# DearCaat/MHIM-MIL

Measured on AMD Instinct MI355X. Metric: patch-instances/sec through MHIM fwd+bwd, N=10k D=1024, higher is better.
Workload: dtype f32; 1 GPU; c2: MHIM(ABMIL) train step, one bag N=10000 D=1024 per GPU per step (teacher fwd + select + student fwd + bwd + Adam + EMA); rotating_bags_per_gpu=8, matrix_core_form=bf16x3, parallelism=dp1, launch=hipGraph replay, one graph per resident bag

## Files before the change

### include/mhimx.h

```cpp
#ifndef MHIMX_H
#define MHIMX_H

#include <stdint.h>

#ifdef __cplusplus
extern "C" {
#endif

#define MHIMX_VERSION 620

enum { MHIMX_ACT_NONE = 0, MHIMX_ACT_RELU = 1, MHIMX_ACT_GELU = 2, MHIMX_ACT_TANH = 3 };

enum { MHIMX_PREC_F32 = 0, MHIMX_PREC_F16S = 1, MHIMX_PREC_BF16X3 = 2 };

const char* mhimx_last_error(void);
int mhimx_version(void);


typedef struct {
  const float* A; int64_t lda; const int64_t* rows;
  const float* B; int64_t ldb;
  float* C; int64_t ldc;
  int64_t M, N, K;
  const float* bias;
// ... 81 lines not shown
  float* C; int64_t ldc;
  int64_t M, K1, K2;
  int32_t splits; float* ws;
  int32_t accumulate;
  int32_t prec;
  int64_t ws_floats;
  mhimx_reduce_list* defer;
} mhimx_gemm_tn_args;
int mhimx_gemm_tn(void* stream, const mhimx_gemm_tn_args* a);

int mhimx_pair_planes(void* stream, const float* x, int64_t ldx, int64_t M, int64_t K, float* out);

#define MHIMX_PREP_MAX 32
typedef struct { int32_t kind; const float* in; float* out; int64_t R, C; } mhimx_prep_job;
int mhimx_prep_batch(void* stream, const mhimx_prep_job* jobs, int32_t n);

int mhimx_transpose(void* stream, const float* in, float* out, int64_t R, int64_t C);

typedef struct {
  int64_t E;
  int64_t A;
  int32_t act;
  int32_t gated;
  int32_t prec;
  const float* wa; const float* ba;
  const float* wb; const float* bb;
  const float* wc; const float* bc;
  const float* wa_frag;
  float gate_drop_p;
  uint64_t gate_drop_seed;
} mhimx_scorer;

typedef struct {
  const float* T1; int64_t M1; const float* T2; int64_t M2;
  float* s; float* stats; float* z;
  float* u_pre;
  const float* wp; int64_t C; float* cproj;
  void* ws; int64_t ws_bytes;
  const float* bp; float* pscore;
  const int64_t* rows1;
  const uint8_t* excl;
  const mhimx_prep_job* ride_jobs;
  int32_t n_ride_jobs;
  int32_t phase; int32_t tail_tokens;
  const void* ride_merge;
  const float* ride_X; int64_t ride_R; void* ride_ws; int64_t ride_ws_bytes;
  int32_t rode_merge;
  const float* tail_wa_t;
  int64_t tail_row0;
  int32_t no_backward;
} mhimx_pool_io;
int64_t mhimx_abmil_pool_ws_bytes(int64_t M, int64_t E, int64_t A, int32_t gated);
int mhimx_abmil_pool_fwd(void* stream, const mhimx_scorer* sc, mhimx_pool_io* io);

typedef struct {
  const float* g_z;
  float* dT1; float* dT2;
  float* d_wa; float* d_ba; float* d_wb; float* d_bb; float* d_wc; float* d_bc;
  const float* wa_t; const float* wb_t;
  int32_t accumulate;
  int32_t splits;
  mhimx_reduce_list* defer;
  const float* wa_t_frag;
  void* img; const void* img_dact; float* img_part; int64_t img_rows;
} mhimx_pool_grad;
int mhimx_abmil_pool_bwd(void* stream, const mhimx_scorer* sc, const mhimx_pool_io* io, const mhimx_pool_grad* g);

int mhimx_softmax_from_stats(void* stream, const float* s, const float* stats, float* attn, int64_t M);

int mhimx_lse_merge(void* stream, const float* parts, int64_t W, int64_t E, float* stats, float* z);

int mhimx_pseudo_score(void* stream, const float* s, const float* stats, const float* cproj, const float* bp,
                       float* score, float* attn_out, int64_t M, int64_t C);

int mhimx_layernorm_fwd(void* stream, const float* x, int64_t M, int64_t E, const float* w, const float* b, float* y, float* mean,
                        float* rstd);
int mhimx_layernorm_bwd(void* stream, const float* dy, const float* x, int64_t M, int64_t E, const float* w, const float* mean,
                        const float* rstd, float* dx, float* d_w, float* d_b, int32_t accumulate, float* ws);
int mhimx_layernorm_bwd_res(void* stream, const float* dy, const float* x, int64_t M, int64_t E, const float* w, const float* mean,
                            const float* rstd, const float* resid, float* dx, float* d_w, float* d_b, int32_t accumulate, float* ws);
int mhimx_dropout_apply(void* stream, const float* x, float* out, int64_t M, int64_t E, float p, uint64_t seed, const uint64_t* tick);
int mhimx_dropout_apply_proj(void* stream, const float* x, float* out, int64_t M, int64_t E, float p, uint64_t seed, const uint64_t* tick);
int mhimx_softmax_rows(void* stream, const float* x, float* y, int64_t R, int64_t L, float alpha);
int mhimx_softmax_rows_bwd(void* stream, const float* y, const float* dy, float* dx, int64_t R, int64_t L, float alpha);
int mhimx_landmark_mean(void* stream, const float* x, int64_t ldx, int64_t T, int64_t l, int64_t C, float* out);
int mhimx_landmark_mean_bwd(void* stream, const float* dout, int64_t T, int64_t l, int64_t C, float* dx, int64_t ldx, int32_t accumulate);
int mhimx_affine_ident(void* stream, const float* x, float* y, int64_t B, int64_t n, float a, float b);
int mhimx_axpby(void* stream, const float* x, float* y, int64_t n, float alpha, float beta);
int mhimx_pinv_init(void* stream, const float* a, int64_t B, int64_t n, float* z, float* stats, float* ws);
int mhimx_pinv_init_bwd(void* stream, const float* dz, const float* z0, const float* stats, int64_t B, int64_t n, float* da, float* ws);
int mhimx_resconv(void* stream, const float* v, int64_t ldv, const float* w, int64_t KS, int64_t dh, int64_t T, int64_t C, float* out,
                  int64_t ldo, int32_t accumulate, int32_t flip);
int64_t mhimx_resconv_dw_ws_floats(int64_t T, int64_t C, int64_t dh, int64_t KS);
int mhimx_resconv_dw(void* stream, const float* dout, int64_t ldo, const float* v, int64_t ldv, int64_t KS, int64_t dh, int64_t T,
                     int64_t C, float* dw, float* ws);
typedef struct mhimx_nys {
  const float* q; const float* k; const float* v;
  int64_t ld, T;
  const float* ql; const float* kl;
  int64_t ldl;
  float scale;
  float* ws;
  int64_t ws_floats;
} mhimx_nys;
int64_t mhimx_nys_ws_floats(int64_t T);
int mhimx_nys_a3v_fwd(void* stream, const mhimx_nys* a, float* a3v, float* lse3);
int mhimx_nys_out_fwd(void* stream, const mhimx_nys* a, const float* w2, float* out, int64_t ldo, float* lse1, int32_t accumulate);
int mhimx_nys_out_bwd(void* stream, const mhimx_nys* a, const float* w2, const float* dout, int64_t ldd, const float* lse1,
                      float* delta1, float* dq, int64_t lddq, float* dkl, int64_t lddl, float* dw2);
int mhimx_nys_a3v_bwd(void* stream, const mhimx_nys* a, const float* a3v, const float* da3v, const float* lse3, float* dk, float* dv,
                      int64_t lddk, int32_t accumulate_dv, float* dql, int64_t lddl);
int mhimx_nys_cls_attn(void* stream, const mhimx_nys* a, const float* lse3, const float* u, float* r);
int64_t mhimx_bn_ws_floats(int64_t M, int64_t C);
int mhimx_bn_fwd(void* stream, const float* x, int64_t M, int64_t C, const float* w, const float* b, float eps, int32_t training, float* mean,
                 float* rstd, float* var_out, float* y, float* ws);
int mhimx_bn_bwd(void* stream, const float* dy, const float* x, int64_t M, int64_t C, const float* w, const float* mean, const float* rstd,
                 int32_t training, float* dx, float* dw, float* db, float* ws);
int mhimx_sincos_add(void* stream, const float* x, const int64_t* pos_xy, int64_t N, int64_t C, float* out);
int mhimx_ppeg_combine(void* stream, const float* w7, const float* w5, const float* w3, const float* b7, const float* b5,
                       const float* b3, int64_t C, float* wc, float* bc);
int mhimx_ppeg_fwd(void* stream, const float* x, int64_t N, int64_t C, const float* wc, const float* bc, float* y,
                   int64_t grid );
int64_t mhimx_ppeg_bwd_ws_floats(int64_t N, int64_t C);
int mhimx_ppeg_bwd(void* stream, const float* dy, const float* x, int64_t N, int64_t C, const float* wc, float* dx, float* dwc, float* dbc,
                   float* ws, int64_t grid);
typedef struct { int64_t H, cell0, ncell, out0, out1; } mhimx_ppeg_band;
int64_t mhimx_ppeg_side(int64_t N, int64_t* wrapN);
int mhimx_ppeg_band_fwd(void* stream, const float* xb, const mhimx_ppeg_band* band, int64_t C, const float* wc, const float* bc, float* y);
int64_t mhimx_ppeg_band_bwd_ws_floats(int64_t n_out, int64_t C);
int mhimx_ppeg_band_bwd(void* stream, const float* dyb, const float* xb, const mhimx_ppeg_band* band, int64_t n_dw, int64_t C, const float* wc,
                        float* dx, float* dwc, float* dbc, float* ws);
int mhimx_scale_heads(void* stream, const float* v, int64_t ldv, const float* a, int64_t lda, int64_t dh, int64_t T, int64_t C, float* out);

int64_t mhimx_select_ws_bytes(int64_t N);
int mhimx_select_mask(void* stream, const float* score, int64_t N, int64_t k, int64_t n_sel, int32_t largest,
                      const int64_t* perm, const int64_t* other, int64_t n_other,
                      int64_t* mask_ids, int64_t* len_keep_dev, int64_t* topk_sorted ,
                      void* ws, int64_t ws_bytes);

int mhimx_select_rows(void* stream, const float* score, int64_t N, int64_t k, int64_t n_sel, int32_t largest,
                      uint64_t rand_seed, const uint64_t* tick, int64_t merge_R, int64_t* rows_out, int64_t* mask_ids,
                      void* ws, int64_t ws_bytes, int32_t merge_first );

int mhimx_select_rows_img(void* stream, const float* score, int64_t N, int64_t k, int64_t n_sel, int32_t largest, uint64_t rand_seed,
                          const uint64_t* tick, int64_t merge_R, int64_t* rows_out, int64_t* rows_img, int64_t img_merge_off, void* ws,
                          int64_t ws_bytes, int32_t merge_first);
int mhimx_vote_scores(void* stream, const float* attn, int64_t H, int64_t N, int64_t k, int32_t largest,
                      float* vote, void* ws, int64_t ws_bytes);

int mhimx_compose_ids(void* stream, const int64_t* a, const int64_t* b, int64_t* out, int64_t n);
int mhimx_random_perm(void* stream, int64_t n, uint64_t seed, const uint64_t* tick, const int64_t* src, int64_t* out);

typedef struct { int64_t row0, N, k, n_sel, merge_R, out0; uint64_t seed; } mhimx_select_bag;
int64_t mhimx_select_rows_many_ws_bytes(int32_t n_bags, const mhimx_select_bag* bags);
int mhimx_select_rows_many(void* stream, const float* score, int32_t n_bags, const mhimx_select_bag* bags, const uint64_t* tick,
                           int64_t* rows_out, void* ws, int64_t ws_bytes, int32_t merge_first);

typedef struct {
  int64_t E; int64_t k;
  int64_t heads; int64_t dim_head;
  const float* q_param;
  const float* ln_w; const float* ln_b;
  const float* wkv; const float* wq; const float* wo; const float* bo;
  const float* wkv_t; const float* wq_t; const float* wo_t;
  float mm;
  float drop_p; uint64_t drop_seed;
  int32_t prec;
  const uint64_t* drop_tick;
  const float* wkv_frag;
  const int64_t* x_rows;
  int32_t prepared;
  int64_t own_lo, own_n;
  float rep;
  int32_t rows_done;
} mhimx_merge;
int64_t mhimx_merge_ws_bytes(int64_t R, int64_t E, int64_t k, int64_t heads, int64_t dim_head);
int mhimx_merge_fwd(void* stream, const mhimx_merge* m, const float* X, int64_t R, float* z, float* q_new,
                    int32_t update_q, void* ws, int64_t ws_bytes);
typedef struct {
  float* d_ln_w; float* d_ln_b; float* d_wkv; float* d_wq; float* d_wo; float* d_bo;
  int32_t accumulate; int32_t splits;
  mhimx_reduce_list* defer;
} mhimx_merge_grad;
int64_t mhimx_merge_part_floats(void);
int mhimx_merge_fwd_part(void* stream, const mhimx_merge* m, const float* X, int64_t R, float* part, void* ws, int64_t ws_bytes);
int mhimx_merge_fwd_finish(void* stream, const mhimx_merge* m, const float* parts, int32_t W, int64_t R, float* z, float* q_new,
                           int32_t update_q, void* ws, int64_t ws_bytes);
int mhimx_merge_bwd(void* stream, const mhimx_merge* m, const float* X, int64_t R, const float* dz, float* dX,
                    const mhimx_merge_grad* g, void* ws, int64_t ws_bytes);
int mhimx_merge_bwd_park(const mhimx_merge* m, const float* X, int64_t R, const float* dz, float* dX, const mhimx_merge_grad* g, void* ws,
                         int64_t ws_bytes);

int mhimx_act_bwd(void* stream, float* dH, const float* H, const float* pre, int64_t M, int64_t E, int32_t act,
                  float drop_p, uint64_t drop_seed, const uint8_t* drop_mask, const int64_t* rows, float* colsum_out,
                  int32_t accumulate, void* ws, int64_t ws_bytes, const uint64_t* drop_tick);
int mhimx_mul_colsum(void* stream, float* dH, const float* dact, int64_t M, int64_t E, float* colsum_out, int32_t accumulate,
                     void* ws, int64_t ws_bytes, mhimx_reduce_list* defer );
int mhimx_rows_dpre(void* stream, const float* dH, const void* dact16, const int64_t* rows, int64_t L, int64_t E, float* dpre,
                    float* colsum_out, int32_t accumulate, void* ws, int64_t ws_bytes, mhimx_reduce_list* defer );
// ... 41 lines not shown

int mhimx_adam_ema(void* stream, float* p, const float* g, float* m, float* v, float* teacher, int64_t n_train,
                   int64_t n_all, int64_t step, float lr, float beta1, float beta2, float eps, float weight_decay,
                   float grad_scale, float ema_mm, int32_t zero_grad ,
                   const uint64_t* step_dev ,
                   const float* mm_table, int64_t mm_len );

typedef struct {
  float* p; float* g; float* m; float* v; float* teacher;
  int64_t n_train, n_all;
  int64_t step; const uint64_t* step_dev;
  float lr; const float* lr_table; int64_t lr_len;
  float beta1, beta2, eps, weight_decay, grad_scale;
  float ema_mm; const float* mm_table; int64_t mm_len;
  int32_t zero_grad;
  const float* g_extra; int64_t n_extra; int64_t extra_pitch;
  float clip_norm;
  float* ws; int64_t ws_floats;
  mhimx_reduce_list* fold;
  int64_t extra_lo;
  int32_t extra_only;
} mhimx_optim_args;
int mhimx_optim_step(void* stream, const mhimx_optim_args* a);

#define MHIMX_STEP_MAX_ROWS 262144
#define MHIMX_WINDOW_MAX 8
typedef struct {
  const float* w1; const float* b1;
  const float* wa; const float* wc;
  const float* wp; const float* bp;
  float* q;
  const float* ln_w; const float* ln_b;
  const float* wkv; const float* wq; const float* wo; const float* bo;
} mhimx_step_params;
typedef struct {
  float* w1; float* b1; float* wa; float* wc; float* wp; float* bp; float* ln_w; float* ln_b; float* wkv; float* wq; float* wo; float* bo;
} mhimx_step_grads;
typedef struct {
  int64_t D, E, A, C, k;
  int32_t act, da_act;
  int32_t attn2score;
  float drop_p_teacher, drop_p_student;
  float merge_drop_p, merge_mm;
  float temp_t, main_alpha, aux_alpha;
  mhimx_step_params student, teacher;
  mhimx_step_grads grad;
  float* p; float* g; float* m; float* v; float* p_teacher;
  int64_t n_train, n_all;
  float lr, beta1, beta2, eps, weight_decay, ema_mm;
  const float* mm_table; int64_t mm_len; const float* lr_table; int64_t lr_len;
  uint64_t* tick; uint64_t* opt_step;
  float* q_out;
  int32_t time_project;
  void* side_stream;
} mhimx_step_cfg;
typedef struct { int64_t k_top, n_sel, len_keep, Lk, R; } mhimx_step_counts;
int mhimx_step_counts_of(int64_t N, double mask_ratio_h, double mask_ratio_hr, double merge_ratio, mhimx_step_counts* out);
typedef struct { uint64_t drop_teacher, drop_student, select, mca; } mhimx_step_seeds;
typedef struct {
  int64_t total;
  int64_t logits, losses;
  int64_t score;
  int64_t rows_all;
  int64_t H_teacher, H_student;
  int64_t dact;
  int64_t z_teacher, z_student, g_z;
  int64_t dH;
} mhimx_step_layout;
int mhimx_step_layout_of(const mhimx_step_cfg* cfg, int64_t N, const mhimx_step_counts* cnt, mhimx_step_layout* out);
int mhimx_step_run(void* stream, const mhimx_step_cfg* cfg, const float* X, int64_t ldx, int64_t N, const int64_t* label_dev,
                   const mhimx_step_counts* cnt, const mhimx_step_seeds* seeds, int64_t host_step, void* ws, int64_t ws_bytes, int32_t update);
int mhimx_step_project_ms(float* ms_out, float* empty_ms_out, int32_t cap);
int mhimx_step_run_many(void* stream, const mhimx_step_cfg* cfg, int32_t n_bags, const float* const* X, const int64_t* ldx, const int64_t* N,
                        const int64_t* const* labels_dev, const mhimx_step_counts* cnt, const mhimx_step_seeds* seeds, int64_t host_step0,
                        void* ws, int64_t ws_bytes);

int mhimx_pure_step_layout_of(const mhimx_step_cfg* cfg, int64_t N, mhimx_step_layout* out);
int mhimx_pure_step_run(void* stream, const mhimx_step_cfg* cfg, const float* X, int64_t ldx, int64_t N, const int64_t* label_dev,
                        uint64_t drop_seed, int64_t host_step, void* ws, int64_t ws_bytes, int32_t update);
int mhimx_pure_step_run_many(void* stream, const mhimx_step_cfg* cfg, int32_t n_bags, const float* const* X, const int64_t* ldx, const int64_t* N,
                             const int64_t* const* labels_dev, const uint64_t* drop_seeds, int64_t host_step0, void* ws, int64_t ws_bytes);

typedef struct { int64_t total, bag0, bag_stride, grad_slab; mhimx_step_layout bag; } mhimx_window_layout;
int mhimx_window_layout_of(const mhimx_step_cfg* cfg, int32_t n_bags, int64_t N, const mhimx_step_counts* cnt, mhimx_window_layout* out);
int mhimx_window_run(void* stream, const mhimx_step_cfg* cfg, int32_t n_bags, const float* const* X, int64_t ldx, int64_t N,
                     const int64_t* const* labels_dev, const mhimx_step_counts* cnt, const mhimx_step_seeds* seeds, int64_t host_step, void* ws,
                     int64_t ws_bytes, int32_t update);

#define MHIMX_PURE_WINDOW_MAX 32
#define MHIMX_PURE_WINDOW_MAX_ROWS 524288
typedef struct {
  const float* X; int64_t ldx, N;
  const int64_t* label_dev;
  uint64_t drop_seed;
} mhimx_pure_window_bag;
typedef struct {
  int64_t total, rows;
  int64_t logits, losses;
  int64_t H, dact, s, stats, z, g_z;
  int64_t row0[MHIMX_PURE_WINDOW_MAX];
} mhimx_pure_window_layout;
int mhimx_pure_window_layout_of(const mhimx_step_cfg* cfg, int32_t n_bags, const mhimx_pure_window_bag* bags, mhimx_pure_window_layout* out);
int mhimx_pure_window_run(void* stream, const mhimx_step_cfg* cfg, int32_t n_bags, const mhimx_pure_window_bag* bags, int64_t host_step,
                          void* ws, int64_t ws_bytes, int32_t update);

#define MHIMX_RAGGED_WINDOW_MAX 32
// ... 241 lines not shown
```

### mhim_mil_amd/_lib.py

```python
from __future__ import annotations

import ctypes as C
import os

HERE = os.path.dirname(os.path.abspath(__file__))
LIB_PATH = os.path.join(HERE, os.environ.get("MHIMX_LIB_NAME", "libmhimx.so"))

c_f32p = C.c_void_p
c_i64p = C.c_void_p
c_u8p = C.c_void_p

ABI_VERSION = 620

ACT = {None: 0, "none": 0, "identity": 0, "relu": 1, "gelu": 2, "tanh": 3}
PREC = {"f32": 0, "f16s": 1, "bf16x3": 2}


def act_code(name, allowed):
    n = name.lower() if isinstance(name, str) else None
    return ACT[n] if n in allowed else 0


class GemmNT(C.Structure):
    _fields_ = [("A", c_f32p), ("lda", C.c_int64), ("rows", c_i64p),
# ... 38 lines not shown
    _fields_ = [("kind", C.c_int32), ("inp", C.c_void_p), ("out", C.c_void_p), ("R", C.c_int64), ("C", C.c_int64)]


class ReduceJob(C.Structure):
    _fields_ = [("kind", C.c_int32), ("accumulate", C.c_int32), ("parts", c_f32p), ("out", c_f32p),
                ("G", C.c_int64), ("W", C.c_int64), ("ld", C.c_int64), ("K1", C.c_int64), ("K2", C.c_int64), ("ldo", C.c_int64)]


REDUCE_MAX = 16


SIDE_BYTES = 512


class SideWork(C.Structure):
    _fields_ = [("pending", C.c_int32), ("reserved", C.c_int32), ("blob", C.c_ubyte * SIDE_BYTES)]


class ParkedGemm(C.Structure):
    _fields_ = [("pending", C.c_int32), ("reserved", C.c_int32), ("blob", C.c_ubyte * 128)]


class ReduceListC(C.Structure):
    _fields_ = [("j", ReduceJob * REDUCE_MAX), ("n", C.c_int32), ("side", SideWork), ("parked", ParkedGemm), ("pre", SideWork)]


class GemmTN(C.Structure):
    _fields_ = [("A", c_f32p), ("lda", C.c_int64),
                ("B", c_f32p), ("ldb", C.c_int64), ("rows", c_i64p),
                ("C", c_f32p), ("ldc", C.c_int64),
                ("M", C.c_int64), ("K1", C.c_int64), ("K2", C.c_int64),
                ("splits", C.c_int32), ("ws", c_f32p),
                ("accumulate", C.c_int32), ("prec", C.c_int32), ("ws_floats", C.c_int64),
                ("defer", C.c_void_p)]


class Scorer(C.Structure):
    _fields_ = [("E", C.c_int64), ("A", C.c_int64), ("act", C.c_int32), ("gated", C.c_int32), ("prec", C.c_int32),
                ("wa", c_f32p), ("ba", c_f32p), ("wb", c_f32p), ("bb", c_f32p), ("wc", c_f32p), ("bc", c_f32p),
                ("wa_frag", c_f32p), ("gate_drop_p", C.c_float), ("gate_drop_seed", C.c_uint64)]


class PoolIO(C.Structure):
    _fields_ = [("T1", c_f32p), ("M1", C.c_int64), ("T2", c_f32p), ("M2", C.c_int64),
                ("s", c_f32p), ("stats", c_f32p), ("z", c_f32p), ("u_pre", c_f32p),
                ("wp", c_f32p), ("C", C.c_int64), ("cproj", c_f32p),
                ("ws", C.c_void_p), ("ws_bytes", C.c_int64), ("bp", c_f32p), ("pscore", c_f32p), ("rows1", c_i64p),
                ("excl", C.c_void_p), ("ride_jobs", C.c_void_p), ("n_ride_jobs", C.c_int32),
                ("phase", C.c_int32), ("tail_tokens", C.c_int32), ("ride_merge", C.c_void_p), ("ride_X", c_f32p), ("ride_R", C.c_int64),
                ("ride_ws", C.c_void_p), ("ride_ws_bytes", C.c_int64), ("rode_merge", C.c_int32), ("tail_wa_t", c_f32p), ("tail_row0", C.c_int64),
                ("no_backward", C.c_int32)]


class PoolGrad(C.Structure):
    _fields_ = [("g_z", c_f32p), ("dT1", c_f32p), ("dT2", c_f32p),
                ("d_wa", c_f32p), ("d_ba", c_f32p), ("d_wb", c_f32p), ("d_bb", c_f32p), ("d_wc", c_f32p),
                ("d_bc", c_f32p), ("wa_t", c_f32p), ("wb_t", c_f32p),
                ("accumulate", C.c_int32), ("splits", C.c_int32), ("defer", C.c_void_p), ("wa_t_frag", c_f32p),
                ("img", C.c_void_p), ("img_dact", C.c_void_p), ("img_part", c_f32p), ("img_rows", C.c_int64)]


class Merge(C.Structure):
    _fields_ = [("E", C.c_int64), ("k", C.c_int64), ("heads", C.c_int64), ("dim_head", C.c_int64),
                ("q_param", c_f32p), ("ln_w", c_f32p), ("ln_b", c_f32p),
                ("wkv", c_f32p), ("wq", c_f32p), ("wo", c_f32p), ("bo", c_f32p),
                ("wkv_t", c_f32p), ("wq_t", c_f32p), ("wo_t", c_f32p),
                ("mm", C.c_float), ("drop_p", C.c_float), ("drop_seed", C.c_uint64), ("prec", C.c_int32), ("drop_tick", C.c_void_p),
                ("wkv_frag", c_f32p), ("x_rows", c_i64p), ("prepared", C.c_int32), ("own_lo", C.c_int64), ("own_n", C.c_int64),
                ("rep", C.c_float), ("rows_done", C.c_int32)]


class MergeGrad(C.Structure):
    _fields_ = [("d_ln_w", c_f32p), ("d_ln_b", c_f32p), ("d_wkv", c_f32p), ("d_wq", c_f32p), ("d_wo", c_f32p),
                ("d_bo", c_f32p), ("accumulate", C.c_int32), ("splits", C.c_int32), ("defer", C.c_void_p)]


_P = C.c_void_p
_I64 = C.c_int64
_I32 = C.c_int32
_F = C.c_float
_U64 = C.c_uint64


class Nys(C.Structure):
    _fields_ = [("q", C.c_void_p), ("k", C.c_void_p), ("v", C.c_void_p), ("ld", C.c_int64), ("T", C.c_int64),
                ("ql", C.c_void_p), ("kl", C.c_void_p), ("ldl", C.c_int64), ("scale", C.c_float),
                ("ws", C.c_void_p), ("ws_floats", C.c_int64)]


class BmmStep(C.Structure):
    _fields_ = [("A", C.c_void_p), ("B", C.c_void_p), ("C", C.c_void_p), ("PN", C.c_void_p), ("PT", C.c_void_p),
                ("PN2", C.c_void_p), ("PT2", C.c_void_p), ("D", C.c_void_p), ("D2", C.c_void_p), ("alpha", C.c_float), ("ident", C.c_float),
                ("alpha2", C.c_float), ("ident2", C.c_float), ("dscale", C.c_float), ("d2scale", C.c_float), ("kind", C.c_int32)]


class OptimArgs(C.Structure):
    _fields_ = [("p", C.c_void_p), ("g", C.c_void_p), ("m", C.c_void_p), ("v", C.c_void_p), ("teacher", C.c_void_p),
                ("n_train", C.c_int64), ("n_all", C.c_int64), ("step", C.c_int64), ("step_dev", C.c_void_p),
                ("lr", C.c_float), ("lr_table", C.c_void_p), ("lr_len", C.c_int64),
                ("beta1", C.c_float), ("beta2", C.c_float), ("eps", C.c_float), ("weight_decay", C.c_float), ("grad_scale", C.c_float),
                ("ema_mm", C.c_float), ("mm_table", C.c_void_p), ("mm_len", C.c_int64), ("zero_grad", C.c_int32),
                ("g_extra", C.c_void_p), ("n_extra", C.c_int64), ("extra_pitch", C.c_int64), ("clip_norm", C.c_float),
                ("ws", C.c_void_p), ("ws_floats", C.c_int64), ("fold", C.c_void_p), ("extra_lo", C.c_int64), ("extra_only", C.c_int32)]


class StepParams(C.Structure):
    _fields_ = [(n, C.c_void_p) for n in ("w1", "b1", "wa", "wc", "wp", "bp", "q", "ln_w", "ln_b", "wkv", "wq", "wo", "bo")]


class StepGrads(C.Structure):
    _fields_ = [(n, C.c_void_p) for n in ("w1", "b1", "wa", "wc", "wp", "bp", "ln_w", "ln_b", "wkv", "wq", "wo", "bo")]


class StepCfg(C.Structure):
    _fields_ = [("D", C.c_int64), ("E", C.c_int64), ("A", C.c_int64), ("C", C.c_int64), ("k", C.c_int64),
                ("act", C.c_int32), ("da_act", C.c_int32), ("attn2score", C.c_int32),
                ("drop_p_teacher", C.c_float), ("drop_p_student", C.c_float), ("merge_drop_p", C.c_float), ("merge_mm", C.c_float),
                ("temp_t", C.c_float), ("main_alpha", C.c_float), ("aux_alpha", C.c_float),
                ("student", StepParams), ("teacher", StepParams), ("grad", StepGrads),
                ("p", C.c_void_p), ("g", C.c_void_p), ("m", C.c_void_p), ("v", C.c_void_p), ("p_teacher", C.c_void_p),
                ("n_train", C.c_int64), ("n_all", C.c_int64),
                ("lr", C.c_float), ("beta1", C.c_float), ("beta2", C.c_float), ("eps", C.c_float), ("weight_decay", C.c_float), ("ema_mm", C.c_float),
                ("mm_table", C.c_void_p), ("mm_len", C.c_int64), ("lr_table", C.c_void_p), ("lr_len", C.c_int64),
                ("tick", C.c_void_p), ("opt_step", C.c_void_p), ("q_out", C.c_void_p), ("time_project", C.c_int32), ("side_stream", C.c_void_p)]


class StepCounts(C.Structure):
    _fields_ = [("k_top", C.c_int64), ("n_sel", C.c_int64), ("len_keep", C.c_int64), ("Lk", C.c_int64), ("R", C.c_int64)]


class StepSeeds(C.Structure):
    _fields_ = [("drop_teacher", C.c_uint64), ("drop_student", C.c_uint64), ("select", C.c_uint64), ("mca", C.c_uint64)]


class StepLayout(C.Structure):
    _fields_ = [(n, C.c_int64) for n in ("total", "logits", "losses", "score", "rows_all", "H_teacher", "H_student", "dact", "z_teacher",
                                        "z_student", "g_z", "dH")]


class WindowLayout(C.Structure):
    _fields_ = [("total", C.c_int64), ("bag0", C.c_int64), ("bag_stride", C.c_int64), ("grad_slab", C.c_int64), ("bag", StepLayout)]


WINDOW_MAX = 8
STEP_MAX_ROWS = 262144


class InferCfg(C.Structure):
    _fields_ = [("D", C.c_int64), ("E", C.c_int64), ("A", C.c_int64), ("C", C.c_int64), ("act", C.c_int32), ("da_act", C.c_int32),
                ("p", StepParams)]


class InferBag(C.Structure):
    _fields_ = [("X", c_f32p), ("ldx", C.c_int64), ("N", C.c_int64)]


class InferOut(C.Structure):
    _fields_ = [(n, c_f32p) for n in ("logits", "z", "stats", "score", "attn", "loss")]


class InferDsmilCfg(C.Structure):
    _fields_ = [("D", C.c_int64), ("E", C.c_int64), ("C", C.c_int64), ("act", C.c_int32), ("cls_attn", C.c_int32), ("no_norm", C.c_int32),
                ("pad", C.c_int32)] + [(n, c_f32p) for n in ("w1", "b1", "wi", "bi", "wq0", "bq0", "wq2", "bq2", "wv", "bv", "wfcc", "bfcc")]


class InferDsmilOut(C.Structure):
    _fields_ = [(n, c_f32p) for n in ("logits_bag", "logits_ins", "logits", "B")] + [("crit", C.c_void_p)] + [(n, c_f32p) for n in ("attn", "loss")]


INFER_MAX = 32


class TransmilLayer(C.Structure):
    _fields_ = [(n, c_f32p) for n in ("ln_w", "ln_b", "w_qkv", "w_out", "b_out", "conv_w")]


class InferTransmilCfg(C.Structure):
# ... 82 lines not shown
                ("q", c_f32p), ("q_out", c_f32p), ("k", C.c_int64), ("cls_attn", C.c_int32), ("pad", C.c_int32),
                ("drop_p_teacher", C.c_float), ("merge_drop_p", C.c_float), ("merge_mm", C.c_float), ("temp_t", C.c_float),
                ("aux_alpha", C.c_float), ("ema_mm", C.c_float), ("p_teacher", c_f32p), ("mm_table", c_f32p), ("mm_len", C.c_int64)]


class DsmilMhimWindowLayout(C.Structure):
    _fields_ = [(n, C.c_int64) for n in ("total", "rows", "tok_rows", "logits", "losses", "logits_bag", "logits_ins", "B", "crit", "B_teacher",
                                        "H_teacher", "H_student", "dact", "score", "rows_all", "tokens")] + [
        ("row0", C.c_int64 * DSMIL_MHIM_WINDOW_MAX), ("tok0", C.c_int64 * DSMIL_MHIM_WINDOW_MAX)]


RAGGED_WINDOW_MAX = 32
RAGGED_WINDOW_MAX_ROWS = 524288


class RaggedWindowBag(C.Structure):
    _fields_ = [("X", c_f32p), ("ldx", C.c_int64), ("N", C.c_int64), ("label_dev", C.c_void_p), ("cnt", StepCounts), ("seeds", StepSeeds)]


class RaggedWindowLayout(C.Structure):
    _fields_ = [(n, C.c_int64) for n in ("total", "rows", "logits", "losses", "score", "rows_all", "H_teacher", "H_student", "dact", "dpre",
                                        "z_teacher", "z_student")] + [("row0", C.c_int64 * RAGGED_WINDOW_MAX)]


class SurvSpec(C.Structure):
    _fields_ = [("alpha", C.c_float), ("eps", C.c_float), ("censor_dev", C.c_void_p * INFER_MAX), ("risk", C.c_void_p)]


SYMBOLS = {
    "mhimx_last_error": (C.c_char_p, []),
    "mhimx_version": (C.c_int, []),
    "mhimx_gemm_nt": (C.c_int, [_P, C.POINTER(GemmNT)]),
    "mhimx_pool_finalize": (C.c_int, [_P, _P, _P, _P, _I64, _I64, _P, _P, _P, _P, _P, _I64, _I64, _P]),
    "mhimx_proj_score_parts": (_I64, [_I64]),
    "mhimx_proj_score_xch_floats": (_I64, [_I64]),
    "mhimx_bag_project": (C.c_int, [_P, C.POINTER(BagProject)]),
    "mhimx_bag_project_multi": (C.c_int, [_P, _P, _I32]),
    "mhimx_gemm_nn": (C.c_int, [_P, C.POINTER(GemmNT), _F, _I32, _P]),
    "mhimx_prep_batch": (C.c_int, [_P, C.POINTER(PrepJob), _I32]),
    "mhimx_pair_planes": (C.c_int, [_P, _P, _I64, _I64, _I64, _P]),
    "mhimx_lse_merge": (C.c_int, [_P, _P, _I64, _I64, _P, _P]),
    "mhimx_gemm_batched": (C.c_int, [_P, _I32, C.POINTER(GemmNT), _I32, _I64, _I64, _I64, _F, _I32, _P]),
    "mhimx_gemm_tn": (C.c_int, [_P, C.POINTER(GemmTN)]),
    "mhimx_transpose": (C.c_int, [_P, _P, _P, _I64, _I64]),
    "mhimx_abmil_pool_ws_bytes": (_I64, [_I64, _I64, _I64, _I32]),
    "mhimx_abmil_pool_fwd": (C.c_int, [_P, C.POINTER(Scorer), C.POINTER(PoolIO)]),
    "mhimx_abmil_pool_bwd": (C.c_int, [_P, C.POINTER(Scorer), C.POINTER(PoolIO), C.POINTER(PoolGrad)]),
    "mhimx_softmax_from_stats": (C.c_int, [_P, _P, _P, _P, _I64]),
    "mhimx_pseudo_score": (C.c_int, [_P, _P, _P, _P, _P, _P, _P, _I64, _I64]),
    "mhimx_select_ws_bytes": (_I64, [_I64]),
    "mhimx_select_mask": (C.c_int, [_P, _P, _I64, _I64, _I64, _I32, _P, _P, _I64, _P, _P, _P, _P, _I64]),
    "mhimx_select_rows": (C.c_int, [_P, _P, _I64, _I64, _I64, _I32, _U64, _P, _I64, _P, _P, _P, _I64, _I32]),
    "mhimx_select_rows_img": (C.c_int, [_P, _P, _I64, _I64, _I64, _I32, _U64, _P, _I64, _P, _P, _I64, _P, _I64, _I32]),
    "mhimx_vote_scores": (C.c_int, [_P, _P, _I64, _I64, _I64, _I32, _P, _P, _I64]),
    "mhimx_compose_ids": (C.c_int, [_P, _P, _P, _P, _I64]),
    "mhimx_random_perm": (C.c_int, [_P, _I64, _U64, _P, _P, _P]),
    "mhimx_select_rows_many_ws_bytes": (_I64, [_I32, _P]),
    "mhimx_select_rows_many": (C.c_int, [_P, _P, _I32, _P, _P, _P, _P, _I64, _I32]),
    "mhimx_merge_ws_bytes": (_I64, [_I64, _I64, _I64, _I64, _I64]),
    "mhimx_merge_fwd": (C.c_int, [_P, C.POINTER(Merge), _P, _I64, _P, _P, _I32, _P, _I64]),
    "mhimx_merge_part_floats": (_I64, []),
    "mhimx_merge_fwd_part": (C.c_int, [_P, C.POINTER(Merge), _P, _I64, _P, _P, _I64]),
    "mhimx_merge_fwd_finish": (C.c_int, [_P, C.POINTER(Merge), _P, _I32, _I64, _P, _P, _I32, _P, _I64]),
    "mhimx_merge_bwd": (C.c_int, [_P, C.POINTER(Merge), _P, _I64, _P, _P, C.POINTER(MergeGrad), _P, _I64]),
    "mhimx_merge_bwd_park": (C.c_int, [C.POINTER(Merge), _P, _I64, _P, _P, C.POINTER(MergeGrad), _P, _I64]),
    "mhimx_act_bwd": (C.c_int, [_P, _P, _P, _P, _I64, _I64, _I32, _F, _U64, _P, _P, _P, _I32, _P, _I64, _P]),
    "mhimx_softmax_cols": (C.c_int, [_P, _P, _P, _I64, _I64, _F]),
    "mhimx_softmax_cols_bwd": (C.c_int, [_P, _P, _P, _P, _I64, _I64, _F]),
    "mhimx_colmax": (C.c_int, [_P, _P, _I64, _I64, _P, _P]),
    "mhimx_rowmax": (C.c_int, [_P, _P, _I64, _I64, _P]),
    "mhimx_dsmil_head": (C.c_int, [_P, _P, _P, _P, _P, _P, _I64, _I64, _F, _F, _F, _F, _P, _P, _P, _P, _P]),
    "mhimx_mul_colsum": (C.c_int, [_P, _P, _P, _I64, _I64, _P, _I32, _P, _I64, _P]),
    "mhimx_rows_dpre": (C.c_int, [_P, _P, _P, _P, _I64, _I64, _P, _P, _I32, _P, _I64, _P]),
    "mhimx_bmm_affine": (C.c_int, [_P, _I32, _P, _I32, _I64, _I64, _I64, C.c_float, C.c_float]),
    "mhimx_bmm_affine2": (C.c_int, [_P, _I32, _P, _I32, _I64, _I64, _I64, C.c_float, C.c_float, _P, C.c_float, C.c_float]),
    "mhimx_bmm_affine_pair": (C.c_int, [_P, _I32, C.POINTER(GemmNT), _F, _F, _I32, C.POINTER(GemmNT), _F, _F, _I32, _I64]),
    "mhimx_shard_flags": (C.c_int, [_P, _P, _I64, _I64, _I64, _I64, _I64, _I32, _P]),
    "mhimx_shard_gather": (C.c_int, [_P, _P, _I64, _P, _I64, _I64, _I64, _P]),
    "mhimx_shard_scatter": (C.c_int, [_P, _P, _I64, _P, _I64, _I64, _I64, _P]),
    "mhimx_rows_dpre_image": (C.c_int, [_P, _P, _P, _P, _I64, _I64, _P, _P, _I32, _P, _I64, _P]),
    "mhimx_rows_dpre_image_c": (C.c_int, [_P, _P, _P, _P, _I64, _I64, _P, _P, _I32, _P, _I64, _P]),
    "mhimx_rows_dpre_image_k": (C.c_int, [_P, _P, _P, _P, _I64, _I64, _P, _P, _I32, _P, _I64, _P]),
    "mhimx_wgrad_image_bytes": (_I64, [_I64, _I64]),
    "mhimx_wgrad_ws_floats": (_I64, [_I64, _I64, _I64]),
    "mhimx_bag_wgrad": (C.c_int, [_P, _P]),
    "mhimx_bag_wgrad_multi": (C.c_int, [_P, _P, _I32]),
    "mhimx_wgrad_multi_ws_floats": (C.c_int64, [_I64, _I64, _I64, _I32]),
    "mhimx_reduce_flush": (C.c_int, [_P, _P]),
    "mhimx_cls_metrics_ws_bytes": (C.c_int64, [_I64, _I64, _I64]),
    "mhimx_cls_metrics": (C.c_int, [_P, _P, _I64, _P, _I64, _I64, _I32, _P, _I64, _P, _P, _I64]),
    "mhimx_surv_nll": (C.c_int, [_P, _P, _I64, _P, _P, _I64, _I64, _F, _F, _F, _P, _P, _P]),
    "mhimx_cindex_ws_bytes": (C.c_int64, [_I64, _I64]),
    "mhimx_cindex": (C.c_int, [_P, _P, _P, _P, _I64, _P, _I64, _F, _P, _P, _I64]),
    "mhimx_colsum": (C.c_int, [_P, _P, _I64, _I64, _P, _I32, _P, _I64]),
    "mhimx_head_fwd_bwd": (C.c_int, [_P, _P, _P, _P, _P, _P, _I64, _I64, _F, _F, _F, _F, _P, _P, _P, _P, _P, _I32, _P, _P]),
    "mhimx_head_surv_fwd_bwd": (C.c_int, [_P, _P, _P, _P, _P, _P, _P, _I64, _I64, _F, _F, _F, _F, _F, _F, _P, _P, _P, _P, _P, _P, _I32]),
    "mhimx_adam_ema": (C.c_int, [_P, _P, _P, _P, _P, _P, _I64, _I64, _I64, _F, _F, _F, _F, _F, _F, _F, _I32, _P, _P, _I64]),
    "mhimx_bmm_chain": (C.c_int, [_P, C.POINTER(BmmStep), _I32, _I32, _P]),
    "mhimx_optim_step": (C.c_int, [_P, C.POINTER(OptimArgs)]),
    "mhimx_stream_copy": (C.c_int, [_P, _P, _P, _I64]),
    "mhimx_tick": (C.c_int, [_P, _P]),
    "mhimx_layernorm_fwd": (C.c_int, [_P, _P, _I64, _I64, _P, _P, _P, _P, _P]),
    "mhimx_layernorm_bwd": (C.c_int, [_P, _P, _P, _I64, _I64, _P, _P, _P, _P, _P, _P, _I32, _P]),
    "mhimx_layernorm_bwd_res": (C.c_int, [_P, _P, _P, _I64, _I64, _P, _P, _P, _P, _P, _P, _P, _I32, _P]),
    "mhimx_dropout_apply": (C.c_int, [_P, _P, _P, _I64, _I64, _F, _U64, _P]),
    "mhimx_dropout_apply_proj": (C.c_int, [_P, _P, _P, _I64, _I64, _F, _U64, _P]),
# ... 102 lines not shown
```

### mhim_mil_amd/csrc/rows.hip

```cpp
#include <math.h>
#include <string.h>

#include "mca2_rows.hpp"
#include "reduce_jobs.hpp"

namespace mhimx {

int gemm_nt(hipStream_t st, const mhimx_gemm_nt_args& g);
int gemm_tn(hipStream_t st, const mhimx_gemm_tn_args& g);
bool scorer_fused_ok(int64_t E, int64_t A, int gated, int prec, const float* T, const float* wa, const float* wp, int64_t C);
int scorer_fused_fwd(hipStream_t st, const float* T, int64_t M, const float* wa, const float* wa_frag, const float* ba, int act, const float* wc,
                     const float* bc, const float* wp, int C, float* u_pre, float* s_out, float* cproj, float* pm, float* pl,
                     float* pz, int max_parts, const int64_t* rows, const uint8_t* excl, const mhimx_prep_job* ride_jobs, int n_ride_jobs,
                     const void* merge_rows);
int merge2_fwd_rows_args(const mhimx_merge* m, const float* X, int64_t R, void* ws, int64_t ws_bytes, M2RowsFwd* out);
int prep_batch(hipStream_t st, const mhimx_prep_job* jobs, int n);
int scorer_fused_bwd(hipStream_t st, const float* T, int64_t M, const float* u_pre, const float* s_in, const float* stats,
                     const float* g_z, const float* z, const float* wc, int act, const float* wa_t, const float* wa_t_frag, float* du,
                     float* dT, float* dwc_part, float* dbc_part, int max_parts, const int64_t* rows, const void* pre_side, int64_t gate_row0,
                     void* img, const void* img_dact, float* img_part, int64_t img_rows);

constexpr int ROWS_THREADS = 256;
constexpr int MAX_PART = 512;
constexpr int TN_SLABS = 128;

MHIMX_DEV float sigmoidf_(float x) { return 1.f / (1.f + __expf(-x)); }

constexpr int FWD_WAVES = 16;
template <int EPL>
__global__ __launch_bounds__(64 * FWD_WAVES) void score_rows_fwd_kernel(
    const float* __restrict__ T, int64_t M, int E, int A, int act, int gated, const float* __restrict__ u_pre,
    const float* __restrict__ wc, const float* __restrict__ bc, const float* __restrict__ wp, int C,
    float* __restrict__ s_out, float* __restrict__ cproj, float* __restrict__ pm, float* __restrict__ pl,
    float* __restrict__ pz, float gdrop_p, uint64_t gdrop_seed, int64_t row0 ) {
  extern __shared__ __attribute__((aligned(16))) float sm[];
  constexpr int NWV = FWD_WAVES;
  const int lane = threadIdx.x & 63, wave = threadIdx.x >> 6;
  const int ldu = A * (1 + gated);
  const float bias_c = bc ? bc[0] : 0.f;

  float mw = -INFINITY, lw = 0.f, zacc[EPL];
#pragma unroll
  for (int q = 0; q < EPL; ++q) zacc[q] = 0.f;

  for (int64_t n = (int64_t)blockIdx.x * NWV + wave; n < M; n += (int64_t)gridDim.x * NWV) {
    const float* up = u_pre + n * ldu;
    float part = 0.f;
    const bool gdrop = gated && gdrop_p > 0.f;
    const uint32_t rkey = gdrop ? drop_row_key(gdrop_seed, (uint64_t)(row0 + n)) : 0u;
    const float ginv = gdrop ? 1.f / (1.f - gdrop_p) : 1.f;
    for (int j = lane; j < A; j += 64) {
      float u = act_fwd(up[j], act);
      if (gated) {
        float sg = sigmoidf_(up[A + j]);
        if (gdrop) {
          u = drop_keep_k(rkey, (uint32_t)j, gdrop_p) ? u * ginv : 0.f;
          sg = drop_keep_k(rkey, (uint32_t)(A + j), gdrop_p) ? sg * ginv : 0.f;
        }
        u *= sg;
      }
      part += wc[j] * u;
    }
    const float s = wave_sum(part) + bias_c;
    const float* h = T + n * (int64_t)E;
    float hv[EPL];
#pragma unroll
    for (int q = 0; q < EPL; ++q) hv[q] = h[lane + 64 * q];
// ... 770 lines not shown

static int grid_for_ln(int64_t M) {
  int64_t g = cdiv(M, 4);
  if (g < 1) g = 1;
  if (g > MAX_PART) g = MAX_PART;
  return (int)g;
}

static int grid_for_rows(int64_t M) {
  int64_t g = cdiv(M, 20);
  if (g < 1) g = 1;
  if (g > MAX_PART) g = MAX_PART;
  return (int)g;
}

struct PoolWs {
  float *pm, *pl, *pz, *attn, *du, *dwc_part, *dbc_part, *u_pre, *tn_ws, *nt_ws;
};

static int64_t pool_ws_layout(Arena& ar, int64_t M, int64_t E, int64_t A, int gated, PoolWs* w) {
  const int64_t G = 2 * MAX_PART;
  PoolWs t;
  t.pm = ar.take<float>(G);
  t.pl = ar.take<float>(G);
  t.pz = ar.take<float>(G * E);
  t.attn = ar.take<float>(M);
  t.du = ar.take<float>(M * A * (1 + gated));
  t.dwc_part = ar.take<float>(G * A);
  t.dbc_part = ar.take<float>(G);
  t.u_pre = ar.take<float>(M * A * (1 + gated));
  t.tn_ws = ar.take<float>((int64_t)TN_SLABS * A * E);
  t.nt_ws = ar.take<float>(4 * M * A);
  if (w) *w = t;
  return ar.off;
}

template <typename F>
static int dispatch_epl(int64_t E, F&& f) {
  switch (E) {
    case 256: return f(std::integral_constant<int, 4>());
    case 512: return f(std::integral_constant<int, 8>());
    case 1024: return f(std::integral_constant<int, 16>());
    default: return fail(-1, "token width E=%lld unsupported (256, 512 or 1024)", (long long)E);
  }
}

static int check_scorer(const mhimx_scorer* sc) {
  MHIMX_CHECK_ARG(sc && sc->wa && sc->wc, "scorer: null weights");
  MHIMX_CHECK_ARG(sc->A > 0 && sc->A <= 512 && sc->A % 4 == 0, "scorer: A must be a multiple of 4, <= 512");
  MHIMX_CHECK_ARG(!sc->gated || sc->wb, "scorer: gated needs wb");
  return 0;
}

int abmil_pool_fwd(hipStream_t st, const mhimx_scorer* sc, mhimx_pool_io* io) {
  if (int r = check_scorer(sc)) return r;
  MHIMX_CHECK_ARG(io && io->T1 && io->M1 > 0 && io->s && io->stats && io->z, "pool_fwd: null io");
  MHIMX_CHECK_ARG(io->M2 == 0 || io->T2, "pool_fwd: M2>0 needs T2");
  MHIMX_CHECK_ARG(!io->cproj || (io->wp && io->C > 0), "pool_fwd: cproj needs wp, C");
  MHIMX_CHECK_ARG(!io->rows1 || (io->M2 == 0 && scorer_fused_ok(sc->E, sc->A, sc->gated, sc->prec, io->T1, sc->wa, io->cproj ? io->wp : nullptr, io->C)),
                  "pool_fwd: gathered tokens (rows1) need the one-pass scorer (E = 512, A = 128, plain form, not f32) and a single segment");
  MHIMX_CHECK_ARG(!io->excl || scorer_fused_ok(sc->E, sc->A, sc->gated, sc->prec, io->T1, sc->wa, io->cproj ? io->wp : nullptr, io->C),
                  "pool_fwd: excluded rows (excl) need the one-pass scorer (E = 512, A = 128, plain form, not f32)");
  const int64_t M = io->M1 + io->M2, E = sc->E, A = sc->A;
  const int gated = sc->gated ? 1 : 0;
  Arena ar(io->ws, io->ws_bytes);
  PoolWs w;
  pool_ws_layout(ar, M, E, A, gated, &w);
  MHIMX_CHECK_ARG(ar.ok(), "pool_fwd: workspace too small (%lld < %lld)", (long long)io->ws_bytes, (long long)ar.off);
  float* u_pre = io->u_pre ? io->u_pre : w.u_pre;
  const int64_t ldu = A * (1 + gated);
  if (io->phase != 0) {
    const int64_t K = io->tail_tokens, Ms1 = io->M1 - K;
    MHIMX_CHECK_ARG((io->phase == 1 || io->phase == 2) && K >= 1 && K <= FIN_MAXTOK && Ms1 >= 1 && io->M2 == 0 && !io->cproj && !io->pscore && !io->excl &&
                        E == 512 && A == 128 && scorer_fused_ok(E, A, gated, sc->prec, io->T1, sc->wa, nullptr, 0),
                    "pool_fwd: the two-call forward takes the one-pass scorer shapes, one segment, 1..%d tail tokens, no class projections", FIN_MAXTOK);
    const int tiles = (int)cdiv(Ms1, 32);
    const int G1 = tiles < MAX_PART ? tiles : MAX_PART;
    if (io->phase == 1) {
      M2RowsFwd mfbuf;
      const void* mf = nullptr;
      io->rode_merge = 0;
      if (io->ride_merge) {
        const int rc = merge2_fwd_rows_args(reinterpret_cast<const mhimx_merge*>(io->ride_merge), io->ride_X, io->ride_R, io->ride_ws, io->ride_ws_bytes,
                                            &mfbuf);
        if (rc < 0) return rc;
        if (rc == 0) { mf = &mfbuf; io->rode_merge = 1; }
      }
      const int g1 = scorer_fused_fwd(st, io->T1, Ms1, sc->wa, sc->wa_frag, sc->ba, sc->act, sc->wc, sc->bc, nullptr, 0, u_pre, io->s, nullptr, w.pm, w.pl,
                                      w.pz, MAX_PART, io->rows1, nullptr, io->ride_jobs, io->n_ride_jobs, mf);
      return g1 < 0 ? g1 : 0;
    }
    hipLaunchKernelGGL(pool_finalize_tok_kernel, bgrid((unsigned)cdiv(E, 64)), dim3(FIN_THREADS), 0, st, w.pm, w.pl, w.pz, G1, (int)E, io->stats, io->z, io->T1,
                       (io->rows1 && io->tail_row0 < 0) ? io->rows1 + Ms1 : nullptr, io->rows1 ? io->tail_row0 : Ms1, (int)K, sc->wa, io->tail_wa_t, sc->ba, sc->wc,
                       sc->bc, (int)A, sc->act, u_pre + Ms1 * ldu, io->s + Ms1, cur_batch());
    MHIMX_LAUNCH_CHECK();
    return 0;
  }

  const float* Ts[2] = {io->T1, io->T2};
  const int64_t Ms[2] = {io->M1, io->M2};
  int64_t off = 0;
  int G = 0;
  bool rode = false;
  for (int seg = 0; seg < 2; ++seg) {
    if (Ms[seg] == 0) continue;
    if (scorer_fused_ok(E, A, gated, sc->prec, Ts[seg], sc->wa, io->cproj ? io->wp : nullptr, io->C)) {
      const int g1 = scorer_fused_fwd(st, Ts[seg], Ms[seg], sc->wa, sc->wa_frag, sc->ba, sc->act, sc->wc, sc->bc, io->cproj ? io->wp : nullptr,
                                      (int)io->C, io->no_backward ? nullptr : u_pre + off * ldu, io->s + off, io->cproj ? io->cproj + off * io->C : nullptr,
                                      w.pm + G, w.pl + G, w.pz + (int64_t)G * E, MAX_PART, seg == 0 ? io->rows1 : nullptr,
                                      seg == 0 ? io->excl : nullptr, rode ? nullptr : io->ride_jobs, rode ? 0 : io->n_ride_jobs, nullptr);
      if (g1 < 0) return g1;
      rode = true;
      G += g1;
      off += Ms[seg];
      continue;
    }
    MHIMX_CHECK_ARG(cur_batch().n == 0, "pool_fwd: a bag-batched launch needs the one-pass scorer");
    mhimx_gemm_nt_args g = {};
    g.A = Ts[seg]; g.lda = E; g.B = sc->wa; g.ldb = E; g.C = u_pre + off * ldu; g.ldc = ldu;
    g.M = Ms[seg]; g.N = A; g.K = E; g.bias = sc->ba;
    g.ws = w.nt_ws; g.ws_floats = 4 * M * A;
    g.prec = sc->prec == MHIMX_PREC_F32 ? MHIMX_PREC_F32 : MHIMX_PREC_BF16X3;
    if (int r = gemm_nt(st, g)) return r;
    if (gated) {
      g.B = sc->wb; g.bias = sc->bb; g.C = u_pre + off * ldu + A;
      if (int r = gemm_nt(st, g)) return r;
    }
    int grid = (int)cdiv(Ms[seg], 5 * FWD_WAVES);
    if (grid < 1) grid = 1;
    if (grid > MAX_PART) grid = MAX_PART;
    const float* Tseg = Ts[seg];
    const int64_t Mseg = Ms[seg];
    int r = dispatch_epl(E, [&](auto epl) {
      constexpr int EPL = decltype(epl)::value;
      const size_t smem = (size_t)(FWD_WAVES * E + 2 * FWD_WAVES) * sizeof(float);
      if (smem > 48 * 1024)
        MHIMX_ONCE_PER_DEVICE(MHIMX_HIP(hipFuncSetAttribute((const void*)score_rows_fwd_kernel<EPL>, hipFuncAttributeMaxDynamicSharedMemorySize, (int)smem)));
      hipLaunchKernelGGL(score_rows_fwd_kernel<EPL>, dim3(grid), dim3(64 * FWD_WAVES), smem, st, Tseg, Mseg, (int)E, (int)A,
                         sc->act, gated, u_pre + off * ldu, sc->wc, sc->bc, io->cproj ? io->wp : nullptr, (int)io->C,
                         io->s + off, io->cproj ? io->cproj + off * io->C : nullptr, w.pm + G, w.pl + G,
                         w.pz + (int64_t)G * E, sc->gate_drop_p, sc->gate_drop_seed, off);
      MHIMX_LAUNCH_CHECK();
      return 0;
    });
    if (r) return r;
    G += grid;
    off += Ms[seg];
  }
  if (!rode && io->ride_jobs && io->n_ride_jobs > 0)
    if (int r = prep_batch(st, io->ride_jobs, io->n_ride_jobs)) return r;
  MHIMX_CHECK_ARG(!io->pscore || io->cproj, "pool_fwd: pscore needs cproj (and wp)");
  static_assert(2 * MAX_PART <= FIN_THREADS, "pool_finalize_kernel reads one partial per thread");
  const int64_t ps_blocks = io->pscore ? (cdiv(io->M1, FIN_THREADS) < 64 ? cdiv(io->M1, FIN_THREADS) : 64) : 0;
  hipLaunchKernelGGL(pool_finalize_kernel, bgrid((unsigned)(cdiv(E, 64) + ps_blocks)), dim3(FIN_THREADS), 0, st, w.pm, w.pl, w.pz, G, (int)E, io->stats,
                     io->z, io->s, io->cproj, io->bp, (int)io->C, io->M1, io->pscore, cur_batch());
  MHIMX_LAUNCH_CHECK();
  return 0;
}

int abmil_pool_bwd(hipStream_t st, const mhimx_scorer* sc, const mhimx_pool_io* io, const mhimx_pool_grad* gr) {
  if (int r = check_scorer(sc)) return r;
  MHIMX_CHECK_ARG(io && gr && gr->g_z && gr->dT1 && gr->d_wa && gr->d_wc && gr->wa_t, "pool_bwd: null args");
  MHIMX_CHECK_ARG(io->M2 == 0 || gr->dT2, "pool_bwd: M2>0 needs dT2");
// ... 203 lines not shown
      Merge2Side sz = {};
      sz.w.T = list->parked.reserved - 1;
      list->parked.reserved = 0;
      const int rc = gemm_tn_rider(st, pg, &sz, 5);
      if (rc < 0) return rc;
    } else if (int r = gemm_tn(st, pg)) return r;
  }
  if (int r = merge2_side_finish(st, &list->side, list->n == 0 ? 3 : 2)) return r;
  if (list->n == 0) return 0;
  ReduceJobs rj;
  rj.side_blocks = 0;
  if (list->side.pending == 3) {
    memcpy(&rj.side, list->side.blob, sizeof(rj.side));
    rj.side_blocks = merge2_side_blocks(3, rj.side);
    list->side.pending = 0;
  }
  for (int i = 0; i < list->n; ++i) {
    const mhimx_reduce_job& j = list->j[i];
    MHIMX_CHECK_ARG(j.parts && j.out && j.G > 0 && (j.kind == 0 ? j.W > 0 : (j.kind == 1 && j.K1 > 0 && j.K2 > 0)), "reduce_flush: bad job %d", i);
  }
  const int first = reduce_table_fill(rj.t, list->j, list->n, RP_THREADS);
  list->n = 0;
  hipLaunchKernelGGL(reduce_batch_kernel, bgrid((unsigned)(first + rj.side_blocks)), dim3(RP_THREADS), 0, st, rj, cur_batch());
  MHIMX_LAUNCH_CHECK();
  return 0;
}

int colsum(hipStream_t st, const float* X, int64_t M, int64_t E, float* out, int accumulate, void* ws, int64_t ws_bytes) {
  MHIMX_CHECK_ARG(X && out && E > 0 && M >= 0, "colsum: bad args");
  const int64_t nrows = M > 0 ? M : 1, avail = ws ? ws_bytes / (E * 4) : 0;
  int64_t want = cdiv(nrows, 16) < 512 ? cdiv(nrows, 16) : 512;
  MHIMX_CHECK_ARG(avail >= (want < 128 ? want : 128), "colsum: workspace too small (need %lld bytes)", (long long)((want < 128 ? want : 128) * E * 4));
  if (want > avail) want = avail;
  const int64_t chunk = cdiv(M > 0 ? M : 1, want);
  const int gy = (int)cdiv(M > 0 ? M : 1, chunk);
  hipLaunchKernelGGL(colsum_part_kernel, dim3((unsigned)cdiv(E, 128), gy), dim3(128), 0, st, X, M, (int)E, chunk, (float*)ws);
  MHIMX_LAUNCH_CHECK();
  hipLaunchKernelGGL(reduce_parts_kernel, dim3((unsigned)cdiv(E, 32)), dim3(RP_THREADS), 0, st, (const float*)ws, gy, (int)E, (int)E, out, accumulate);
  MHIMX_LAUNCH_CHECK();
  return 0;
}

}

using namespace mhimx;

extern "C" int64_t mhimx_abmil_pool_ws_bytes(int64_t M, int64_t E, int64_t A, int32_t gated) {
  Arena ar(nullptr, 0);
  return pool_ws_layout(ar, M, E, A, gated ? 1 : 0, nullptr);
}
extern "C" int mhimx_abmil_pool_fwd(void* stream, const mhimx_scorer* sc, mhimx_pool_io* io) {
  return abmil_pool_fwd((hipStream_t)stream, sc, io);
}
extern "C" int mhimx_abmil_pool_bwd(void* stream, const mhimx_scorer* sc, const mhimx_pool_io* io, const mhimx_pool_grad* g) {
  return abmil_pool_bwd((hipStream_t)stream, sc, io, g);
}
extern "C" int mhimx_softmax_from_stats(void* stream, const float* s, const float* stats, float* attn, int64_t M) {
  if (M <= 0) return 0;
  hipLaunchKernelGGL(softmax_from_stats_kernel, bgrid((unsigned)(cdiv(M, 256) < 1024 ? cdiv(M, 256) : 1024)), dim3(256), 0,
                     (hipStream_t)stream, s, stats, attn, M, cur_batch());
  MHIMX_LAUNCH_CHECK();
  return 0;
}
extern "C" int mhimx_lse_merge(void* stream, const float* parts, int64_t W, int64_t E, float* stats, float* z) {
  MHIMX_CHECK_ARG(parts && stats && z && W >= 1 && E >= 1, "lse_merge: bad args");
  hipLaunchKernelGGL(lse_merge_kernel, dim3((unsigned)cdiv(E, 256)), dim3(256), 0, (hipStream_t)stream, parts, (int)W, (int)E, stats, z);
  MHIMX_LAUNCH_CHECK();
  return 0;
}
extern "C" int mhimx_pseudo_score(void* stream, const float* s, const float* stats, const float* cproj, const float* bp,
                                  float* score, float* attn_out, int64_t M, int64_t C) {
  MHIMX_CHECK_ARG((!s || stats) && cproj && score && C > 0, "pseudo_score: null args");
  if (M <= 0) return 0;
  hipLaunchKernelGGL(pseudo_score_kernel, dim3((unsigned)(cdiv(M, 256) < 1024 ? cdiv(M, 256) : 1024)), dim3(256), 0,
                     (hipStream_t)stream, s, stats, cproj, bp, score, attn_out, M, (int)C);
  MHIMX_LAUNCH_CHECK();
  return 0;
}
extern "C" int mhimx_act_bwd(void* stream, float* dH, const float* H, const float* pre, int64_t M, int64_t E, int32_t act,
                             float drop_p, uint64_t drop_seed, const uint8_t* drop_mask, const int64_t* rows, float* colsum_out,
                             int32_t accumulate, void* ws, int64_t ws_bytes, const uint64_t* drop_tick) {
  MHIMX_CHECK_ARG(dH && (H || pre), "act_bwd: null args");
  MHIMX_CHECK_ARG(act == MHIMX_ACT_NONE || act == MHIMX_ACT_RELU || pre, "act_bwd: gelu/tanh need the pre-activation");
  if (M <= 0) return 0;
  int64_t nblk = cdiv(M, 16);
  if (nblk > 1024) nblk = 1024;
  const int64_t chunk = cdiv(M, nblk);
  nblk = cdiv(M, chunk);
  MHIMX_CHECK_ARG(!colsum_out || (ws && ws_bytes >= nblk * E * 4), "act_bwd: workspace too small for the column sums (%lld bytes)",
                  (long long)(nblk * E * 4));
  hipLaunchKernelGGL(act_bwd_kernel, dim3((unsigned)nblk), dim3(256), 0, (hipStream_t)stream, dH, H, pre, M, (int)E, act, drop_p,
                     drop_seed, drop_mask, rows, chunk, colsum_out ? (float*)ws : nullptr, drop_tick);
  MHIMX_LAUNCH_CHECK();
  if (colsum_out) {
    hipLaunchKernelGGL(reduce_parts_kernel, dim3((unsigned)cdiv(E, 32)), dim3(RP_THREADS), 0, (hipStream_t)stream, (const float*)ws, (int)nblk,
                       (int)E, (int)E, colsum_out, accumulate);
    MHIMX_LAUNCH_CHECK();
  }
  return 0;
}
extern "C" int mhimx_colmax(void* stream, const float* x, int64_t M, int64_t C, float* vals, int64_t* idx) {
  MHIMX_CHECK_ARG(x && vals && idx && M > 0 && C > 0 && C <= 16, "colmax: bad args (C <= 16)");
  hipLaunchKernelGGL(colmax_kernel, dim3(1), dim3(1024), 0, (hipStream_t)stream, x, M, (int)C, vals, idx);
  MHIMX_LAUNCH_CHECK();
  return 0;
}
// ... 116 lines not shown
```

### mhim_mil_amd/csrc/scorer_fused.hip

```cpp
#include <math.h>

#include "common.hpp"
#include "mca2_rows.hpp"
#include "prep_jobs.hpp"

namespace mhimx {

typedef float sf_f32x16 __attribute__((ext_vector_type(16)));
typedef float sf_f4 __attribute__((ext_vector_type(4)));
typedef __bf16 sf_b8 __attribute__((ext_vector_type(8)));

#ifdef MHIMX_SF_PROF
__device__ unsigned long long sf_prof[16];
#define SF_STAMP(i) do { __syncthreads(); if (threadIdx.x == 0 && blockIdx.x == 7) sf_prof[i] = wall_clock64(); } while (0)
#else
#define SF_STAMP(i)
#endif

constexpr int SF_ROWS = 32, SF_E = 512, SF_A = 128, SF_LD = SF_E + 4, SF_THREADS = 256;
constexpr int SF_MAXC = 4;
constexpr size_t SF_SMEM = (size_t)(SF_ROWS * SF_LD + 4 * SF_ROWS + 2 * SF_ROWS + SF_MAXC * SF_E + 2 * SF_ROWS) * sizeof(float);

MHIMX_DEV void sf_split(const sf_f4& a, const sf_f4& b, sf_b8& hi, sf_b8& lo) {
  const float x[8] = {a[0], a[1], a[2], a[3], b[0], b[1], b[2], b[3]};
#pragma unroll
  for (int i = 0; i < 8; ++i) {
    const __bf16 h = (__bf16)x[i];
    hi[i] = h;
    lo[i] = (__bf16)(x[i] - (float)h);
  }
}

MHIMX_DEV float sf_sum32(float v) {
  v += dpp_mov<0xB1, 0xf>(0.f, v);
  v += dpp_mov<0x4E, 0xf>(0.f, v);
  v += dpp_mov<0x141, 0xf>(0.f, v);
  v += dpp_mov<0x140, 0xf>(0.f, v);
  v += dpp_mov<0x142, 0xa>(0.f, v);
  return v;
}

template <bool FRAG>
__global__ __launch_bounds__(SF_THREADS, 2) void scorer_fused_kernel(
    const float* __restrict__ T, int64_t M, const float* __restrict__ wa, const float* __restrict__ wa_frag,
    const float* __restrict__ ba, int act,
    const float* __restrict__ wc, const float* __restrict__ bc, const float* __restrict__ wp, int C, float* __restrict__ u_pre,
    float* __restrict__ s_out, float* __restrict__ cproj, float* __restrict__ pm, float* __restrict__ pl, float* __restrict__ pz,
    int tiles, const int64_t* __restrict__ rows ,
    const uint8_t* __restrict__ excl ,
    int n_main , PrepJobs rider,
    int n_front ,
    M2RowsFwd mf, BagBatch bb ) {
  extern __shared__ __attribute__((aligned(16))) float sf_sm[];
  if (blockIdx.z) {
    MHIMX_BAG(T); MHIMX_BAG(u_pre); MHIMX_BAG(s_out); MHIMX_BAG(cproj); MHIMX_BAG(pm); MHIMX_BAG(pl); MHIMX_BAG(pz); MHIMX_BAG(rows); MHIMX_BAG(excl);
    MHIMX_BAG(wa_frag);
    bag_move(mf, bb);
  }
  if ((int)blockIdx.x < n_front) {
    if ((int)blockIdx.x < mf.w.T)
      merge2_rows_fwd_body<16>((int)blockIdx.x, sf_sm, mf.X, mf.xrows, mf.R, mf.ln_w, mf.ln_b, mf.J, mf.drop_p, mf.seed0, mf.tick, mf.w);
    return;
  }
  const int bid = (int)blockIdx.x - n_front;
  if (bid >= n_main) {
    prep_job_block(rider, bid - n_main, sf_sm);
    return;
  }
  float* Hs = sf_sm;
  float* sred = Hs + SF_ROWS * SF_LD;
  float* srow = sred + 4 * SF_ROWS;
  float* prow = srow + SF_ROWS;
  float* wps = prow + SF_ROWS;
  int64_t* ridx = reinterpret_cast<int64_t*>(wps + SF_MAXC * SF_E);
  const int tid = threadIdx.x, lane = tid & 63, wave = tid >> 6;
  const int r32 = lane & 31, kg = lane >> 5;
  const int n_col = 32 * wave + r32;
  const float bias_c = bc ? bc[0] : 0.f;
  const float bn = ba ? ba[n_col] : 0.f, wn = wc[n_col];
  const float* bptr = wa + (int64_t)n_col * SF_E + 8 * kg;
  const float* fptr = wa_frag ? wa_frag + ((int64_t)wave * (SF_E / 16) * 64 + lane) * 8 : nullptr;
  const unsigned foff = ((unsigned)wave * (SF_E / 16) * 64 + (unsigned)lane) * 8;
  const float* aptr = Hs + r32 * SF_LD + 8 * kg;
  if (wp)
    for (int i = tid; i < C * SF_E / 4; i += SF_THREADS) reinterpret_cast<sf_f4*>(wps)[i] = reinterpret_cast<const sf_f4*>(wp)[i];

  float m_run = -INFINITY, l_run = 0.f, z0 = 0.f, z1 = 0.f;
  for (int tile = bid; tile < tiles; tile += n_main) {
    const int64_t row0 = (int64_t)tile * SF_ROWS;
    SF_STAMP(0);
    sf_f32x16 acc, acc2, acc3;
    if constexpr (FRAG) {
    if (rows) {
      if (tid < SF_ROWS) { const int64_t n = row0 + tid; ridx[tid] = rows[n < M ? n : M - 1]; }
      __syncthreads();
    }
    const int lr = tid >> 3, ls = tid & 7;
    const int64_t ln = row0 + lr;
    const float* lsrc = T + (rows ? ridx[lr] : (ln < M ? ln : M - 1)) * SF_E + 4 * ls;
    float* ldst = Hs + lr * SF_LD + 4 * ls;
    const unsigned fo = foff * 4;
    sf_f4 av[16], bh_[4], bl_[4];
#pragma unroll
    for (int i = 0; i < 16; ++i) { acc[i] = 0.f; acc2[i] = 0.f; acc3[i] = 0.f; }
#define SF_LOAD_A(c)                                                                                                                          \
    asm volatile("global_load_dwordx4 %0, %4, off offset:%5\n\tglobal_load_dwordx4 %1, %4, off offset:%6\n\t"                                  \
                 "global_load_dwordx4 %2, %4, off offset:%7\n\tglobal_load_dwordx4 %3, %4, off offset:%8"                                      \
                 : "=&v"(av[4 * (c)]), "=&v"(av[4 * (c) + 1]), "=&v"(av[4 * (c) + 2]), "=&v"(av[4 * (c) + 3])                                  \
                 : "v"(lsrc), "i"(512 * (c)), "i"(512 * (c) + 128), "i"(512 * (c) + 256), "i"(512 * (c) + 384) : "memory")
#define SF_LOAD_B(ks)                                                                                                                         \
    asm volatile("s_nop 4\n\tglobal_load_dwordx4 %0, %2, %3\n\tglobal_load_dwordx4 %1, %2, %3 offset:16"                                      \
                 : "=&v"(bh_[(ks) & 3]), "=&v"(bl_[(ks) & 3]) : "v"(fo + 2048u * (ks)), "s"(wa_frag) : "memory")
#define SF_WAIT_B(n, ks) asm volatile("s_waitcnt vmcnt(" #n ")" : "+v"(bh_[(ks) & 3]), "+v"(bl_[(ks) & 3]) : : "memory")
#define SF_WAIT_A(n, c)                                                                                                                       \
    asm volatile("s_waitcnt vmcnt(" #n ")" : "+v"(av[4 * (c)]), "+v"(av[4 * (c) + 1]), "+v"(av[4 * (c) + 2]), "+v"(av[4 * (c) + 3]) : : "memory")
#define SF_KSTEP(ks, n, refill)                                                                                                               \
    {                                                                                                                                        \
      SF_WAIT_B(n, ks);                                                                                                                      \
      const sf_b8 bh = __builtin_bit_cast(sf_b8, bh_[(ks) & 3]), bl = __builtin_bit_cast(sf_b8, bl_[(ks) & 3]);                             \
      if (refill) SF_LOAD_B((ks) + 4 < SF_E / 16 ? (ks) + 4 : (ks));                                                                         \
      const sf_f4 a0 = *reinterpret_cast<const sf_f4*>(aptr + 16 * (ks)), a1 = *reinterpret_cast<const sf_f4*>(aptr + 16 * (ks) + 4);       \
      sf_b8 ah, al;                                                                                                                          \
      sf_split(a0, a1, ah, al);                                                                                                              \
      acc2 = __builtin_amdgcn_mfma_f32_32x32x16_bf16(al, bh, acc2, 0, 0, 0);                                                                 \
      acc = __builtin_amdgcn_mfma_f32_32x32x16_bf16(ah, bh, acc, 0, 0, 0);                                                                   \
      acc3 = __builtin_amdgcn_mfma_f32_32x32x16_bf16(ah, bl, acc3, 0, 0, 0);                                                                 \
    }
#define SF_STORE_A(c)                                                                                                                         \
    _Pragma("unroll") for (int q = 0; q < 4; ++q)                                                                                            \
        *reinterpret_cast<sf_f4*>(ldst + 128 * (c) + 32 * q) = ln < M ? av[4 * (c) + q] : sf_f4{0.f, 0.f, 0.f, 0.f};
    SF_LOAD_A(0);
    SF_LOAD_A(1);
    SF_LOAD_B(0); SF_LOAD_B(1); SF_LOAD_B(2); SF_LOAD_B(3);
    SF_WAIT_A(12, 0);
    SF_STORE_A(0);
    __syncthreads();
    SF_STAMP(1);
    SF_LOAD_A(2);
    SF_KSTEP(0, 10, true) SF_KSTEP(1, 10, true) SF_KSTEP(2, 10, true) SF_KSTEP(3, 10, true)
    SF_KSTEP(4, 6, true) SF_KSTEP(5, 6, true) SF_KSTEP(6, 6, true) SF_KSTEP(7, 6, true)
    SF_WAIT_A(8, 1);
    SF_STORE_A(1);
    __syncthreads();
// ... 23 lines not shown
    }
#pragma unroll
    for (int i = 0; i < 16; ++i) {
      const int f = tid + SF_THREADS * i, r = f >> 7, c4 = f & 127;
      const int64_t n = row0 + r;
      const int64_t nc = n < M ? n : M - 1;
      sf_f4 v = reinterpret_cast<const sf_f4*>(T + (rows ? ridx[r] : nc) * SF_E)[c4];
      if (n >= M) v = sf_f4{0.f, 0.f, 0.f, 0.f};
      *reinterpret_cast<sf_f4*>(Hs + r * SF_LD + 4 * c4) = v;
    }
    __syncthreads();
    SF_STAMP(1);
#pragma unroll
    for (int i = 0; i < 16; ++i) { acc[i] = 0.f; acc2[i] = 0.f; acc3[i] = 0.f; }
    {
      sf_f4 b0 = *reinterpret_cast<const sf_f4*>(bptr), b1 = *reinterpret_cast<const sf_f4*>(bptr + 4);
#pragma unroll 4
      for (int ks = 0; ks < SF_E / 16; ++ks) {
        const int kn = ks + 1 < SF_E / 16 ? ks + 1 : ks;
        const sf_f4 nb0 = *reinterpret_cast<const sf_f4*>(bptr + 16 * kn), nb1 = *reinterpret_cast<const sf_f4*>(bptr + 16 * kn + 4);
        const sf_f4 a0 = *reinterpret_cast<const sf_f4*>(aptr + 16 * ks), a1 = *reinterpret_cast<const sf_f4*>(aptr + 16 * ks + 4);
        sf_b8 ah, al, bh, bl;
        sf_split(a0, a1, ah, al);
        sf_split(b0, b1, bh, bl);
        acc2 = __builtin_amdgcn_mfma_f32_32x32x16_bf16(al, bh, acc2, 0, 0, 0);
        acc = __builtin_amdgcn_mfma_f32_32x32x16_bf16(ah, bh, acc, 0, 0, 0);
        acc3 = __builtin_amdgcn_mfma_f32_32x32x16_bf16(ah, bl, acc3, 0, 0, 0);
        b0 = nb0;
        b1 = nb1;
      }
    }
    }
#pragma unroll
    for (int i = 0; i < 16; ++i) acc[i] += acc2[i] + acc3[i];
    SF_STAMP(2);
#pragma unroll
    for (int i = 0; i < 16; ++i) {
      const int row = 8 * (i >> 2) + 4 * kg + (i & 3);
      const int64_t n = row0 + row;
      const float u = acc[i] + bn;
      if (n < M && u_pre) u_pre[n * SF_A + n_col] = u;
      const float v = sf_sum32(wn * act_fwd(u, act));
      if (r32 == 31) sred[wave * SF_ROWS + row] = v;
    }
    __syncthreads();
    if (tid < SF_ROWS) {
      const int64_t n = row0 + tid;
      float s = (sred[tid] + sred[SF_ROWS + tid]) + (sred[2 * SF_ROWS + tid] + sred[3 * SF_ROWS + tid]) + bias_c;
      if (n >= M || (excl && excl[rows ? ridx[tid] : n])) s = -INFINITY;
      if (n < M) s_out[n] = s;
      srow[tid] = s;
    }
    __syncthreads();
    SF_STAMP(3);
    float mt = -INFINITY;
#pragma unroll
    for (int q = 0; q < SF_ROWS / 4; ++q) {
      const sf_f4 v = reinterpret_cast<const sf_f4*>(srow)[q];
      mt = fmaxf(fmaxf(mt, fmaxf(v[0], v[1])), fmaxf(v[2], v[3]));
    }
    const float m_new = fmaxf(m_run, mt);
    const float scale = (m_run == -INFINITY) ? 0.f : __expf(m_run - m_new);
    if (tid < SF_ROWS) prow[tid] = srow[tid] == -INFINITY ? 0.f : __expf(srow[tid] - m_new);
    __syncthreads();
    float lsum = 0.f, a0 = 0.f, a1 = 0.f;
#pragma unroll
    for (int q = 0; q < SF_ROWS / 4; ++q) {
      const sf_f4 p = reinterpret_cast<const sf_f4*>(prow)[q];
#pragma unroll
      for (int j = 0; j < 4; ++j) {
        const float* hr = Hs + (4 * q + j) * SF_LD;
        lsum += p[j];
        a0 += p[j] * hr[tid];
        a1 += p[j] * hr[tid + SF_THREADS];
      }
    }
    l_run = l_run * scale + lsum;
    z0 = z0 * scale + a0;
    z1 = z1 * scale + a1;
    m_run = m_new;
    SF_STAMP(4);
    if (wp) {
      const int r = tid >> 3, seg = tid & 7;
      const int64_t n = row0 + r;
      const sf_f4* hr = reinterpret_cast<const sf_f4*>(Hs + r * SF_LD) + seg;
      for (int c = 0; c < C; ++c) {
        const sf_f4* w = reinterpret_cast<const sf_f4*>(wps + c * SF_E) + seg;
        float d = 0.f;
#pragma unroll 8
        for (int q = 0; q < 16; ++q) {
          const sf_f4 hv = hr[8 * q], ww = w[8 * q];
          d += hv[0] * ww[0] + hv[1] * ww[1] + hv[2] * ww[2] + hv[3] * ww[3];
        }
        d += dpp_mov<0xB1, 0xf>(0.f, d);
        d += dpp_mov<0x4E, 0xf>(0.f, d);
        d += dpp_mov<0x141, 0xf>(0.f, d);
        if (seg == 0 && n < M) cproj[n * C + c] = d;
      }
    }
    __syncthreads();
    SF_STAMP(5);
  }
  if (tid == 0) { pm[bid] = m_run; pl[bid] = l_run; }
  pz[(int64_t)bid * SF_E + tid] = z0;
  pz[(int64_t)bid * SF_E + tid + SF_THREADS] = z1;
}
// ... 323 lines not shown
          *reinterpret_cast<sf_f4*>(u) = __builtin_bit_cast(sf_f4, hi);
          *reinterpret_cast<sf_f4*>(u + 2048) = __builtin_bit_cast(sf_f4, lo);
        }
        if (img_part) {
          const float tot = cs + __shfl_xor(cs, 32);
          if (kg == 0) img_part[(int64_t)tile * SF_E + e] = tot;
        }
      }
    } else {
#pragma unroll
    for (int nt = 0; nt < 4; ++nt) {
      const int e = 128 * wave + 32 * nt + r32;
      const float ge = gzs[e];
#pragma unroll
      for (int i = 0; i < 16; ++i) {
        const int row = 8 * (i >> 2) + 4 * kg + (i & 3);
        const int64_t n = row0 + row;
        if (n < M) {
          const int64_t dr = rows ? ridx[row] : n;
          const float v = acc[nt][i] + an_s[row] * ge;
          if (gated && dr >= gate_row0) {
            if (n < tok_n0) __hip_atomic_store(dT + dr * SF_E + e, v, __ATOMIC_RELAXED, __HIP_MEMORY_SCOPE_AGENT);
          } else dT[dr * SF_E + e] = v;
        }
      }
    }
    }
    if (gated) asm volatile("s_waitcnt vmcnt(0)" ::: "memory");
    __syncthreads();
    if (gated && wave == 0) {
      const int64_t n = row0 + lane;
      const bool mine = lane < SF_ROWS && n < M && (rows ? ridx[lane < SF_ROWS ? lane : 0] : n) >= gate_row0 && n < tok_n0;
      const unsigned cnt = (unsigned)__builtin_popcountll(__builtin_amdgcn_ballot_w64(mine));
      if (lane == 0 && cnt) __hip_atomic_fetch_add(pre.w.gate + 1, cnt, __ATOMIC_RELAXED, __HIP_MEMORY_SCOPE_AGENT);
    }
  }
  dwc_s[half * SF_A + a_col] = dwc_run;
  __syncthreads();
  if (tid < SF_A) dwc_part[(int64_t)bx * SF_A + tid] = dwc_s[tid] + dwc_s[SF_A + tid];
  if (tid == 0) dbc_part[bx] = dbc_run;
}

#ifdef MHIMX_SF_PROF
extern "C" int mhimx_sf_prof_read(unsigned long long* out) { return (int)hipMemcpyFromSymbol(out, HIP_SYMBOL(sf_prof), 16 * 8); }
#endif

bool scorer_fused_ok(int64_t E, int64_t A, int gated, int prec, const float* T, const float* wa, const float* wp, int64_t C) {
  return E == SF_E && A == SF_A && !gated && prec != MHIMX_PREC_F32 && aligned16(T) && aligned16(wa) && (!wp || (aligned16(wp) && C <= SF_MAXC));
}

int scorer_fused_fwd(hipStream_t st, const float* T, int64_t M, const float* wa, const float* wa_frag, const float* ba, int act, const float* wc,
                     const float* bc, const float* wp, int C, float* u_pre, float* s_out, float* cproj, float* pm, float* pl,
                     float* pz, int max_parts, const int64_t* rows, const uint8_t* excl, const mhimx_prep_job* ride_jobs, int n_ride_jobs,
                     const void* merge_rows ) {
  MHIMX_ONCE_PER_DEVICE(MHIMX_HIP(hipFuncSetAttribute((const void*)scorer_fused_kernel<true>, hipFuncAttributeMaxDynamicSharedMemorySize, (int)SF_SMEM)));
  MHIMX_ONCE_PER_DEVICE(MHIMX_HIP(hipFuncSetAttribute((const void*)scorer_fused_kernel<false>, hipFuncAttributeMaxDynamicSharedMemorySize, (int)SF_SMEM)));
  const int tiles = (int)cdiv(M, SF_ROWS);
  const int grid = tiles < max_parts ? tiles : max_parts;
  static_assert(SF_SMEM >= PREP_LDS_FLOATS * sizeof(float), "the riders' LDS is the scorer's");
  static_assert(SF_SMEM >= m2_fwd_smem(16), "the Merge row tiles' LDS is the scorer's");
  static_assert(SF_THREADS == 256 && SF_THREADS == M2_THREADS, "the preparation jobs and the Merge row tiles are written for 256 threads");
  PrepJobs rider = {};
  int ride_blocks = 0;
  MHIMX_CHECK_ARG(!(ride_jobs && n_ride_jobs > 0 && cur_batch().n > 0), "scorer: preparation jobs do not ride in a bag-batched launch");
  if (ride_jobs && n_ride_jobs > 0) {
    ride_blocks = prep_jobs_fill(ride_jobs, n_ride_jobs, &rider);
    if (ride_blocks < 0) return ride_blocks;
  }
  M2RowsFwd mf = {};
  int n_front = 0;
  if (merge_rows) {
    mf = *reinterpret_cast<const M2RowsFwd*>(merge_rows);
    n_front = mf.w.T;
  }
  if (wa_frag)
    hipLaunchKernelGGL(scorer_fused_kernel<true>, bgrid(n_front + grid + ride_blocks), dim3(SF_THREADS), SF_SMEM, st, T, M, wa, wa_frag, ba, act, wc, bc, wp, C, u_pre,
                       s_out, cproj, pm, pl, pz, tiles, rows, excl, grid, rider, n_front, mf, cur_batch());
  else
    hipLaunchKernelGGL(scorer_fused_kernel<false>, bgrid(n_front + grid + ride_blocks), dim3(SF_THREADS), SF_SMEM, st, T, M, wa, wa_frag, ba, act, wc, bc, wp, C, u_pre,
                       s_out, cproj, pm, pl, pz, tiles, rows, excl, grid, rider, n_front, mf, cur_batch());
  MHIMX_LAUNCH_CHECK();
  return grid;
}

int scorer_fused_bwd(hipStream_t st, const float* T, int64_t M, const float* u_pre, const float* s_in, const float* stats,
                     const float* g_z, const float* z, const float* wc, int act, const float* wa_t, const float* wa_t_frag, float* du,
                     float* dT, float* dwc_part, float* dbc_part, int max_parts, const int64_t* rows, const void* pre_side, int64_t gate_row0,
                     void* img, const void* img_dact, float* img_part, int64_t img_rows) {
    MHIMX_ONCE_PER_DEVICE(MHIMX_HIP(hipFuncSetAttribute((const void*)scorer_fused_bwd_kernel, hipFuncAttributeMaxDynamicSharedMemorySize, (int)SB_SMEM_IMG)));
  MHIMX_CHECK_ARG(!img || (img_dact && aligned16(img) && aligned16(img_dact) && img_rows >= 0 && img_rows <= M),
                  "scorer backward: the dPRE image needs the d out / d pre rows, 16-byte aligned buffers and img_rows <= M");
  const int tiles = (int)cdiv(M, SF_ROWS);
  const int grid = tiles < max_parts ? tiles : max_parts;
  static_assert(SB_SMEM >= M2_BWD_PRE_LDS * sizeof(float), "the riding Merge stage's LDS is the backward's");
  static_assert(SF_THREADS == M2_THREADS, "the riding Merge stage is written for 256 threads");
  MHIMX_CHECK_ARG(!pre_side || gate_row0 >= 0, "scorer backward: a riding Merge stage needs the first row of its dz in dT");
  Merge2Side pre = {};
  int front = 0, ride = 0;
  if (pre_side) {
    pre = *reinterpret_cast<const Merge2Side*>(pre_side);
    front = 1;
    ride = M2_BWD_PRE_BLOCKS;
  } else {
    gate_row0 = -1;
  }
  hipLaunchKernelGGL(scorer_fused_bwd_kernel, bgrid(front + grid + ride), dim3(SF_THREADS), img ? SB_SMEM_IMG : SB_SMEM, st, T, M, u_pre, s_in, stats, g_z, z, wc, act, wa_t,
                     wa_t_frag, du, dT, dwc_part, dbc_part, tiles, rows, grid, pre, gate_row0, (char*)img, (const _Float16*)img_dact, img_part, img_rows, cur_batch());
  MHIMX_LAUNCH_CHECK();
  return grid;
}

}
```

### mhim_mil_amd/csrc/select.hip

```cpp
#include "select_dev.hpp"

namespace mhimx {

#ifdef MHIMX_SEL_PROF
__device__ unsigned long long sel_prof[32];
#define SEL_STAMP(i) do { __syncthreads(); if (threadIdx.x == 0) sel_prof[i] = wall_clock64(); } while (0)
#else
#define SEL_STAMP(i)
#endif


template <bool VOTE>
__global__ __launch_bounds__(SEL_THREADS) void select_kernel(
    const float* __restrict__ score_all, int64_t N, int k, int n_sel, int largest, const int64_t* __restrict__ perm,
    const int64_t* __restrict__ other, int64_t n_other, int64_t* __restrict__ mask_ids,
    int64_t* __restrict__ len_keep_dev, int64_t* __restrict__ topk_out, uint8_t* __restrict__ flags,
    float* __restrict__ vote, int P ) {
  extern __shared__ __attribute__((aligned(16))) char smem_raw[];
  uint64_t* keys = reinterpret_cast<uint64_t*>(smem_raw);
  uint32_t* hist = reinterpret_cast<uint32_t*>(keys + P);
  uint32_t* wave_tot = hist + SEL_WAVES * 256;
  uint32_t* misc = wave_tot + SEL_WAVES;
  const int tid = threadIdx.x, lane = tid & 63, wave = tid >> 6;
  const float* score = score_all + (VOTE ? (int64_t)blockIdx.x * N : 0);
  const bool lg = largest != 0;

  uint32_t mn = 0xFFFFFFFFu, mx = 0u;
  for (int64_t i = tid; i < N; i += SEL_THREADS) {
    const uint32_t key = mono32(score[i], lg);
    mn = key < mn ? key : mn;
    mx = key > mx ? key : mx;
  }
#pragma unroll
  for (int o = 32; o > 0; o >>= 1) {
    const uint32_t a = (uint32_t)__shfl_xor((int)mn, o, 64), c = (uint32_t)__shfl_xor((int)mx, o, 64);
    mn = a < mn ? a : mn;
    mx = c > mx ? c : mx;
  }
  if (lane == 0) { hist[wave] = mn; hist[SEL_WAVES + wave] = mx; }
  __syncthreads();
  for (int w = 0; w < SEL_WAVES; ++w) {
    const uint32_t a = hist[w], c = hist[SEL_WAVES + w];
    mn = a < mn ? a : mn;
    mx = c > mx ? c : mx;
  }
  __syncthreads();
  uint32_t prefix = mx, remaining = (uint32_t)k;
  if (mn != mx) {
    const int hb = 31 - __clz(mn ^ mx);
    uint32_t fixed_mask = hb >= 31 ? 0u : ~((2u << hb) - 1u);
    prefix = mx & fixed_mask;
    int shift = hb - 7 < 0 ? 0 : hb - 7;
// ... 78 lines not shown
      __syncthreads();
    }
  }
  if (topk_out)
    for (int j = tid; j < k; j += SEL_THREADS) topk_out[j] = (int64_t)(0xFFFFFFFFu - (uint32_t)(keys[j] & 0xFFFFFFFFull));

  for (int64_t i = tid; i < N; i += SEL_THREADS) flags[i] = 0;
  __syncthreads();
  const bool has_other = other != nullptr && n_other > 0;
  const int64_t len_keep_simple = N - n_sel;
  for (int j = tid; j < n_sel; j += SEL_THREADS) {
    const int64_t src = perm ? perm[j] : (int64_t)j;
    const int64_t idx = (int64_t)(0xFFFFFFFFu - (uint32_t)(keys[src] & 0xFFFFFFFFull));
    flags[idx] = 1;
    if (!has_other) mask_ids[len_keep_simple + j] = idx;
  }
  if (has_other)
    for (int64_t j = tid; j < n_other; j += SEL_THREADS) flags[other[j]] = 1;
  __threadfence_block();
  __syncthreads();

  uint32_t kept_base = 0;
  for (int64_t c0 = 0; c0 < N; c0 += SEL_THREADS) {
    const int64_t i = c0 + tid;
    const bool keep = (i < N) && flags[i] == 0;
    uint32_t tot;
    const uint32_t rank = block_prefix(keep, wave_tot, &tot);
    if (keep) mask_ids[kept_base + rank] = i;
    kept_base += tot;
  }
  if (has_other) {
    uint32_t m_base = 0;
    for (int64_t c0 = 0; c0 < N; c0 += SEL_THREADS) {
      const int64_t i = c0 + tid;
      const bool msk = (i < N) && flags[i] != 0;
      uint32_t tot;
      const uint32_t rank = block_prefix(msk, wave_tot, &tot);
      if (msk) mask_ids[kept_base + m_base + rank] = i;
      m_base += tot;
    }
  }
  if (tid == 0 && len_keep_dev) *len_keep_dev = (int64_t)kept_base;
}



template <int KPT, bool LEAN = false>
__global__ __launch_bounds__(SEL_THREADS) void select_small_kernel(
    const float* __restrict__ score, int N, int k, int n_sel, int largest, const int64_t* __restrict__ perm,
    const int64_t* __restrict__ other, int64_t n_other, int64_t* __restrict__ mask_ids, int64_t* __restrict__ len_keep_dev,
    int64_t* __restrict__ topk_out, int P, int use_rand, uint64_t rand_seed0, const uint64_t* __restrict__ tick, int merge_R,
    int64_t* __restrict__ rows_out,
    int64_t* __restrict__ rows_img ,
    int img_off, BagBatch bb ) {
  extern __shared__ __attribute__((aligned(16))) char smem_raw[];
  if (blockIdx.z) {
    MHIMX_BAG(score); MHIMX_BAG(perm); MHIMX_BAG(other); MHIMX_BAG(mask_ids); MHIMX_BAG(len_keep_dev); MHIMX_BAG(topk_out); MHIMX_BAG(rows_out);
    MHIMX_BAG(rows_img);
    rand_seed0 = bag_sel_seed(rand_seed0, bb);
  }
  const uint64_t rand_seed = eff_seed(rand_seed0, tick);
  uint64_t* keys = reinterpret_cast<uint64_t*>(smem_raw);
  uint64_t* sorted = keys + P;
  uint32_t* hist = reinterpret_cast<uint32_t*>(sorted + P);
  uint32_t* wave_tot = hist + SEL_COPIES * SEL_BINS;
  uint32_t* misc = wave_tot + SEL_WAVES;
  uint32_t* bitmap = misc + 8;
  uint32_t* rank = bitmap + 512;
  uint16_t* klist = reinterpret_cast<uint16_t*>(rank + P);
  uint16_t* stage = reinterpret_cast<uint16_t*>(smem_raw);
  const int tid = threadIdx.x;
  const bool lg = largest != 0;
  const int i0 = tid * KPT;

  SEL_STAMP(8);
  uint32_t key[KPT];
  bool valid[KPT];
#pragma unroll
  for (int j = 0; j < KPT; ++j) {
    valid[j] = (i0 + j) < N;
    key[j] = valid[j] ? mono32(score[i0 + j], lg) : 0u;
  }
  SEL_STAMP(0);
  for (int i = tid; i < 512; i += SEL_THREADS) bitmap[i] = 0;
  if (tid == 0) misc[2] = 0;

  uint32_t remaining, n_eq;
  const uint32_t T = radix_select_regs<KPT, false>(key, valid, (uint32_t)k, hist, wave_tot, misc, &remaining, &n_eq);

  SEL_STAMP(1);
  uint32_t eq_rank = 0;
  if (remaining != n_eq) {
    uint32_t neq = 0;
#pragma unroll
    for (int j = 0; j < KPT; ++j) neq += (valid[j] && key[j] == T) ? 1u : 0u;
    uint32_t tot;
    eq_rank = block_scan_excl(neq, wave_tot, &tot);
  }
  bool take[KPT];
  uint32_t ntake = 0;
#pragma unroll
  for (int j = 0; j < KPT; ++j) {
    bool t = valid[j] && key[j] > T;
    if (valid[j] && key[j] == T) { t = remaining == n_eq || eq_rank < remaining; ++eq_rank; }
    take[j] = t;
    ntake += t ? 1u : 0u;
  }
  {
// ... 359 lines not shown

using namespace mhimx;

#ifdef MHIMX_SEL_PROF
extern "C" int mhimx_sel_prof_read(unsigned long long* out) {
  return (int)hipMemcpyFromSymbol(out, HIP_SYMBOL(mhimx::sel_prof), 32 * 8);
}
#endif

static int64_t selm_extra_bytes() { return 3 * SELM_BINS * 4 + 2 * 16384 * 4 + 4 * SELM_MAXG * 4 + 256 + 16384 * 8; }
extern "C" int64_t mhimx_select_ws_bytes(int64_t N) { return align_up(N, 256) + (N > 16384 ? selm_extra_bytes() : 0); }

static int select_multi(hipStream_t st, const float* score, int64_t N, int k, int n_sel, int largest, const int64_t* perm, const int64_t* other,
                        int64_t n_other, int64_t* mask_ids, int64_t* len_keep_dev, int64_t* topk_sorted, void* ws, int P) {
  char* base = (char*)ws;
  SelMultiWs w;
  const int64_t nf = align_up(N, 256);
  w.flags = (uint8_t*)base;
  w.hist = (uint32_t*)(base + nf);
  w.rank = w.hist + 3 * SELM_BINS;
  w.selpos = w.rank + 16384;
  w.blk_gt = w.selpos + 16384;
  w.blk_eq = w.blk_gt + SELM_MAXG;
  w.blk_keep = w.blk_eq + SELM_MAXG;
  w.blk_mask = w.blk_keep + SELM_MAXG;
  w.state = w.blk_mask + SELM_MAXG;
  w.cand = (uint64_t*)((char*)w.state + 256);
  MHIMX_CHECK_ARG(aligned16(ws), "select_mask: workspace must be 16-byte aligned");
  sel_zero(st, base, nf + (3 * SELM_BINS + 2 * 16384) * 4);
  int G = (int)cdiv(N, 4 * SEL_THREADS);
  if (G > SELM_MAXG) G = SELM_MAXG;
  if (G < 1) G = 1;
  const int64_t chunk = cdiv(N, G);
  hipLaunchKernelGGL(selm_hist_kernel<0>, dim3(G), dim3(SEL_THREADS), 0, st, score, N, largest, k, w);
  hipLaunchKernelGGL(selm_hist_kernel<1>, dim3(G), dim3(SEL_THREADS), 0, st, score, N, largest, k, w);
  hipLaunchKernelGGL(selm_hist_kernel<2>, dim3(G), dim3(SEL_THREADS), 0, st, score, N, largest, k, w);
  hipLaunchKernelGGL(selm_count_kernel, dim3(G), dim3(SEL_THREADS), 0, st, score, N, largest, k, chunk, w);
  hipLaunchKernelGGL(selm_gather_kernel, dim3(G), dim3(SEL_THREADS), 0, st, score, N, largest, chunk, w);
  (void)P;
  hipLaunchKernelGGL(selm_rank_kernel, dim3((unsigned)cdiv(k, SEL_THREADS), (unsigned)cdiv(k, SELM_SEG)), dim3(SEL_THREADS), 0, st, k, n_sel, perm, w);
  hipLaunchKernelGGL(selm_finish_kernel, dim3((unsigned)(cdiv(k, SEL_THREADS) < 16 ? 16 : cdiv(k, SEL_THREADS))), dim3(SEL_THREADS), 0, st, k, n_sel, N,
                     other, n_other, mask_ids, topk_sorted, w);
  hipLaunchKernelGGL(selm_keepcount_kernel, dim3(G), dim3(SEL_THREADS), 0, st, N, chunk, w);
  hipLaunchKernelGGL(selm_compact_kernel, dim3(G), dim3(SEL_THREADS), 0, st, N, chunk, (other != nullptr && n_other > 0) ? 1 : 0, mask_ids,
                     len_keep_dev, w);
  MHIMX_LAUNCH_CHECK();
  return 0;
}

static int select_impl(void* stream, const float* score, int64_t N, int64_t k, int64_t n_sel, int32_t largest,
                       const int64_t* perm, const int64_t* other, int64_t n_other, int64_t* mask_ids,
                       int64_t* len_keep_dev, int64_t* topk_sorted, void* ws, int64_t ws_bytes, int g_use_rand,
                       uint64_t g_rand_seed, const uint64_t* g_tick, int g_merge_R, int64_t* g_rows_out, int64_t* g_rows_img = nullptr,
                       int g_img_off = 0) {
  MHIMX_CHECK_ARG(score && (mask_ids || g_rows_out) && ws, "select_mask: null args");
  MHIMX_CHECK_ARG(!g_rows_img || (g_rows_out && N <= 16384 && next_pow2((int)k < 2 ? 2 : (int)k) <= 4096),
                  "select_rows_img: the image-order list comes from the one-workgroup select (N <= 16384, k <= 4096)");
  MHIMX_CHECK_ARG(!g_rows_out || N <= 16384, "select_rows: fused row list needs N <= 16384 (use select_mask + compose_ids)");
  MHIMX_CHECK_ARG(N > 0 && N <= (1ll << 24), "select_mask: N out of range");
  MHIMX_CHECK_ARG(k >= 1 && k <= N && k <= 16384, "select_mask: k=%lld out of range (1..min(N,16384))", (long long)k);
  MHIMX_CHECK_ARG(n_sel >= 0 && n_sel <= k, "select_mask: n_sel out of range");
  MHIMX_CHECK_ARG(ws_bytes >= N, "select_mask: workspace too small");
  const int P = next_pow2((int)k < 2 ? 2 : (int)k);
  if (N <= 16384 && P <= 4096) {
    const size_t sm = select_small_smem(P);
#define MHIMX_SEL_SMALL(KPT)                                                                                                   \
    hipLaunchKernelGGL(select_small_kernel<KPT>, bgrid(1), dim3(SEL_THREADS), sm, (hipStream_t)stream, score, (int)N, (int)k,   \
                       (int)n_sel, largest, perm, other, n_other, mask_ids, len_keep_dev, topk_sorted, P, g_use_rand,          \
                       g_rand_seed, g_tick, g_merge_R, g_rows_out, g_rows_img, g_img_off, cur_batch())
    MHIMX_ONCE_PER_DEVICE(
        MHIMX_HIP(hipFuncSetAttribute((const void*)select_small_kernel<16>, hipFuncAttributeMaxDynamicSharedMemorySize, (int)select_small_smem(4096)));
        MHIMX_HIP(hipFuncSetAttribute((const void*)select_small_kernel<10>, hipFuncAttributeMaxDynamicSharedMemorySize, (int)select_small_smem(4096)));
        MHIMX_HIP(hipFuncSetAttribute((const void*)select_small_kernel<4>, hipFuncAttributeMaxDynamicSharedMemorySize, (int)select_small_smem(4096))));
    const bool lean = g_use_rand && g_rows_out && !perm && !other && !mask_ids && !len_keep_dev && !topk_sorted && n_sel < k;
    if (lean) {
#define MHIMX_SEL_LEAN(KPT)                                                                                                    \
      hipLaunchKernelGGL((select_small_kernel<KPT, true>), bgrid(1), dim3(SEL_THREADS), sm, (hipStream_t)stream, score, (int)N, (int)k,   \
                         (int)n_sel, largest, perm, other, n_other, mask_ids, len_keep_dev, topk_sorted, P, g_use_rand,        \
                         g_rand_seed, g_tick, g_merge_R, g_rows_out, g_rows_img, g_img_off, cur_batch())
      MHIMX_ONCE_PER_DEVICE(
          MHIMX_HIP(hipFuncSetAttribute((const void*)select_small_kernel<16, true>, hipFuncAttributeMaxDynamicSharedMemorySize, (int)select_small_smem(4096)));
          MHIMX_HIP(hipFuncSetAttribute((const void*)select_small_kernel<10, true>, hipFuncAttributeMaxDynamicSharedMemorySize, (int)select_small_smem(4096)));
          MHIMX_HIP(hipFuncSetAttribute((const void*)select_small_kernel<4, true>, hipFuncAttributeMaxDynamicSharedMemorySize, (int)select_small_smem(4096))));
      if (N <= 4096) MHIMX_SEL_LEAN(4);
      else if (N <= 10240) MHIMX_SEL_LEAN(10);
      else MHIMX_SEL_LEAN(16);
#undef MHIMX_SEL_LEAN
    } else if (N <= 4096) MHIMX_SEL_SMALL(4);
    else if (N <= 10240) MHIMX_SEL_SMALL(10);
    else MHIMX_SEL_SMALL(16);
#undef MHIMX_SEL_SMALL
    MHIMX_LAUNCH_CHECK();
    return 0;
  }
  MHIMX_CHECK_ARG(cur_batch().n == 0, "select: a bag-batched launch takes the one-workgroup select (N <= 16384, k <= 4096)");
  const size_t smem = select_smem(P);
    MHIMX_ONCE_PER_DEVICE(MHIMX_HIP(hipFuncSetAttribute((const void*)select_kernel<false>, hipFuncAttributeMaxDynamicSharedMemorySize, (int)select_smem(16384))); MHIMX_HIP(hipFuncSetAttribute((const void*)select_kernel<true>, hipFuncAttributeMaxDynamicSharedMemorySize, (int)select_smem(16384))));
  MHIMX_CHECK_ARG(!g_use_rand && !g_rows_out, "select: the random-subset forms need N <= 16384 and k <= 4096");
  if (N > 16384 && ws_bytes >= mhimx_select_ws_bytes(N) && mask_ids)
    return select_multi((hipStream_t)stream, score, N, (int)k, (int)n_sel, largest, perm, other, n_other, mask_ids, len_keep_dev, topk_sorted, ws, P);
  hipLaunchKernelGGL(select_kernel<false>, dim3(1), dim3(SEL_THREADS), smem, (hipStream_t)stream, score, N, (int)k, (int)n_sel,
                     largest, perm, other, n_other, mask_ids, len_keep_dev, topk_sorted, (uint8_t*)ws, (float*)nullptr, P);
  MHIMX_LAUNCH_CHECK();
  return 0;
}

extern "C" int mhimx_select_mask(void* stream, const float* score, int64_t N, int64_t k, int64_t n_sel, int32_t largest,
                                 const int64_t* perm, const int64_t* other, int64_t n_other, int64_t* mask_ids,
                                 int64_t* len_keep_dev, int64_t* topk_sorted, void* ws, int64_t ws_bytes) {
  return select_impl(stream, score, N, k, n_sel, largest, perm, other, n_other, mask_ids, len_keep_dev, topk_sorted, ws, ws_bytes,
                     0, 0, nullptr, 0, nullptr);
}

extern "C" int mhimx_select_rows(void* stream, const float* score, int64_t N, int64_t k, int64_t n_sel, int32_t largest,
                                 uint64_t rand_seed, const uint64_t* tick, int64_t merge_R, int64_t* rows_out, int64_t* mask_ids,
                                 void* ws, int64_t ws_bytes, int32_t merge_first) {
  MHIMX_CHECK_ARG(rows_out && merge_R >= 0 && merge_R <= N - n_sel, "select_rows: bad args");
  return select_impl(stream, score, N, k, n_sel, largest, nullptr, nullptr, 0, mask_ids, nullptr, nullptr, ws, ws_bytes,
                     merge_first ? 2 : 1, rand_seed, tick, (int)merge_R, rows_out);
}

extern "C" int mhimx_select_rows_img(void* stream, const float* score, int64_t N, int64_t k, int64_t n_sel, int32_t largest, uint64_t rand_seed,
                                     const uint64_t* tick, int64_t merge_R, int64_t* rows_out, int64_t* rows_img, int64_t img_merge_off, void* ws,
                                     int64_t ws_bytes, int32_t merge_first) {
  MHIMX_CHECK_ARG(rows_out && rows_img && merge_R >= 0 && merge_R <= N - n_sel && img_merge_off >= N - n_sel - merge_R && img_merge_off % 32 == 0 &&
                      img_merge_off <= 32768,
                  "select_rows_img: bad args (the merged rows' image position is a multiple of 32 behind the rows that stay)");
  return select_impl(stream, score, N, k, n_sel, largest, nullptr, nullptr, 0, nullptr, nullptr, nullptr, ws, ws_bytes, merge_first ? 2 : 1, rand_seed, tick,
                     (int)merge_R, rows_out, rows_img, (int)img_merge_off);
}

extern "C" int mhimx_vote_scores(void* stream, const float* attn, int64_t H, int64_t N, int64_t k, int32_t largest,
                                 float* vote, void* ws, int64_t ws_bytes) {
  (void)ws; (void)ws_bytes;
  MHIMX_CHECK_ARG(attn && vote && H > 0 && N > 0 && N <= (1ll << 24), "vote_scores: bad args");
  MHIMX_CHECK_ARG(k >= 1 && k <= N && k <= 16384, "vote_scores: k out of range");
  {
    const int64_t nb = (N * 4 / 16) * 16;
    if (aligned16(vote) && nb) sel_zero((hipStream_t)stream, vote, nb);
    if (!aligned16(vote) || nb != N * 4) MHIMX_HIP(hipMemsetAsync((char*)vote + (aligned16(vote) ? nb : 0), 0, (size_t)(N * 4 - (aligned16(vote) ? nb : 0)), (hipStream_t)stream));
  }
  const int P = next_pow2((int)k < 2 ? 2 : (int)k);
    MHIMX_ONCE_PER_DEVICE(MHIMX_HIP(hipFuncSetAttribute((const void*)select_kernel<true>, hipFuncAttributeMaxDynamicSharedMemorySize, (int)select_smem(16384))));
  hipLaunchKernelGGL(select_kernel<true>, dim3((unsigned)H), dim3(SEL_THREADS), select_smem(P), (hipStream_t)stream, attn, N, (int)k,
                     0, largest, (const int64_t*)nullptr, (const int64_t*)nullptr, (int64_t)0, (int64_t*)nullptr,
                     (int64_t*)nullptr, (int64_t*)nullptr, (uint8_t*)nullptr, vote, P);
  MHIMX_LAUNCH_CHECK();
  return 0;
}
```

### mhim_mil_amd/csrc/step.hip

```cpp
#include <math.h>
#include <string.h>

#include "infer_tab.hpp"
#include "step_mid.hpp"

namespace mhimx {

int64_t merge2_rows_tiles(int64_t R);

namespace {

struct DagEvents {
  hipEvent_t e[64][6];
  bool have[64] = {};
  int get(hipEvent_t** out) {
    int dev = 0;
    MHIMX_HIP(hipGetDevice(&dev));
    MHIMX_CHECK_ARG(dev >= 0 && dev < 64, "step: device index %d", dev);
    if (!have[dev]) {
      for (int i = 0; i < 6; ++i) MHIMX_HIP(hipEventCreateWithFlags(&e[dev][i], hipEventDisableTiming));
      have[dev] = true;
    }
    *out = e[dev];
    return 0;
  }
};
DagEvents g_dag_events;
constexpr int TP_RING = 256;
struct ProjTimes {
  hipEvent_t e[64][TP_RING][3];
  bool have[64] = {};
  int n[64] = {};
  int next(int* dev_out, hipEvent_t** pair) {
    int dev = 0;
    MHIMX_HIP(hipGetDevice(&dev));
    MHIMX_CHECK_ARG(dev >= 0 && dev < 64, "step: device index %d", dev);
    if (!have[dev]) {
      for (int i = 0; i < TP_RING; ++i)
        for (int j = 0; j < 3; ++j) MHIMX_HIP(hipEventCreate(&e[dev][i][j]));
      have[dev] = true;
    }
    *dev_out = dev;
    *pair = n[dev] < TP_RING ? e[dev][n[dev]] : nullptr;
    return 0;
  }
};
ProjTimes g_proj_times;
int dag_edge(hipEvent_t ev, hipStream_t from, hipStream_t to) {
  MHIMX_HIP(hipEventRecord(ev, from));
  MHIMX_HIP(hipStreamWaitEvent(to, ev, 0));
  return 0;
}

struct Carve {
  char* base;
  int64_t off = 0;
  explicit Carve(void* p) : base(static_cast<char*>(p)) {}
  int64_t take_off(int64_t bytes) {
    const int64_t o = off;
    off = (off + bytes + 255) / 256 * 256;
    return o;
  }
  template <typename T> T* at(int64_t o) const { return base ? reinterpret_cast<T*>(base + o) : nullptr; }
};

struct StepBufs {
  int64_t w1p_t, wa_frag_t, w1p_s, wa_frag_s, wa_t, wa_t_frag, wo_t, q_old, merge_ws, merge_ws_bytes;
  int64_t H_t, Hbuf, dact;
  int64_t s_t, stats_t, z_t, cproj_t, pscore, attn, pool_ws_t, pool_ws_t_bytes;
  int64_t rows_all, sel_ws, sel_ws_bytes, sel_perm, sel_ids, sel_rows, sel_lk;
  int64_t s_s, stats_s, z_s, pool_ws_s, pool_ws_s_bytes;
  int64_t logits, losses, g_z;
  int64_t dH, img, ws_b, ws_b_bytes, wg_ws, wg_ws_floats;
  int64_t q_scr, gslab;
  int64_t rows_img, P0, L_img;
  int64_t bag0, bag_stride;
  int64_t total;
};

int dpre_merge_rows(void* stream, const float* dH, const void* dact, const int64_t* rows_merge, int64_t R, int64_t E, char* img, int64_t P0, float* d_b1,
                    float* ws_b, int64_t ws_b_bytes, mhimx_reduce_list* lst) {
  const int64_t t0 = P0 / 32;
  const int n0 = lst->n;
  float* part_m = ws_b + t0 * E;
  if (int r = mhimx_rows_dpre_image(stream, dH, dact, rows_merge, R, E, img + t0 * (E / 128) * 16384, d_b1, 0, part_m, ws_b_bytes - t0 * E * 4, lst)) return r;
  MHIMX_CHECK_ARG(lst->n == n0 + 1 && lst->j[n0].kind == 0 && lst->j[n0].parts == part_m, "step: the bias gradient's partial sum was not queued");
  lst->j[n0].parts = ws_b;
  lst->j[n0].G += t0;
  return 0;
}

int check_cfg(const mhimx_step_cfg* c, int64_t N, const mhimx_step_counts* n) {
  MHIMX_CHECK_ARG(c && n, "step: null configuration / counts");
  MHIMX_CHECK_ARG(c->E == 512 && c->A == 128 && c->C >= 1 && c->C <= 4 && c->k >= 1 && 8 * c->k <= 48 && c->D > 0 && c->D % 256 == 0,
                  "step: shapes outside the single-pass ABMIL step (E = 512, A = 128, C <= 4, 8 k <= 48, D %% 256 == 0)");
  MHIMX_CHECK_ARG(N >= 64 && N <= MHIMX_STEP_MAX_ROWS && n->k_top >= 1 && n->k_top <= (N <= 16384 ? 4096 : 16384) && n->n_sel >= 1 && n->n_sel <= n->k_top &&
                      n->len_keep == N - n->n_sel && n->Lk >= 1 && n->R >= 1 && n->R <= 32768 && n->Lk + n->R == n->len_keep,
                  "step: row counts outside the device-drawn select (64 <= N <= %d, k_top <= 4096 up to 16384 rows / 16384 above, rows to merge "
                  "<= 32768, rows to merge and rows that stay >= 1)", MHIMX_STEP_MAX_ROWS);
  const mhimx_step_params &s = c->student, &t = c->teacher;
  MHIMX_CHECK_ARG(s.w1 && s.b1 && s.wa && s.wc && s.wp && s.bp && s.q && s.ln_w && s.ln_b && s.wkv && s.wq && s.wo && s.bo, "step: null student parameter");
  MHIMX_CHECK_ARG(t.w1 && t.b1 && t.wa && t.wc && (!c->attn2score || (t.wp && t.bp)), "step: null teacher parameter");
  const mhimx_step_grads& g = c->grad;
  MHIMX_CHECK_ARG(g.w1 && g.b1 && g.wa && g.wc && g.wp && g.bp && g.ln_w && g.ln_b && g.wkv && g.wq && g.wo && g.bo, "step: null gradient view");
  MHIMX_CHECK_ARG(c->tick, "step: the device dropout / draw counter (tick) is required");
  return 0;
}

void layout(const mhimx_step_cfg* c, int64_t N, const mhimx_step_counts* n, StepBufs* b, int n_bags = 1) {
  const int64_t D = c->D, E = c->E, A = c->A, C = c->C, k = c->k, I = 512;
  Carve cv(nullptr);
  const int64_t F = sizeof(float);
  b->w1p_t = cv.take_off(E * D * F);
  b->wa_frag_t = cv.take_off(A * E * F);
  b->w1p_s = cv.take_off(E * D * F);
  b->wa_frag_s = cv.take_off(A * E * F);
  b->wa_t = cv.take_off(E * A * F);
  b->wa_t_frag = cv.take_off(E * A * F);
  b->wo_t = cv.take_off(I * E * F);
  b->q_old = cv.take_off(k * E * F);
  if (n_bags > 1) {
    b->wg_ws_floats = mhimx_wgrad_multi_ws_floats(N <= 16384 ? (n->Lk + k + 31) / 32 * 32 + n->R : n->len_keep, E, D, n_bags);
    b->wg_ws = cv.take_off(b->wg_ws_floats * F);
  }
  b->bag0 = cv.off;
  b->merge_ws_bytes = mhimx_merge_ws_bytes(n->R, E, k, 8, 64);
  b->merge_ws = cv.take_off(b->merge_ws_bytes);
  const bool fuse_img = N <= 16384;
  b->P0 = fuse_img ? (n->Lk + k + 31) / 32 * 32 : 0;
  b->L_img = fuse_img ? b->P0 + n->R : n->len_keep;
  b->H_t = cv.take_off(N * E * F);
  b->Hbuf = cv.take_off((N + k) * E * F);
  b->dact = cv.take_off(N * E * 2);
  b->s_t = cv.take_off(N * F);
  b->stats_t = cv.take_off(2 * F);
  b->z_t = cv.take_off(E * F);
  b->cproj_t = cv.take_off(N * C * F);
  b->pscore = cv.take_off(N * F);
  b->attn = cv.take_off(N * F);
  b->pool_ws_t_bytes = mhimx_abmil_pool_ws_bytes(N, E, A, 0);
  b->pool_ws_t = cv.take_off(b->pool_ws_t_bytes);
  b->rows_all = cv.take_off((n->len_keep + k) * 8);
  b->sel_ws_bytes = mhimx_select_ws_bytes(N);
  b->sel_ws = cv.take_off(b->sel_ws_bytes);
  b->rows_img = fuse_img ? cv.take_off((b->L_img + 31) / 32 * 32 * 8) : 0;
  b->sel_perm = b->sel_ids = b->sel_rows = b->sel_lk = 0;
  if (N > 16384) {
    b->sel_perm = cv.take_off(n->k_top * 8);
    b->sel_ids = cv.take_off(N * 8);
    b->sel_rows = cv.take_off(n->len_keep * 8);
    b->sel_lk = cv.take_off(8);
  }
  const int64_t M = n->Lk + k;
  b->s_s = cv.take_off(M * F);
  b->stats_s = cv.take_off(2 * F);
  b->z_s = cv.take_off(E * F);
  b->pool_ws_s_bytes = mhimx_abmil_pool_ws_bytes(M, E, A, 0);
  b->pool_ws_s = cv.take_off(b->pool_ws_s_bytes);
  b->logits = cv.take_off(16 * F);
  b->losses = cv.take_off(4 * F);
  b->g_z = cv.take_off(E * F);
  b->dH = cv.take_off((N + k) * E * F);
  b->img = cv.take_off(mhimx_wgrad_image_bytes(b->L_img, E));
  b->ws_b_bytes = (fuse_img ? b->P0 / 32 + (n->R + 31) / 32 : (n->len_keep + 31) / 32) * E * F;
  b->ws_b = cv.take_off(b->ws_b_bytes);
  b->q_scr = b->gslab = 0;
  if (n_bags > 1) {
    b->q_scr = cv.take_off(k * E * F);
    b->gslab = cv.take_off(c->n_all * F);
  } else {
    b->wg_ws_floats = mhimx_wgrad_ws_floats(b->L_img, E, D);
    b->wg_ws = cv.take_off(b->wg_ws_floats * F);
  }
  b->bag_stride = cv.off - b->bag0;
  b->total = b->bag0 + (int64_t)n_bags * b->bag_stride;
}

}

int step_check_cfg(const mhimx_step_cfg* c, int64_t N, const mhimx_step_counts* n) { return check_cfg(c, N, n); }

mhimx_merge mid_merge_params(const mhimx_step_cfg& c) {
  const mhimx_step_params& S = c.student;
  mhimx_merge m = {};
  m.E = c.E; m.k = c.k; m.heads = 8; m.dim_head = 64;
  m.q_param = S.q; m.ln_w = S.ln_w; m.ln_b = S.ln_b; m.wkv = S.wkv; m.wq = S.wq; m.wo = S.wo; m.bo = S.bo;
  m.mm = c.merge_mm; m.prec = MHIMX_PREC_BF16X3; m.drop_tick = c.tick; m.rep = 1.f;
  return m;
}

int mid_prep_head(const mhimx_step_cfg& c, const MidImages& im, mhimx_prep_job* j) {
  int n = prep_counters(c, j);
  j[n++] = mhimx_prep_job{1, c.teacher.w1, im.w1p_t, c.E, c.D};
  j[n++] = mhimx_prep_job{4, c.teacher.wa, im.wa_frag_t, c.A, c.E};
  j[n++] = mhimx_prep_job{1, c.student.w1, im.w1p_s, c.E, c.D};
  return n;
}

int mid_prep_student(const mhimx_step_cfg& c, const MidImages& im, mhimx_prep_job* j) {
  const mhimx_step_params& S = c.student;
  j[0] = mhimx_prep_job{4, S.wa, im.wa_frag_s, c.A, c.E};
  j[1] = mhimx_prep_job{0, S.wa, im.wa_t, c.A, c.E};
  j[2] = mhimx_prep_job{5, S.wa, im.wa_t_frag, c.A, c.E};
  j[3] = mhimx_prep_job{0, S.wo, im.wo_t, c.E, 512};
  j[4] = mhimx_prep_job{2, S.q, im.q_old, 1, c.k * c.E};
  return 5;
}

mhimx_scorer mid_scorer(const mhimx_step_cfg& c, const mhimx_step_params& p, const float* wa_frag) {
  mhimx_scorer sc = {};
  sc.E = c.E; sc.A = c.A; sc.act = c.da_act; sc.prec = MHIMX_PREC_BF16X3; sc.wa = p.wa; sc.wc = p.wc; sc.wa_frag = wa_frag;
  return sc;
}

int mid_student_fwd(void* stream, const mhimx_step_cfg& c, const MidImages& im, const mhimx_merge& mw_prep, const MidBag& g, const MidDag* dag, MidFwd* f) {
  const int64_t E = c.E, k = c.k;
  mhimx_merge& mw = f->mw;
  mw = mw_prep;
  mw.drop_p = c.merge_drop_p; mw.drop_seed = g.mca_seed; mw.x_rows = g.rows_all; mw.prepared = 1;
  f->sc_s = mid_scorer(c, c.student, im.wa_frag_s);
  mhimx_pool_io& io = f->io_s;
  io = mhimx_pool_io{};
  io.T1 = g.Hbuf; io.M1 = g.Lk + k; io.s = g.s_s; io.stats = g.stats_s; io.z = g.z_s;
  io.ws = g.pool_ws; io.ws_bytes = g.pool_ws_bytes; io.rows1 = g.rows_all + g.R;
  io.tail_row0 = -1;
  io.phase = 1; io.tail_tokens = (int32_t)k;
  if (dag) {
    if (int r = dag_edge(dag->ev[0], dag->main_st, dag->side_st)) return r;
  } else {
    io.ride_merge = &mw; io.ride_X = g.Hbuf; io.ride_R = g.R; io.ride_ws = g.merge_ws; io.ride_ws_bytes = g.merge_ws_bytes;
  }
  if (int r = mhimx_abmil_pool_fwd(dag ? dag->side_st : stream, &f->sc_s, &io)) return r;
  mw.rows_done = io.rode_merge;
  if (int r = mhimx_merge_fwd(stream, &mw, g.Hbuf, g.R, g.Hbuf + g.N * E, g.q_out, 1, g.merge_ws, g.merge_ws_bytes)) return r;
  mw.rows_done = 0;
  if (dag)
    if (int r = dag_edge(dag->ev[1], dag->side_st, dag->main_st)) return r;
  io.phase = 2; io.tail_wa_t = im.wa_t; io.tail_row0 = g.N;
  if (int r = mhimx_abmil_pool_fwd(stream, &f->sc_s, &io)) return r;
  io.phase = 0; io.ride_merge = nullptr;
  return 0;
}

int mid_head(void* stream, const mhimx_step_cfg& c, const MidBag& g, const float* z_t, const int64_t* label, float loss_scale, float* logits,
             float* losses, const mhimx_step_grads& gr, int accumulate, const MidSurv* sv) {
  if (sv)
    return mhimx_head_surv_fwd_bwd(stream, g.z_s, c.aux_alpha != 0.f ? z_t : nullptr, c.student.wp, c.student.bp, label, sv->censor, c.E, c.C, c.temp_t,
                                   c.main_alpha, c.aux_alpha, loss_scale, sv->alpha, sv->eps, logits, losses, sv->risk, g.g_z, gr.wp, gr.bp, accumulate);
  return mhimx_head_fwd_bwd(stream, g.z_s, c.aux_alpha != 0.f ? z_t : nullptr, c.student.wp, c.student.bp, label, c.E, c.C, c.temp_t, c.main_alpha,
                            c.aux_alpha, loss_scale, logits, losses, g.g_z, gr.wp, gr.bp, accumulate, nullptr, nullptr);
}

int mid_bwd_rows(void* stream, const MidImages& im, const MidFwd& f, const MidBag& g, const mhimx_step_grads& gr, int accumulate, const MidImg* img,
                 const MidDag* dag, mhimx_reduce_list* lst) {
  const int64_t E = f.mw.E;
  float* d_tok = g.dH + g.N * E;
  mhimx_merge mwb = f.mw;
  mwb.q_param = im.q_old; mwb.wo_t = im.wo_t; mwb.prepared = 0;
  mhimx_merge_grad mg = {};
  mg.d_ln_w = gr.ln_w; mg.d_ln_b = gr.ln_b; mg.d_wkv = gr.wkv; mg.d_wq = gr.wq; mg.d_wo = gr.wo; mg.d_bo = gr.bo;
  mg.accumulate = accumulate; mg.splits = 8; mg.defer = lst;
  if (int r = mhimx_merge_bwd_park(&mwb, g.Hbuf, g.R, d_tok, g.dH, &mg, g.merge_ws, g.merge_ws_bytes)) return r;
  {
    mhimx_scorer sc_b = f.sc_s;
    sc_b.wa_frag = nullptr;
    mhimx_pool_grad pg = {};
    pg.g_z = g.g_z; pg.dT1 = g.dH; pg.d_wa = gr.wa; pg.d_wc = gr.wc; pg.wa_t = im.wa_t; pg.accumulate = accumulate; pg.splits = 8; pg.defer = lst;
    pg.wa_t_frag = im.wa_t_frag;
    if (img) { pg.img = img->img; pg.img_dact = img->dact; pg.img_part = img->part; pg.img_rows = g.Lk; }
    if (int r = mhimx_abmil_pool_bwd(stream, &sc_b, &f.io_s, &pg)) return r;
  }
  if (dag) {
    if (int r = dag_edge(dag->ev[2], dag->main_st, dag->side_st)) return r;
    if (lst->parked.pending && lst->pre.pending == 2) lst->parked.reserved = (int32_t)merge2_rows_tiles(g.R) + 1;
    if (int r = mhimx_reduce_flush(dag->side_st, lst)) return r;
  }
  if (int r = mhimx_merge_bwd(stream, &mwb, g.Hbuf, g.R, d_tok, g.dH, &mg, g.merge_ws, g.merge_ws_bytes)) return r;
  if (dag) {
    if (int r = dag_edge(dag->ev[3], dag->main_st, dag->side_st)) return r;
    if (int r = mhimx_reduce_flush(dag->side_st, lst)) return r;
  }
  return 0;
}

void q_chain_weights(double mm, int n, float* wq, float* w) {
// ... 59 lines not shown
    if (int r = g_dag_events.get(&dag_st.ev)) return r;

  const mhimx_merge mw_prep = mid_merge_params(c);
  {
    mhimx_prep_job early[8];
    int n = mid_prep_head(c, im, early);
    early[n++] = mhimx_prep_job{10, nullptr, reinterpret_cast<float*>(rows_all + len_keep), N, k};
    if (int r = mhimx_prep_batch(stream, early, n)) return r;
  }
  mhimx_prep_job late[6];
  mid_prep_student(c, im, late);
  late[5] = mhimx_prep_job{6, reinterpret_cast<const float*>(&mw_prep), static_cast<float*>(merge_ws), R, b.merge_ws_bytes};

  {
    mhimx_bag_project_args a = {};
    a.X = X; a.ldx = ldx; a.N = N; a.D = D; a.E = E; a.act = c.act; a.n_heads = 2; a.drop_tick = tick;
    a.head[0].wp = im.w1p_t; a.head[0].bias = T.b1; a.head[0].H = H_t; a.head[0].ldh = E; a.head[0].drop_p = c.drop_p_teacher; a.head[0].drop_seed = seeds->drop_teacher;
    a.head[1].wp = im.w1p_s; a.head[1].bias = S.b1; a.head[1].H = Hbuf; a.head[1].ldh = E; a.head[1].dact = dact; a.head[1].drop_p = c.drop_p_student;
    a.head[1].drop_seed = seeds->drop_student;
    hipEvent_t* tp = nullptr;
    int tp_dev = 0;
    if (c.time_project) {
      hipStreamCaptureStatus cs = hipStreamCaptureStatusNone;
      MHIMX_HIP(hipStreamIsCapturing(main_st, &cs));
      if (cs == hipStreamCaptureStatusNone)
        if (int r = g_proj_times.next(&tp_dev, &tp)) return r;
    }
    if (tp) MHIMX_HIP(hipEventRecord(tp[0], main_st));
    if (int r = mhimx_bag_project(stream, &a)) return r;
    if (tp) {
      MHIMX_HIP(hipEventRecord(tp[1], main_st));
      MHIMX_HIP(hipEventRecord(tp[2], main_st));
      ++g_proj_times.n[tp_dev];
    }
  }

  const mhimx_scorer sc_t = mid_scorer(c, T, im.wa_frag_t);
  const float* score = nullptr;
  {
    mhimx_pool_io io = {};
    io.T1 = H_t; io.M1 = N; io.s = cv.at<float>(b.s_t); io.stats = cv.at<float>(b.stats_t); io.z = cv.at<float>(b.z_t);
    io.ws = cv.at<char>(b.pool_ws_t); io.ws_bytes = b.pool_ws_t_bytes;
    if (c.attn2score) { io.wp = T.wp; io.C = C; io.cproj = cv.at<float>(b.cproj_t); io.bp = T.bp; io.pscore = cv.at<float>(b.pscore); }
    io.no_backward = 1;
    io.ride_jobs = late; io.n_ride_jobs = 6;
    if (int r = mhimx_abmil_pool_fwd(stream, &sc_t, &io)) return r;
    if (c.attn2score) score = io.pscore;
    else {
      if (int r = mhimx_softmax_from_stats(stream, io.s, io.stats, cv.at<float>(b.attn), N)) return r;
      score = cv.at<float>(b.attn);
    }
  }

  if (fuse_img) {
    if (int r = mhimx_select_rows_img(stream, score, N, cnt->k_top, cnt->n_sel, 1, seeds->select, tick, R, rows_all, cv.at<int64_t>(b.rows_img), b.P0,
                                      cv.at<char>(b.sel_ws), b.sel_ws_bytes, 1))
      return r;
  } else {
    const SelLargeWs lw = {cv.at<int64_t>(b.sel_perm), cv.at<int64_t>(b.sel_ids), cv.at<int64_t>(b.sel_rows), cv.at<int64_t>(b.sel_lk), cv.at<char>(b.sel_ws),
                           b.sel_ws_bytes};
    if (int r = select_large_rows(main_st, score, N, cnt->k_top, cnt->n_sel, seeds->select, tick, R, rows_all, 1, lw)) return r;
  }

  const MidBag bag = {Hbuf, dH, rows_all, N, R, Lk, seeds->mca, c.q_out ? c.q_out : S.q, cv.at<float>(b.s_s), cv.at<float>(b.stats_s), cv.at<float>(b.z_s),
                      cv.at<float>(b.g_z), cv.at<char>(b.pool_ws_s), b.pool_ws_s_bytes, merge_ws, b.merge_ws_bytes};
  MidFwd fwd;
  if (int r = mid_student_fwd(stream, c, im, mw_prep, bag, dag, &fwd)) return r;
  if (int r = mid_head(stream, c, bag, cv.at<float>(b.z_t), label_dev, 1.f, cv.at<float>(b.logits), cv.at<float>(b.losses), c.grad, 0)) return r;

  mhimx_reduce_list lst;
  memset(&lst, 0, sizeof(lst));
  const MidImg pimg = {cv.at<char>(b.img), dact, cv.at<float>(b.ws_b)};
  if (int r = mid_bwd_rows(stream, im, fwd, bag, c.grad, 0, fuse_img ? &pimg : nullptr, dag, &lst)) return r;
  mhimx_reduce_list lst_main;
  memset(&lst_main, 0, sizeof(lst_main));
  mhimx_reduce_list* lm = dag ? &lst_main : &lst;
  if (fuse_img) {
    if (int r = dpre_merge_rows(stream, dH, dact, rows_all, R, E, cv.at<char>(b.img), b.P0, c.grad.b1, cv.at<float>(b.ws_b), b.ws_b_bytes, lm)) return r;
  } else if (int r = mhimx_rows_dpre_image(stream, dH, dact, rows_all, len_keep, E, cv.at<char>(b.img), c.grad.b1, 0, cv.at<char>(b.ws_b), b.ws_b_bytes, lm))
    return r;
  {
    mhimx_bag_wgrad_args g = {};
    g.img = cv.at<char>(b.img); g.X = X; g.ldx = ldx; g.n_bag_rows = N; g.rows = fuse_img ? cv.at<int64_t>(b.rows_img) : rows_all; g.L = b.L_img; g.E = E; g.D = D;
    g.C = c.grad.w1; g.ldc = D;
    g.accumulate = 0; g.ws = cv.at<float>(b.wg_ws); g.ws_floats = b.wg_ws_floats; g.defer = lm; g.ride_tail = update ? 1 : 0;
    if (int r = mhimx_bag_wgrad(stream, &g)) return r;
  }
  if (dag)
    if (int r = dag_edge(dag->ev[4], dag->side_st, dag->main_st)) return r;
  if (!update) return mhimx_reduce_flush(stream, lm);

  mhimx_optim_args o = optim_args_of(c, host_step, true);
  o.fold = lm;
  return mhimx_optim_step(stream, &o);
}

namespace mhimx {
namespace {

struct QChainW { float wq; float w[MHIMX_WINDOW_MAX]; };
struct SlabGaps { int n; int64_t off[16], len[16]; };
__global__ __launch_bounds__(256) void window_q_chain_kernel(float* __restrict__ q, const float* __restrict__ z0, int64_t z_stride, int n_bags, int64_t n,
                                                             QChainW cw, float* __restrict__ slab0, int64_t pitch, SlabGaps gaps) {
  for (int64_t i = (int64_t)blockIdx.x * blockDim.x + threadIdx.x; i < n; i += (int64_t)gridDim.x * blockDim.x) {
    float acc = 0.f;
    for (int b = 0; b < n_bags; ++b) acc += z0[b * z_stride + i] * cw.w[b];
    q[i] = q[i] * cw.wq + acc;
  }
  for (int gi = 0; gi < gaps.n; ++gi)
    for (int b = 0; b < n_bags; ++b)
      for (int64_t i = (int64_t)blockIdx.x * blockDim.x + threadIdx.x; i < gaps.len[gi]; i += (int64_t)gridDim.x * blockDim.x)
        slab0[b * pitch + gaps.off[gi] + i] = 0.f;
}
__global__ __launch_bounds__(256) void window_sum_slabs_kernel(float* __restrict__ g, const float* __restrict__ slab0, int64_t pitch, int n_bags, int64_t n) {
  for (int64_t i = (int64_t)blockIdx.x * blockDim.x + threadIdx.x; i < n; i += (int64_t)gridDim.x * blockDim.x) {
    float acc = 0.f;
    for (int b = 0; b < n_bags; ++b) acc += slab0[b * pitch + i];
    g[i] = acc;
  }
}
// ... 359 lines not shown
```

### mhim_mil_amd/csrc/step_mid.hpp

```cpp
#pragma once
#include "common.hpp"

namespace mhimx {

struct MidImages { float *w1p_t, *wa_frag_t, *w1p_s, *wa_frag_s, *wa_t, *wa_t_frag, *wo_t, *q_old; };

struct MidBag {
  float *Hbuf, *dH;
  int64_t* rows_all;
  int64_t N, R, Lk;
  uint64_t mca_seed;
  float* q_out;
  float *s_s, *stats_s, *z_s, *g_z;
  void* pool_ws; int64_t pool_ws_bytes;
  void* merge_ws; int64_t merge_ws_bytes;
};
struct MidDag { hipStream_t main_st, side_st; hipEvent_t* ev; };
struct MidFwd { mhimx_merge mw; mhimx_scorer sc_s; mhimx_pool_io io_s; };
struct MidImg { void* img; const void* dact; float* part; };

mhimx_merge mid_merge_params(const mhimx_step_cfg& c);
int mid_prep_head(const mhimx_step_cfg& c, const MidImages& im, mhimx_prep_job* j);
int mid_prep_student(const mhimx_step_cfg& c, const MidImages& im, mhimx_prep_job* j);
mhimx_scorer mid_scorer(const mhimx_step_cfg& c, const mhimx_step_params& p, const float* wa_frag);
int mid_student_fwd(void* stream, const mhimx_step_cfg& c, const MidImages& im, const mhimx_merge& mw_prep, const MidBag& g, const MidDag* dag, MidFwd* f);
struct MidSurv { const float* censor; float alpha, eps; float* risk; };
int mid_head(void* stream, const mhimx_step_cfg& c, const MidBag& g, const float* z_t, const int64_t* label, float loss_scale, float* logits,
             float* losses, const mhimx_step_grads& gr, int accumulate, const MidSurv* sv = nullptr);
int mid_bwd_rows(void* stream, const MidImages& im, const MidFwd& f, const MidBag& g, const mhimx_step_grads& gr, int accumulate, const MidImg* img,
                 const MidDag* dag, mhimx_reduce_list* lst);
void q_chain_weights(double mm, int n, float* wq, float* w);

}
```

### mhim_mil_amd/engine.py

```python
from __future__ import annotations

from typing import Optional

import collections
import contextlib
import dataclasses
import os

import torch

from . import mhim as mh
from . import ops
from .mhim import MHIM, BagPlan


class CommonMIL:

    def __init__(self, args=None, fused=None, graph_cache=0) -> None:
        self.training = True
        self.fused = fused
        self.graph_cache = int(graph_cache)

    def _native_step(self, tr, bag, label, n_iter, extra):
        if self.graph_cache > 0 and not extra:
# ... 363 lines not shown
            if process_group is not None or (torch.distributed.is_available() and torch.distributed.is_initialized()
                                             and torch.distributed.get_world_size() > 1):
                raise mh.L.MhimxError("FusedTrainer(loss='nll_surv'): one process (world > 1 trains through CommonMIL.forward_func's autograd form)")
            if not (0.0 <= float(surv_alpha) <= 1.0 and 0.0 < float(surv_eps) < 1.0):
                raise mh.L.MhimxError(f"FusedTrainer(loss='nll_surv'): surv_alpha={surv_alpha} must be in [0, 1], surv_eps={surv_eps} in (0, 1)")
        self.loss, self.surv_alpha, self.surv_eps = loss, float(surv_alpha), float(surv_eps)
        if model == "mhim" and teacher is None:
            raise mh.L.MhimxError("FusedTrainer(model='mhim') needs the EMA teacher (modules/__init__.py:176-214 builds it)")
        if model == "mhim" and not student.merge_enable:
            raise mh.L.MhimxError("FusedTrainer(model='mhim') needs merge_enable=True: the reference's MHIM.forward rejects the Identity "
                                  "merge (mhim.py:82,351)")
        self.s, self.t = student, teacher
        self.flat = FlatState(student, teacher, step_merges=(model == "mhim"))
        self.lr, self.wd, self.betas, self.eps, self.mm = lr, weight_decay, betas, eps, mm
        self.main_alpha, self.aux_alpha = main_alpha, aux_alpha
        self.accum = max(1, int(accumulation_steps))
        self.pg = process_group
        self.comm = None
        self.world = torch.distributed.get_world_size(process_group) if self._dist() else 1
        self.model_kind = model
        self._chain, self._chain_tokens, self._q_scratch = None, None, None
        if (self.world > 1 and self.accum == 1 and model == "mhim" and student.merge_enable and student.baseline == "attn"
                and "merge.global_q_mm" in self.flat.offsets):
            rank = torch.distributed.get_rank(process_group)
            self._chain = QueryChain(self.flat.offsets["merge.global_q_mm"], student.merge.global_q_mm.numel(), float(student.merge.g_q_mm),
                                     self.world, rank)
        self._micro = 0
        self.last = {}
        dev = self.flat.student.device
        self.tick = torch.zeros(1, dtype=torch.int64, device=dev)
        self.opt_step = torch.zeros(1, dtype=torch.int64, device=dev)
        self._defer = ops.ReduceList()
        self.overlap_comm = True
        self._work_a = None
        self._capturing = False
        fo = self.flat.offsets
        self._split = fo["feature.0.bias"] + (student.feature[0].bias.numel() + 3) // 4 * 4 if "feature.0.bias" in fo else 0
        if not (self.flat.names[:2] == ["feature.0.weight", "feature.0.bias"]):
            self._split = 0
        student._tick = self.tick
        if teacher is not None:
            teacher._tick = self.tick
        self.mm_table = None if mm_sche is None else torch.as_tensor(mm_sche, dtype=torch.float32).to(dev).contiguous()
        self.clip_grad = None if clip_grad is None else float(clip_grad)
        self.lr_table = None if lr_sche is None else torch.as_tensor(lr_sche, dtype=torch.float32).to(dev).contiguous()
        self._clip_ws = torch.empty(1024, device=dev) if self.clip_grad else None
        self._g_extra = None
        self._fold_now, self._fold_list = False, None
        self._graph_pool = None
        self._cap_stream = None
        self._side = None
        self.step_dag = os.environ.get("MHIMX_STEP_DAG", "0") != "0"
        self.use_executor = os.environ.get("MHIMX_STEP_EXEC", "1") != "0"
        self._exec, self.time_project = None, False
        self.exec_max_rows = 262144
        self.single_pass = True
        self.window_streams = 4
        self.window_batched = _WINDOW_BATCHED
        self._win, self._win_w, self._shape_graphs = None, {}, None
        self._rows_cache = {}
        self.pure_window_row_cap = 262144
        self.ragged_window_row_cap = 262144
        self.dsmil_window_row_cap = 131072
        self._dsmil_exec = None
        self.dsmil_mhim_window_row_cap = 131072
        self._dsmil_mhim_exec = None

    def _dist(self):
        return torch.distributed.is_available() and torch.distributed.is_initialized()

    @contextlib.contextmanager
    def _merge_off_if_pure(self):
        s, merge_on = self.s, self.s.merge_enable
        if self.model_kind != "mhim":
            s.merge_enable = False
        try:
            yield
        finally:
            s.merge_enable = merge_on

    def _head(self, z, teacher_feat, label, gv, accumulate):
        s = self.s
        t_in = teacher_feat.view(-1) if (teacher_feat is not None and self.aux_alpha != 0.) else None
        logits, losses, g_z, _, _ = (self._surv_head if self.loss == "nll_surv" else ops.head_fwd_bwd)(
            z, t_in, s.predictor.weight.data, s.predictor.bias.data, label, temp_t=float(s.temp_t),
            main_alpha=self.main_alpha, aux_alpha=self.aux_alpha, inv_accum=1.0 / self.accum,
            d_wp=gv["predictor.weight"], d_bp=gv["predictor.bias"], accumulate=accumulate)
        return logits, losses, g_z

    def _overlap_hook(self, first):
        return self._mid_hook if (first and self.overlap_comm and self.comm is None and self.world > 1 and self.accum == 1
                                  and not self._capturing and self._split > 0) else None

    def forward_backward(self, bag, label, perm=None, ids_shuffle=None, i=None):
        x = self.s._check_x(bag)
        if self.loss == "nll_surv":
            label = self._surv_label(label, x.device)
        r = self._step_route(x, label, i, perm, ids_shuffle)
        if r.fam is not None:
            out = self._run_native(r.fam, [x], r.labels, i, bool(self._fold_now), surv=r.surv, single=True)
            return out[0][0], out[1][0]
        if r.name == "exec":
            return self._exec_step(x, label, i)
        return (self._forward_backward_nat if r.name == "nat" else self._forward_backward_py)(x, label, perm, ids_shuffle, i)

    def _step_route(self, x, label, i, perm, ids_shuffle, executor=True):
# ... 394 lines not shown

    def _exec_cfg(self):
        s, t, fl = self.s, self.t, self.flat
        L = mh.L
        ex = self._exec
        mhim = self.model_kind == "mhim"
        key = (s.feature[0].weight.data_ptr(), t.feature[0].weight.data_ptr() if mhim else 0, fl.grad.data_ptr())
        if ex is None or ex["key"] != key:
            P = lambda tns: tns.data_ptr()
            def params(m, with_merge):
                att = m.online_encoder.attention
                pr = L.StepParams(w1=P(m.feature[0].weight), b1=P(m.feature[0].bias), wa=P(att.attention[0].weight), wc=P(att.attention[2].weight),
                                  wp=P(m.predictor.weight), bp=P(m.predictor.bias))
                if with_merge:
                    mg = m.merge
                    pr.q, pr.ln_w, pr.ln_b = P(mg.global_q_mm), P(mg.norm.weight), P(mg.norm.bias)
                    pr.wkv, pr.wq, pr.wo, pr.bo = P(mg.attn.to_kv.weight), P(mg.attn.to_q.weight), P(mg.attn.to_out[0].weight), P(mg.attn.to_out[0].bias)
                return pr
            gv = fl.grad_views
            pre = "online_encoder.attention.attention."
            grads = L.StepGrads(w1=P(gv["feature.0.weight"]), b1=P(gv["feature.0.bias"]), wa=P(gv[pre + "0.weight"]), wc=P(gv[pre + "2.weight"]),
                                wp=P(gv["predictor.weight"]), bp=P(gv["predictor.bias"]))
            if mhim:
                grads.ln_w, grads.ln_b = P(gv["merge.norm.weight"]), P(gv["merge.norm.bias"])
                grads.wkv, grads.wq = P(gv["merge.attn.to_kv.weight"]), P(gv["merge.attn.to_q.weight"])
                grads.wo, grads.bo = P(gv["merge.attn.to_out.0.weight"]), P(gv["merge.attn.to_out.0.bias"])
            cfg = L.StepCfg(D=s.input_dim, E=s.mlp_dim, A=s.online_encoder.attention.attention[0].weight.shape[0], C=s.n_classes,
                            k=s.merge.k if mhim else 0,
                            act=L.act_code(s.act, mh._FEATURE_ACTS), da_act=L.act_code(s.da_act, mh._SCORER_ACTS),
                            student=params(s, mhim), teacher=params(t, False) if mhim else L.StepParams(), grad=grads,
                            p=P(fl.student), g=P(fl.grad), m=P(fl.m), v=P(fl.v), n_train=fl.n_train, n_all=fl.n_all,
                            tick=P(self.tick), opt_step=P(self.opt_step))
            ex = self._exec = {"key": key, "cfg": cfg, "layouts": {}, "ws": None}
        cfg = ex["cfg"]
        cfg.lr, cfg.beta1, cfg.beta2, cfg.eps, cfg.weight_decay, cfg.ema_mm = self.lr, self.betas[0], self.betas[1], self.eps, self.wd, self.mm
        cfg.lr_table, cfg.lr_len = (None, 0) if self.lr_table is None else (self.lr_table.data_ptr(), self.lr_table.numel())
        cfg.drop_p_student = float(s.dropout_p)
        cfg.main_alpha = float(self.main_alpha)
        if not mhim:
            return ex
        if self.step_dag:
            if self._side is None or self._side.device != fl.student.device:
                self._side = torch.cuda.Stream(device=fl.student.device)
            cfg.side_stream = self._side.cuda_stream
        else:
            cfg.side_stream = None
        if self._chain is not None:
            if self._q_scratch is None:
                self._q_scratch = torch.empty((s.merge.k, s.mlp_dim), device=fl.student.device)
            cfg.q_out = self._q_scratch.data_ptr()
        else:
            cfg.q_out = None
        cfg.time_project = int(bool(self.time_project))
        cfg.attn2score = int(bool(t.attn2score))
        cfg.drop_p_teacher = float(t.dropout_p if t.training else 0.0)
        cfg.merge_drop_p, cfg.merge_mm = float(s.merge.dropout), float(s.merge.g_q_mm)
        cfg.temp_t, cfg.aux_alpha = float(s.temp_t), float(self.aux_alpha)
        cfg.p_teacher = None if fl.same_teacher else fl.teacher.data_ptr()
        cfg.mm_table, cfg.mm_len = (None, 0) if self.mm_table is None else (self.mm_table.data_ptr(), self.mm_table.numel())
        return ex

    def _exec_window_ok(self, xs, labels, i=None):
        n = len(xs)
        if not (self.window_batched and 2 <= n <= _L.WINDOW_MAX and self.world == 1 and self._chain is None and not self.step_dag
                and self.flat.n_all % 4 == 0 and self.s.merge.k <= 6 and self.s.mrh_sche is None and self.flat.names[0] == "feature.0.weight"):
            return False
        x0 = xs[0]
        if not (x0.dim() == 2 and x0.shape[0] <= 16384 and all(x.shape == x0.shape and x.stride() == x0.stride() and x.device == x0.device for x in xs)):
            return False
        if not ops.window_labels_ok(labels, x0.device):
            return False
        return all(self._exec_ok(x, i, window=True) for x in xs)

    def _exec_window(self, xs, labels, i, update):
        L = mh.L
        s, t, fl = self.s, self.t, self.flat
        n = len(xs)
        ex = self._exec_cfg()
        N = xs[0].shape[0]
        k, n_sel, len_keep, Lk, R = s.v2_counts(N, i)
        key = ("window", n, N, k, n_sel, Lk)
        ent = ex["layouts"].get(key)
        if ent is None:
            cnt = L.StepCounts(k_top=k, n_sel=n_sel, len_keep=len_keep, Lk=Lk, R=R)
            ent = ex["layouts"][key] = (cnt, ops.window_layout(ex["cfg"], n, N, cnt))
        cnt, lay = ent
        ws = ops.workspace(ex, "ws_win", lay.total, xs[0].device, slack=1.0)
        seeds = (L.StepSeeds * n)()
        for j in range(n):
            seeds[j].drop_teacher, seeds[j].drop_student = t._next_seed(teacher=True), s._next_seed()
        for j in range(n):
            seeds[j].select, seeds[j].mca = s._next_seed(), s._next_seed()
        inside = bool(update and not self.clip_grad)
        ops.window_run(ex["cfg"], xs, labels, cnt, seeds, fl.step + int(inside), ws, inside)
        bg = lay.bag
        per = []
        for j in range(n):
            base = j * lay.bag_stride
            per.append(self._last_full(ws, bg, N, cnt, ops.ws_view(ws, base + bg.logits, s.n_classes), ops.ws_view(ws, base + bg.losses, 3), base=base))
        logits, losses = [p["logits"] for p in per], [p["losses"] for p in per]
        self.last = dict(per[-1], logits=logits, losses=losses, bags=per, ws=ws, exec="mhimx_window_run")
        self._window_done(n, inside, update)
        return logits, losses

    @staticmethod
    def ragged_window_shapes_ok(bags, D, k, E=512, A=128, C=2, max_rows=262144, row_cap=524288, max_bags=32, elem=4):
# ... 622 lines not shown
```

### mhim_mil_amd/ops.py

```python
from __future__ import annotations

import collections
import ctypes as C
import functools
import itertools
import math
from typing import Optional

import torch

from . import _lib as L


KERNEL_EVENT_HOOK = None


import threading

_PIN = threading.local()


def _pinned():
    st = getattr(_PIN, "stream", None)
    if st is not None and getattr(_PIN, "device", -1) == torch.cuda.current_device():
# ... 248 lines not shown
    if splits > 1:
        nslab = max(nslab, min(64, -(-512 // max(1, (K1 // 128) * (K2 // 128)))), -(-M // 4096))
    ws = torch.empty((nslab, K1, K2), device=a.device, dtype=torch.float32) if nslab > 1 else None
    g = L.GemmTN(A=_p(a), lda=a.stride(0), B=_p(b), ldb=b.stride(0), rows=_p(rows), C=_p(out), ldc=out.stride(0), M=M,
                 K1=K1, K2=K2, splits=int(splits), ws=_p(ws), accumulate=int(bool(accumulate)), prec=prec_code(prec),
                 ws_floats=0 if ws is None else ws.numel(), defer=_dp(defer))
    L.check(L.lib().mhimx_gemm_tn(_stream(), C.byref(g)), "mhimx_gemm_tn")
    if defer is not None:
        defer.keep.append(ws)
    return out


def transpose(x, out=None):
    _chk(x, name="x")
    R, Cc = x.shape
    if out is None:
        out = torch.empty((Cc, R), device=x.device, dtype=torch.float32)
    L.check(L.lib().mhimx_transpose(_stream(), _p(x), _p(out), R, Cc), "mhimx_transpose")
    return out


class ScorerW:

    def __init__(self, wa, wc, act, ba=None, wb=None, bb=None, bc=None, prec="bf16x3", wa_frag=None, gate_drop_p=0.0, gate_drop_seed=0):
        self.t = (wa, wc, ba, wb, bb, bc, wa_frag)
        for t in self.t:
            _chk(t, name="scorer weight")
        self.A, self.E = wa.shape
        self.gated = wb is not None
        self.c = L.Scorer(E=self.E, A=self.A, act=int(act), gated=int(self.gated), prec=prec_code(prec), wa=_p(wa),
                          ba=_p(ba), wb=_p(wb), bb=_p(bb), wc=_p(wc), bc=_p(bc), wa_frag=_p(wa_frag),
                          gate_drop_p=float(gate_drop_p), gate_drop_seed=int(gate_drop_seed) & 0xFFFFFFFFFFFFFFFF)


class PoolState:

    def __init__(self, T1, T2, C_classes=0, wp=None, device=None, bp=None, rows1=None, excl=None):
        dev = T1.device
        M1 = T1.shape[0] if rows1 is None else rows1.shape[0]
        self.rows1 = rows1
        self.excl = excl
        M2 = 0 if T2 is None else T2.shape[0]
        self.T1, self.T2, self.M1, self.M2 = T1, T2, M1, M2
        M = M1 + M2
        self.s = torch.empty(M, device=dev)
        self.stats = torch.empty(2, device=dev)
        self.z = torch.empty(T1.shape[1], device=dev)
        self.cproj = torch.empty((M, C_classes), device=dev) if wp is not None else None
        self.wp = wp
        self.bp = bp
        self.pscore = torch.empty(M1, device=dev) if (wp is not None and bp is not None) else None
        self.ws = None
        self.ride = None

    def io(self, sc: ScorerW):
        M = self.M1 + self.M2
        nbytes = L.lib().mhimx_abmil_pool_ws_bytes(M, sc.E, sc.A, int(sc.gated))
        if self.ws is None or self.ws.numel() < nbytes:
            self.ws = torch.empty(nbytes, device=self.T1.device, dtype=torch.uint8)
        return L.PoolIO(T1=_p(self.T1), M1=self.M1, T2=_p(self.T2), M2=self.M2, s=_p(self.s), stats=_p(self.stats),
                        z=_p(self.z), u_pre=None, wp=_p(self.wp), C=0 if self.cproj is None else self.cproj.shape[1],
                        cproj=_p(self.cproj), ws=_p(self.ws), ws_bytes=self.ws.numel(), bp=_p(self.bp), pscore=_p(self.pscore),
                        rows1=_p(self.rows1), excl=_p(self.excl),
                        ride_jobs=None if self.ride is None else C.cast(self.ride[0], C.c_void_p), n_ride_jobs=0 if self.ride is None else self.ride[1])


def abmil_pool_fwd_split(sc: ScorerW, T1, rows1, tail_tokens, ride_merge=None):
    _chk(T1, name="T1"); _chk(rows1, torch.int64, "rows1")
    st = PoolState(T1, None, 0, None, rows1=rows1)
    st.tail_tokens = int(tail_tokens)
    io = st.io(sc)
    io.phase, io.tail_tokens = 1, st.tail_tokens
    if ride_merge is not None:
        mw, X, ws = ride_merge
        io.ride_merge, io.ride_X = C.cast(C.pointer(mw.c), C.c_void_p), _p(X)
        io.ride_R, io.ride_ws, io.ride_ws_bytes = mw.x_rows.shape[0], _p(ws), ws.numel()
    L.check(L.lib().mhimx_abmil_pool_fwd(_stream(), C.byref(sc.c), C.byref(io)), "mhimx_abmil_pool_fwd (phase 1)")
    return st, bool(io.rode_merge)


def abmil_pool_fwd_finish(sc: ScorerW, st: PoolState, wa_t=None, tail_row0=-1):
    io = st.io(sc)
    io.phase, io.tail_tokens = 2, st.tail_tokens
    io.tail_wa_t, io.tail_row0 = _p(wa_t), int(tail_row0)
    L.check(L.lib().mhimx_abmil_pool_fwd(_stream(), C.byref(sc.c), C.byref(io)), "mhimx_abmil_pool_fwd (phase 2)")
    return st


def abmil_pool_fwd(sc: ScorerW, T1, T2=None, wp=None, bp=None, rows1=None, excl=None, ride_jobs=None, no_backward=False):
    _chk(T1, name="T1"); _chk(T2, name="T2"); _chk(wp, name="wp"); _chk(bp, name="bp"); _chk(rows1, torch.int64, "rows1")
    _chk(excl, torch.uint8, "excl")
    st = PoolState(T1, T2, 0 if wp is None else wp.shape[0], wp, bp=bp, rows1=rows1, excl=excl)
    if ride_jobs:
        st.ride = (_prep_array(ride_jobs), len(ride_jobs))
    io = st.io(sc)
    io.no_backward = int(bool(no_backward))
    L.check(L.lib().mhimx_abmil_pool_fwd(_stream(), C.byref(sc.c), C.byref(io)), "mhimx_abmil_pool_fwd")
    st.ride = None
    return st


def abmil_pool_bwd(sc: ScorerW, st: PoolState, g_z, wa_t, wb_t=None, need_bias=False, splits=8, grads=None,
                   accumulate=False, defer=None, wa_t_frag=None, img=None, img_dact=None, img_part=None, img_rows=0):
    dev = g_z.device
    E, A = sc.E, sc.A
    out = grads or {}
    out.setdefault("dT1", torch.empty((st.M1, E), device=dev))
    if st.M2:
        out.setdefault("dT2", torch.empty((st.M2, E), device=dev))
    out.setdefault("d_wa", torch.empty((A, E), device=dev))
    out.setdefault("d_wc", torch.empty((1, A), device=dev))
    if sc.gated:
        out.setdefault("d_wb", torch.empty((A, E), device=dev))
    if need_bias:
        out.setdefault("d_ba", torch.empty(A, device=dev))
        out.setdefault("d_bc", torch.empty(1, device=dev))
        if sc.gated:
            out.setdefault("d_bb", torch.empty(A, device=dev))
    io = st.io(sc)
    g = L.PoolGrad(g_z=_p(g_z), dT1=_p(out["dT1"]), dT2=_p(out.get("dT2")), d_wa=_p(out["d_wa"]), d_ba=_p(out.get("d_ba")),
                   d_wb=_p(out.get("d_wb")), d_bb=_p(out.get("d_bb")), d_wc=_p(out["d_wc"]), d_bc=_p(out.get("d_bc")),
                   wa_t=_p(wa_t), wb_t=_p(wb_t), accumulate=int(bool(accumulate)), splits=int(splits), defer=_dp(defer),
                   wa_t_frag=_p(wa_t_frag), img=_p(img), img_dact=_p(img_dact), img_part=_p(img_part), img_rows=int(img_rows))
    if defer is not None:
        defer.keep.append(st)
    L.check(L.lib().mhimx_abmil_pool_bwd(_stream(), C.byref(sc.c), C.byref(io), C.byref(g)), "mhimx_abmil_pool_bwd")
    return out


def softmax_from_stats(s, stats):
    out = torch.empty_like(s)
    L.check(L.lib().mhimx_softmax_from_stats(_stream(), _p(s), _p(stats), _p(out), s.numel()), "mhimx_softmax_from_stats")
    return out


def pseudo_score(s, stats, cproj, bp, want_attn=False):
    M = cproj.shape[0] if s is None else s.numel()
    score = torch.empty(M, device=cproj.device)
    attn = torch.empty_like(s) if want_attn else None
    L.check(L.lib().mhimx_pseudo_score(_stream(), _p(s), _p(stats), _p(cproj), _p(bp), _p(score), _p(attn), M,
                                       cproj.shape[1]), "mhimx_pseudo_score")
    return (score, attn) if want_attn else score


def lse_merge(parts):
    _chk(parts, name="parts")
    W, E = parts.shape[0], parts.shape[1] - 2
    stats, z = torch.empty(2, device=parts.device), torch.empty(E, device=parts.device)
    L.check(L.lib().mhimx_lse_merge(_stream(), _p(parts), W, E, _p(stats), _p(z)), "mhimx_lse_merge")
    return stats, z


def select_mask(score, k, n_sel, largest=True, perm=None, other=None, want_topk=False):
    _chk(score, name="score"); _chk(perm, torch.int64, "perm"); _chk(other, torch.int64, "other")
    N = score.numel()
    dev = score.device
    mask_ids = torch.empty(N, device=dev, dtype=torch.int64)
    len_keep = torch.empty(1, device=dev, dtype=torch.int64)
    topk = torch.empty(k, device=dev, dtype=torch.int64) if want_topk else None
    ws = torch.empty(L.lib().mhimx_select_ws_bytes(N), device=dev, dtype=torch.uint8)
    L.check(L.lib().mhimx_select_mask(_stream(), _p(score), N, int(k), int(n_sel), int(bool(largest)), _p(perm), _p(other),
                                      0 if other is None else other.numel(), _p(mask_ids), _p(len_keep), _p(topk), _p(ws),
                                      ws.numel()), "mhimx_select_mask")
    return mask_ids, len_keep, topk


def select_rows(score, k, n_sel, merge_R, rand_seed, tick=None, largest=True, want_mask_ids=False, merge_first=False, out=None):
    _chk(score, name="score")
    N = score.numel()
    dev = score.device
    rows = out if out is not None else torch.empty(N - n_sel, device=dev, dtype=torch.int64)
    _chk(rows, torch.int64, "rows out")
    mask_ids = torch.empty(N, device=dev, dtype=torch.int64) if want_mask_ids else None
    ws = torch.empty(L.lib().mhimx_select_ws_bytes(N), device=dev, dtype=torch.uint8)
    L.check(L.lib().mhimx_select_rows(_stream(), _p(score), N, int(k), int(n_sel), int(bool(largest)),
                                      int(rand_seed) & 0xFFFFFFFFFFFFFFFF, _p(tick), int(merge_R), _p(rows), _p(mask_ids), _p(ws),
                                      ws.numel(), int(bool(merge_first))), "mhimx_select_rows")
    return (rows, mask_ids) if want_mask_ids else rows


def select_rows_img(score, k, n_sel, merge_R, rand_seed, img_merge_off, tick=None, largest=True, merge_first=True):
    _chk(score, name="score")
    N = score.numel()
    dev = score.device
    rows = torch.empty(N - n_sel, device=dev, dtype=torch.int64)
    rows_img = torch.empty(-(-(int(img_merge_off) + int(merge_R)) // 32) * 32, device=dev, dtype=torch.int64)
    ws = torch.empty(L.lib().mhimx_select_ws_bytes(N), device=dev, dtype=torch.uint8)
    L.check(L.lib().mhimx_select_rows_img(_stream(), _p(score), N, int(k), int(n_sel), int(bool(largest)), int(rand_seed) & 0xFFFFFFFFFFFFFFFF,
                                          _p(tick), int(merge_R), _p(rows), _p(rows_img), int(img_merge_off), _p(ws), ws.numel(),
                                          int(bool(merge_first))), "mhimx_select_rows_img")
    return rows, rows_img


def vote_scores(attn, k, largest=True):
    _chk(attn, name="attn")
    H, N = attn.shape
    vote = torch.empty(N, device=attn.device)
    L.check(L.lib().mhimx_vote_scores(_stream(), _p(attn), H, N, int(k), int(bool(largest)), _p(vote), None, 0),
            "mhimx_vote_scores")
    return vote


def random_perm(n, seed, tick=None, src=None, out=None, device=None):
    _chk(src, torch.int64, "src"); _chk(out, torch.int64, "out")
    dev = device if device is not None else (src.device if src is not None else (out.device if out is not None else torch.device("cuda")))
    if out is None:
        out = torch.empty(int(n), dtype=torch.int64, device=dev)
    L.check(L.lib().mhimx_random_perm(_stream(), int(n), int(seed) & 0xFFFFFFFFFFFFFFFF, _p(tick), _p(src), _p(out)), "mhimx_random_perm")
    return out


def compose_ids(a, b):
    _chk(a, torch.int64, "a"); _chk(b, torch.int64, "b")
    out = torch.empty_like(b)
    L.check(L.lib().mhimx_compose_ids(_stream(), _p(a), _p(b), _p(out), b.numel()), "mhimx_compose_ids")
    return out


class MergeW:
    def __init__(self, q_param, ln_w, ln_b, wkv, wq, wo, bo, mm, heads=8, dim_head=64, drop_p=0.0, drop_seed=0,
                 prec="bf16x3", transposes=None, drop_tick=None, wkv_frag=None, x_rows=None, prepared=False, own=None, rep=1.0):
        self.t = [q_param, ln_w, ln_b, wkv, wq, wo, bo, wkv_frag]
        _chk(x_rows, torch.int64, "x_rows")
        self.x_rows = x_rows
        for t in self.t:
            _chk(t, name="merge weight")
        self.k, self.E = q_param.shape[-2], q_param.shape[-1]
        self.heads, self.dim_head = heads, dim_head
        self.tr = transposes or (None, None, None)
        self.c = L.Merge(E=self.E, k=self.k, heads=heads, dim_head=dim_head, q_param=_p(q_param), ln_w=_p(ln_w),
                         ln_b=_p(ln_b), wkv=_p(wkv), wq=_p(wq), wo=_p(wo), bo=_p(bo), wkv_t=_p(self.tr[0]),
                         wq_t=_p(self.tr[1]), wo_t=_p(self.tr[2]), mm=float(mm), drop_p=float(drop_p),
                         drop_seed=int(drop_seed) & 0xFFFFFFFFFFFFFFFF, prec=prec_code(prec), drop_tick=_p(drop_tick),
                         wkv_frag=_p(wkv_frag), x_rows=_p(x_rows), prepared=int(bool(prepared)),
                         own_lo=0 if own is None else int(own[0]), own_n=0 if own is None else int(own[1]), rep=float(rep))
        self.own = own

    def ws_for(self, R, device):
        n = L.lib().mhimx_merge_ws_bytes(R, self.E, self.k, self.heads, self.dim_head)
        return torch.empty(n, device=device, dtype=torch.uint8)


def merge_fwd(mw: MergeW, X, z_out=None, update_q=True, ws=None, q_out=None, rows_done=False):
    _chk(X, name="X")
# ... 840 lines not shown
```

Measured before the change: 33.01 million patch-instances/s.

## Precompute student scorer rows inside the select kernel and gather them in pooling

New measurement: 32.78 million patch-instances/s. Within noise of the previous version (-0.7%).

```diff
diff --git a/include/mhimx.h b/include/mhimx.h
--- a/include/mhimx.h
+++ b/include/mhimx.h
@@ -157,6 +157,7 @@
 } mhimx_pool_io;
 int64_t mhimx_abmil_pool_ws_bytes(int64_t M, int64_t E, int64_t A, int32_t gated);
 int mhimx_abmil_pool_fwd(void* stream, const mhimx_scorer* sc, mhimx_pool_io* io);
+int mhimx_abmil_pool_fwd_pre(void* stream, const mhimx_scorer* sc, mhimx_pool_io* io, const float* pre_u, const float* pre_s);
 
 typedef struct {
   const float* g_z;
@@ -250,6 +251,14 @@
 int mhimx_select_rows_img(void* stream, const float* score, int64_t N, int64_t k, int64_t n_sel, int32_t largest, uint64_t rand_seed,
                           const uint64_t* tick, int64_t merge_R, int64_t* rows_out, int64_t* rows_img, int64_t img_merge_off, void* ws,
                           int64_t ws_bytes, int32_t merge_first);
+typedef struct {
+  const float* T; int64_t N;
+  const mhimx_scorer* sc;
+  float* u_src; float* s_src;
+} mhimx_pre_rows;
+int mhimx_select_rows_pre(void* stream, const float* score, int64_t N, int64_t k, int64_t n_sel, int32_t largest, uint64_t rand_seed,
+                          const uint64_t* tick, int64_t merge_R, int64_t* rows_out, int64_t* rows_img, int64_t img_merge_off, void* ws,
+                          int64_t ws_bytes, int32_t merge_first, const mhimx_pre_rows* pre);
 int mhimx_vote_scores(void* stream, const float* attn, int64_t H, int64_t N, int64_t k, int32_t largest,
                       float* vote, void* ws, int64_t ws_bytes);
 
@@ -397,6 +406,7 @@
   uint64_t* tick; uint64_t* opt_step;
   float* q_out;
   int32_t time_project;
+  int32_t no_pre_select;
   void* side_stream;
 } mhimx_step_cfg;
 typedef struct { int64_t k_top, n_sel, len_keep, Lk, R; } mhimx_step_counts;
diff --git a/mhim_mil_amd/_lib.py b/mhim_mil_amd/_lib.py
--- a/mhim_mil_amd/_lib.py
+++ b/mhim_mil_amd/_lib.py
@@ -114,6 +114,10 @@
                 ("no_backward", C.c_int32)]
 
 
+class PreRows(C.Structure):
+    _fields_ = [("T", c_f32p), ("N", C.c_int64), ("sc", C.c_void_p), ("u_src", c_f32p), ("s_src", c_f32p)]
+
+
 class PoolGrad(C.Structure):
     _fields_ = [("g_z", c_f32p), ("dT1", c_f32p), ("dT2", c_f32p),
                 ("d_wa", c_f32p), ("d_ba", c_f32p), ("d_wb", c_f32p), ("d_bb", c_f32p), ("d_wc", c_f32p),
@@ -184,7 +188,7 @@
                 ("n_train", C.c_int64), ("n_all", C.c_int64),
                 ("lr", C.c_float), ("beta1", C.c_float), ("beta2", C.c_float), ("eps", C.c_float), ("weight_decay", C.c_float), ("ema_mm", C.c_float),
                 ("mm_table", C.c_void_p), ("mm_len", C.c_int64), ("lr_table", C.c_void_p), ("lr_len", C.c_int64),
-                ("tick", C.c_void_p), ("opt_step", C.c_void_p), ("q_out", C.c_void_p), ("time_project", C.c_int32), ("side_stream", C.c_void_p)]
+                ("tick", C.c_void_p), ("opt_step", C.c_void_p), ("q_out", C.c_void_p), ("time_project", C.c_int32), ("no_pre_select", C.c_int32), ("side_stream", C.c_void_p)]
 
 
 class StepCounts(C.Structure):
@@ -373,6 +377,8 @@
     "mhimx_select_mask": (C.c_int, [_P, _P, _I64, _I64, _I64, _I32, _P, _P, _I64, _P, _P, _P, _P, _I64]),
     "mhimx_select_rows": (C.c_int, [_P, _P, _I64, _I64, _I64, _I32, _U64, _P, _I64, _P, _P, _P, _I64, _I32]),
     "mhimx_select_rows_img": (C.c_int, [_P, _P, _I64, _I64, _I64, _I32, _U64, _P, _I64, _P, _P, _I64, _P, _I64, _I32]),
+    "mhimx_select_rows_pre": (C.c_int, [_P, _P, _I64, _I64, _I64, _I32, _U64, _P, _I64, _P, _P, _I64, _P, _I64, _I32, _P]),
+    "mhimx_abmil_pool_fwd_pre": (C.c_int, [_P, C.POINTER(Scorer), C.POINTER(PoolIO), _P, _P]),
     "mhimx_vote_scores": (C.c_int, [_P, _P, _I64, _I64, _I64, _I32, _P, _P, _I64]),
     "mhimx_compose_ids": (C.c_int, [_P, _P, _P, _P, _I64]),
     "mhimx_random_perm": (C.c_int, [_P, _I64, _U64, _P, _P, _P]),
diff --git a/mhim_mil_amd/csrc/pre_rows.hpp b/mhim_mil_amd/csrc/pre_rows.hpp
--- /dev/null
+++ b/mhim_mil_amd/csrc/pre_rows.hpp
@@ -0,0 +1,130 @@
+#pragma once
+#include "common.hpp"
+
+namespace mhimx {
+
+typedef float sf_f32x16 __attribute__((ext_vector_type(16)));
+typedef float sf_f4 __attribute__((ext_vector_type(4)));
+typedef __bf16 sf_b8 __attribute__((ext_vector_type(8)));
+
+constexpr int SF_ROWS = 32, SF_E = 512, SF_A = 128, SF_LD = SF_E + 4, SF_THREADS = 256;
+
+MHIMX_DEV void sf_split(const sf_f4& a, const sf_f4& b, sf_b8& hi, sf_b8& lo) {
+  const float x[8] = {a[0], a[1], a[2], a[3], b[0], b[1], b[2], b[3]};
+#pragma unroll
+  for (int i = 0; i < 8; ++i) {
+    const __bf16 h = (__bf16)x[i];
+    hi[i] = h;
+    lo[i] = (__bf16)(x[i] - (float)h);
+  }
+}
+
+MHIMX_DEV float sf_sum32(float v) {
+  v += dpp_mov<0xB1, 0xf>(0.f, v);
+  v += dpp_mov<0x4E, 0xf>(0.f, v);
+  v += dpp_mov<0x141, 0xf>(0.f, v);
+  v += dpp_mov<0x140, 0xf>(0.f, v);
+  v += dpp_mov<0x142, 0xa>(0.f, v);
+  return v;
+}
+
+struct PreRows {
+  const float* T;
+  const float *wa_frag, *ba, *wc, *bc;
+  float* u_src;
+  float* s_src;
+  int N, act, tiles;
+};
+
+typedef __bf16 sf_b4 __attribute__((ext_vector_type(4)));
+constexpr int PR_ROWS = 64, PR_THREADS = 1024, PR_RING = 6;
+constexpr int PR_PITCH = 2 * SF_E * 2 + 16;
+constexpr size_t PR_SMEM = (size_t)PR_ROWS * PR_PITCH + 4 * PR_ROWS * sizeof(float);
+
+MHIMX_DEV void pre_rows_tile(const PreRows& p, const int tile, float* sm) {
+  char* Hb = reinterpret_cast<char*>(sm);
+  float* sred = reinterpret_cast<float*>(Hb + PR_ROWS * PR_PITCH);
+  const int tid = threadIdx.x, lane = tid & 63;
+  const int wave = __builtin_amdgcn_readfirstlane(tid >> 6);
+  const int row0 = tile * PR_ROWS;
+  const int r32 = lane & 31, kg = lane >> 5;
+  const int rh = (wave >> 2) & 1, cg = wave & 3;
+  const int n_col = 32 * cg + r32;
+  if (wave >= 8) {
+    const int lt = tid - 512, lr = lt >> 5, lc = lt & 31;
+    sf_f4 av[16];
+#pragma unroll
+    for (int j = 0; j < 16; ++j) {
+      const int n = row0 + lr + 16 * (j & 3);
+      av[j] = *reinterpret_cast<const sf_f4*>(p.T + (int64_t)(n < p.N ? n : p.N - 1) * SF_E + 128 * (j >> 2) + 4 * lc);
+    }
+#pragma unroll
+    for (int c = 0; c < 4; ++c) {
+#pragma unroll
+      for (int q = 0; q < 4; ++q) {
+        sf_b4 hi, lo;
+#pragma unroll
+        for (int i = 0; i < 4; ++i) {
+          const float x = av[4 * c + q][i];
+          const __bf16 h = (__bf16)x;
+          hi[i] = h;
+          lo[i] = (__bf16)(x - (float)h);
+        }
+        char* dst = Hb + (lr + 16 * q) * PR_PITCH + (128 * c + 4 * lc) * 2;
+        *reinterpret_cast<sf_b4*>(dst) = hi;
+        *reinterpret_cast<sf_b4*>(dst + SF_E * 2) = lo;
+      }
+      __syncthreads();
+    }
+  } else {
+    const float bn = p.ba ? p.ba[n_col] : 0.f, wn = p.wc[n_col];
+    const float* fptr = p.wa_frag + ((int64_t)cg * (SF_E / 16) * 64 + lane) * 8;
+    const char* aptr = Hb + (32 * rh + r32) * PR_PITCH + 16 * kg;
+    sf_f32x16 acc, acc2, acc3;
+#pragma unroll
+    for (int i = 0; i < 16; ++i) { acc[i] = 0.f; acc2[i] = 0.f; acc3[i] = 0.f; }
+    sf_f4 bh_[PR_RING], bl_[PR_RING];
+#pragma unroll
+    for (int ks = 0; ks < PR_RING; ++ks) {
+      bh_[ks] = *reinterpret_cast<const sf_f4*>(fptr + ks * 512);
+      bl_[ks] = *reinterpret_cast<const sf_f4*>(fptr + ks * 512 + 4);
+    }
+#pragma unroll
+    for (int c = 0; c < 4; ++c) {
+      __syncthreads();
+#pragma unroll
+      for (int ks = 8 * c; ks < 8 * c + 8; ++ks) {
+        const sf_b8 bh = __builtin_bit_cast(sf_b8, bh_[ks % PR_RING]), bl = __builtin_bit_cast(sf_b8, bl_[ks % PR_RING]);
+        if (ks + PR_RING < SF_E / 16) {
+          bh_[ks % PR_RING] = *reinterpret_cast<const sf_f4*>(fptr + (ks + PR_RING) * 512);
+          bl_[ks % PR_RING] = *reinterpret_cast<const sf_f4*>(fptr + (ks + PR_RING) * 512 + 4);
+        }
+        __builtin_amdgcn_sched_barrier(0);
+        const sf_b8 ah = *reinterpret_cast<const sf_b8*>(aptr + 32 * ks), al = *reinterpret_cast<const sf_b8*>(aptr + SF_E * 2 + 32 * ks);
+        acc2 = __builtin_amdgcn_mfma_f32_32x32x16_bf16(al, bh, acc2, 0, 0, 0);
+        acc = __builtin_amdgcn_mfma_f32_32x32x16_bf16(ah, bh, acc, 0, 0, 0);
+        acc3 = __builtin_amdgcn_mfma_f32_32x32x16_bf16(ah, bl, acc3, 0, 0, 0);
+      }
+    }
+#pragma unroll
+    for (int i = 0; i < 16; ++i) acc[i] += acc2[i] + acc3[i];
+#pragma unroll
+    for (int i = 0; i < 16; ++i) {
+      const int row = 32 * rh + 8 * (i >> 2) + 4 * kg + (i & 3);
+      const int n = row0 + row;
+      const float u = acc[i] + bn;
+      if (n < p.N) p.u_src[(int64_t)n * SF_A + n_col] = u;
+      const float v = sf_sum32(wn * act_fwd(u, p.act));
+      if (r32 == 31) sred[cg * PR_ROWS + row] = v;
+    }
+  }
+  __syncthreads();
+  if (tid < PR_ROWS) {
+    const int n = row0 + tid;
+    const float bias_c = p.bc ? p.bc[0] : 0.f;
+    const float s = (sred[tid] + sred[PR_ROWS + tid]) + (sred[2 * PR_ROWS + tid] + sred[3 * PR_ROWS + tid]) + bias_c;
+    if (n < p.N) p.s_src[n] = s;
+  }
+}
+
+}
diff --git a/mhim_mil_amd/csrc/rows.hip b/mhim_mil_amd/csrc/rows.hip
--- a/mhim_mil_amd/csrc/rows.hip
+++ b/mhim_mil_amd/csrc/rows.hip
@@ -12,7 +12,7 @@
 int scorer_fused_fwd(hipStream_t st, const float* T, int64_t M, const float* wa, const float* wa_frag, const float* ba, int act, const float* wc,
                      const float* bc, const float* wp, int C, float* u_pre, float* s_out, float* cproj, float* pm, float* pl,
                      float* pz, int max_parts, const int64_t* rows, const uint8_t* excl, const mhimx_prep_job* ride_jobs, int n_ride_jobs,
-                     const void* merge_rows);
+                     const void* merge_rows, const float* pre_u = nullptr, const float* pre_s = nullptr);
 int merge2_fwd_rows_args(const mhimx_merge* m, const float* X, int64_t R, void* ws, int64_t ws_bytes, M2RowsFwd* out);
 int prep_batch(hipStream_t st, const mhimx_prep_job* jobs, int n);
 int scorer_fused_bwd(hipStream_t st, const float* T, int64_t M, const float* u_pre, const float* s_in, const float* stats,
@@ -889,7 +889,7 @@
   return 0;
 }
 
-int abmil_pool_fwd(hipStream_t st, const mhimx_scorer* sc, mhimx_pool_io* io) {
+int abmil_pool_fwd(hipStream_t st, const mhimx_scorer* sc, mhimx_pool_io* io, const float* pre_u = nullptr, const float* pre_s = nullptr) {
   if (int r = check_scorer(sc)) return r;
   MHIMX_CHECK_ARG(io && io->T1 && io->M1 > 0 && io->s && io->stats && io->z, "pool_fwd: null io");
   MHIMX_CHECK_ARG(io->M2 == 0 || io->T2, "pool_fwd: M2>0 needs T2");
@@ -898,6 +898,10 @@
                   "pool_fwd: gathered tokens (rows1) need the one-pass scorer (E = 512, A = 128, plain form, not f32) and a single segment");
   MHIMX_CHECK_ARG(!io->excl || scorer_fused_ok(sc->E, sc->A, sc->gated, sc->prec, io->T1, sc->wa, io->cproj ? io->wp : nullptr, io->C),
                   "pool_fwd: excluded rows (excl) need the one-pass scorer (E = 512, A = 128, plain form, not f32)");
+  MHIMX_CHECK_ARG(!pre_u == !pre_s && (!pre_u || (io->M2 == 0 && !io->cproj && cur_batch().n == 0 &&
+                                               scorer_fused_ok(sc->E, sc->A, sc->gated, sc->prec, io->T1, sc->wa, nullptr, 0))),
+                  "pool_fwd_pre: precomputed rows need pre_u and pre_s, the one-pass scorer (E = 512, A = 128, plain form, not f32), a single segment, "
+                  "no class projections and one bag");
   const int64_t M = io->M1 + io->M2, E = sc->E, A = sc->A;
   const int gated = sc->gated ? 1 : 0;
   Arena ar(io->ws, io->ws_bytes);
@@ -924,7 +928,7 @@
         if (rc == 0) { mf = &mfbuf; io->rode_merge = 1; }
       }
       const int g1 = scorer_fused_fwd(st, io->T1, Ms1, sc->wa, sc->wa_frag, sc->ba, sc->act, sc->wc, sc->bc, nullptr, 0, u_pre, io->s, nullptr, w.pm, w.pl,
-                                      w.pz, MAX_PART, io->rows1, nullptr, io->ride_jobs, io->n_ride_jobs, mf);
+                                      w.pz, MAX_PART, io->rows1, nullptr, io->ride_jobs, io->n_ride_jobs, mf, pre_u, pre_s);
       return g1 < 0 ? g1 : 0;
     }
     hipLaunchKernelGGL(pool_finalize_tok_kernel, bgrid((unsigned)cdiv(E, 64)), dim3(FIN_THREADS), 0, st, w.pm, w.pl, w.pz, G1, (int)E, io->stats, io->z, io->T1,
@@ -945,7 +949,7 @@
       const int g1 = scorer_fused_fwd(st, Ts[seg], Ms[seg], sc->wa, sc->wa_frag, sc->ba, sc->act, sc->wc, sc->bc, io->cproj ? io->wp : nullptr,
                                       (int)io->C, io->no_backward ? nullptr : u_pre + off * ldu, io->s + off, io->cproj ? io->cproj + off * io->C : nullptr,
                                       w.pm + G, w.pl + G, w.pz + (int64_t)G * E, MAX_PART, seg == 0 ? io->rows1 : nullptr,
-                                      seg == 0 ? io->excl : nullptr, rode ? nullptr : io->ride_jobs, rode ? 0 : io->n_ride_jobs, nullptr);
+                                      seg == 0 ? io->excl : nullptr, rode ? nullptr : io->ride_jobs, rode ? 0 : io->n_ride_jobs, nullptr, pre_u, pre_s);
       if (g1 < 0) return g1;
       rode = true;
       G += g1;
@@ -1255,6 +1259,10 @@
 extern "C" int mhimx_abmil_pool_fwd(void* stream, const mhimx_scorer* sc, mhimx_pool_io* io) {
   return abmil_pool_fwd((hipStream_t)stream, sc, io);
 }
+extern "C" int mhimx_abmil_pool_fwd_pre(void* stream, const mhimx_scorer* sc, mhimx_pool_io* io, const float* pre_u, const float* pre_s) {
+  MHIMX_CHECK_ARG(pre_u && pre_s, "pool_fwd_pre: null pre_u / pre_s");
+  return abmil_pool_fwd((hipStream_t)stream, sc, io, pre_u, pre_s);
+}
 extern "C" int mhimx_abmil_pool_bwd(void* stream, const mhimx_scorer* sc, const mhimx_pool_io* io, const mhimx_pool_grad* g) {
   return abmil_pool_bwd((hipStream_t)stream, sc, io, g);
 }
diff --git a/mhim_mil_amd/csrc/scorer_fused.hip b/mhim_mil_amd/csrc/scorer_fused.hip
--- a/mhim_mil_amd/csrc/scorer_fused.hip
+++ b/mhim_mil_amd/csrc/scorer_fused.hip
@@ -2,13 +2,10 @@
 
 #include "common.hpp"
 #include "mca2_rows.hpp"
+#include "pre_rows.hpp"
 #include "prep_jobs.hpp"
 
 namespace mhimx {
-
-typedef float sf_f32x16 __attribute__((ext_vector_type(16)));
-typedef float sf_f4 __attribute__((ext_vector_type(4)));
-typedef __bf16 sf_b8 __attribute__((ext_vector_type(8)));
 
 #ifdef MHIMX_SF_PROF
 __device__ unsigned long long sf_prof[16];
@@ -17,30 +14,10 @@
 #define SF_STAMP(i)
 #endif
 
-constexpr int SF_ROWS = 32, SF_E = 512, SF_A = 128, SF_LD = SF_E + 4, SF_THREADS = 256;
 constexpr int SF_MAXC = 4;
 constexpr size_t SF_SMEM = (size_t)(SF_ROWS * SF_LD + 4 * SF_ROWS + 2 * SF_ROWS + SF_MAXC * SF_E + 2 * SF_ROWS) * sizeof(float);
 
-MHIMX_DEV void sf_split(const sf_f4& a, const sf_f4& b, sf_b8& hi, sf_b8& lo) {
-  const float x[8] = {a[0], a[1], a[2], a[3], b[0], b[1], b[2], b[3]};
-#pragma unroll
-  for (int i = 0; i < 8; ++i) {
-    const __bf16 h = (__bf16)x[i];
-    hi[i] = h;
-    lo[i] = (__bf16)(x[i] - (float)h);
-  }
-}
-
-MHIMX_DEV float sf_sum32(float v) {
-  v += dpp_mov<0xB1, 0xf>(0.f, v);
-  v += dpp_mov<0x4E, 0xf>(0.f, v);
-  v += dpp_mov<0x141, 0xf>(0.f, v);
-  v += dpp_mov<0x140, 0xf>(0.f, v);
-  v += dpp_mov<0x142, 0xa>(0.f, v);
-  return v;
-}
-
-template <bool FRAG>
+template <bool FRAG, bool PRE = false>
 __global__ __launch_bounds__(SF_THREADS, 2) void scorer_fused_kernel(
     const float* __restrict__ T, int64_t M, const float* __restrict__ wa, const float* __restrict__ wa_frag,
     const float* __restrict__ ba, int act,
@@ -50,7 +27,8 @@
     const uint8_t* __restrict__ excl ,
     int n_main , PrepJobs rider,
     int n_front ,
-    M2RowsFwd mf, BagBatch bb ) {
+    M2RowsFwd mf, BagBatch bb ,
+    const float* __restrict__ pre_u , const float* __restrict__ pre_s ) {
   extern __shared__ __attribute__((aligned(16))) float sf_sm[];
   if (blockIdx.z) {
     MHIMX_BAG(T); MHIMX_BAG(u_pre); MHIMX_BAG(s_out); MHIMX_BAG(cproj); MHIMX_BAG(pm); MHIMX_BAG(pl); MHIMX_BAG(pz); MHIMX_BAG(rows); MHIMX_BAG(excl);
@@ -89,6 +67,36 @@
   for (int tile = bid; tile < tiles; tile += n_main) {
     const int64_t row0 = (int64_t)tile * SF_ROWS;
     SF_STAMP(0);
+    if constexpr (PRE) {
+    if (tid < SF_ROWS) {
+      const int64_t n = row0 + tid, nc = n < M ? n : M - 1;
+      ridx[tid] = rows ? rows[nc] : nc;
+    }
+    __syncthreads();
+#pragma unroll
+    for (int i = 0; i < 16; ++i) {
+      const int f = tid + SF_THREADS * i, r = f >> 7, c4 = f & 127;
+      sf_f4 v = reinterpret_cast<const sf_f4*>(T + ridx[r] * SF_E)[c4];
+      if (row0 + r >= M) v = sf_f4{0.f, 0.f, 0.f, 0.f};
+      *reinterpret_cast<sf_f4*>(Hs + r * SF_LD + 4 * c4) = v;
+    }
+    if (tid < SF_ROWS) {
+      const int64_t n = row0 + tid;
+      float s = pre_s[ridx[tid]];
+      if (n >= M || (excl && excl[ridx[tid]])) s = -INFINITY;
+      if (n < M) s_out[n] = s;
+      srow[tid] = s;
+    }
+    if (u_pre) {
+#pragma unroll
+      for (int q = 0; q < 4; ++q) {
+        const int f = tid + SF_THREADS * q, r = f >> 5, c4 = f & 31;
+        const int64_t n = row0 + r;
+        if (n < M) reinterpret_cast<sf_f4*>(u_pre + n * SF_A)[c4] = reinterpret_cast<const sf_f4*>(pre_u + ridx[r] * SF_A)[c4];
+      }
+    }
+    __syncthreads();
+    } else {
     sf_f32x16 acc, acc2, acc3;
     if constexpr (FRAG) {
     if (rows) {
@@ -218,6 +226,7 @@
       srow[tid] = s;
     }
     __syncthreads();
+    }
     SF_STAMP(3);
     float mt = -INFINITY;
 #pragma unroll
@@ -647,9 +656,11 @@
 int scorer_fused_fwd(hipStream_t st, const float* T, int64_t M, const float* wa, const float* wa_frag, const float* ba, int act, const float* wc,
                      const float* bc, const float* wp, int C, float* u_pre, float* s_out, float* cproj, float* pm, float* pl,
                      float* pz, int max_parts, const int64_t* rows, const uint8_t* excl, const mhimx_prep_job* ride_jobs, int n_ride_jobs,
-                     const void* merge_rows ) {
+                     const void* merge_rows ,
+                     const float* pre_u, const float* pre_s ) {
   MHIMX_ONCE_PER_DEVICE(MHIMX_HIP(hipFuncSetAttribute((const void*)scorer_fused_kernel<true>, hipFuncAttributeMaxDynamicSharedMemorySize, (int)SF_SMEM)));
   MHIMX_ONCE_PER_DEVICE(MHIMX_HIP(hipFuncSetAttribute((const void*)scorer_fused_kernel<false>, hipFuncAttributeMaxDynamicSharedMemorySize, (int)SF_SMEM)));
+  MHIMX_ONCE_PER_DEVICE(MHIMX_HIP(hipFuncSetAttribute((const void*)scorer_fused_kernel<true, true>, hipFuncAttributeMaxDynamicSharedMemorySize, (int)SF_SMEM)));
   const int tiles = (int)cdiv(M, SF_ROWS);
   const int grid = tiles < max_parts ? tiles : max_parts;
   static_assert(SF_SMEM >= PREP_LDS_FLOATS * sizeof(float), "the riders' LDS is the scorer's");
@@ -668,12 +679,16 @@
     mf = *reinterpret_cast<const M2RowsFwd*>(merge_rows);
     n_front = mf.w.T;
   }
-  if (wa_frag)
+  MHIMX_CHECK_ARG(!pre_u == !pre_s && (!pre_u || (aligned16(pre_u) && (!u_pre || aligned16(u_pre)))), "scorer: precomputed rows need both pre_u and pre_s, 16-byte aligned");
+  if (pre_u)
+    hipLaunchKernelGGL((scorer_fused_kernel<true, true>), bgrid(n_front + grid + ride_blocks), dim3(SF_THREADS), SF_SMEM, st, T, M, wa, wa_frag, ba, act, wc, bc, wp, C,
+                       u_pre, s_out, cproj, pm, pl, pz, tiles, rows, excl, grid, rider, n_front, mf, cur_batch(), pre_u, pre_s);
+  else if (wa_frag)
     hipLaunchKernelGGL(scorer_fused_kernel<true>, bgrid(n_front + grid + ride_blocks), dim3(SF_THREADS), SF_SMEM, st, T, M, wa, wa_frag, ba, act, wc, bc, wp, C, u_pre,
-                       s_out, cproj, pm, pl, pz, tiles, rows, excl, grid, rider, n_front, mf, cur_batch());
+                       s_out, cproj, pm, pl, pz, tiles, rows, excl, grid, rider, n_front, mf, cur_batch(), pre_u, pre_s);
   else
     hipLaunchKernelGGL(scorer_fused_kernel<false>, bgrid(n_front + grid + ride_blocks), dim3(SF_THREADS), SF_SMEM, st, T, M, wa, wa_frag, ba, act, wc, bc, wp, C, u_pre,
-                       s_out, cproj, pm, pl, pz, tiles, rows, excl, grid, rider, n_front, mf, cur_batch());
+                       s_out, cproj, pm, pl, pz, tiles, rows, excl, grid, rider, n_front, mf, cur_batch(), pre_u, pre_s);
   MHIMX_LAUNCH_CHECK();
   return grid;
 }
diff --git a/mhim_mil_amd/csrc/select.hip b/mhim_mil_amd/csrc/select.hip
--- a/mhim_mil_amd/csrc/select.hip
+++ b/mhim_mil_amd/csrc/select.hip
@@ -1,3 +1,4 @@
+#include "pre_rows.hpp"
 #include "select_dev.hpp"
 
 namespace mhimx {
@@ -182,8 +183,15 @@
     int64_t* __restrict__ topk_out, int P, int use_rand, uint64_t rand_seed0, const uint64_t* __restrict__ tick, int merge_R,
     int64_t* __restrict__ rows_out,
     int64_t* __restrict__ rows_img ,
-    int img_off, BagBatch bb ) {
+    int img_off, BagBatch bb ,
+    PreRows pre ) {
   extern __shared__ __attribute__((aligned(16))) char smem_raw[];
+  if constexpr (LEAN) {
+    if (blockIdx.x >= 1) {
+      pre_rows_tile(pre, (int)blockIdx.x - 1, reinterpret_cast<float*>(smem_raw));
+      return;
+    }
+  }
   if (blockIdx.z) {
     MHIMX_BAG(score); MHIMX_BAG(perm); MHIMX_BAG(other); MHIMX_BAG(mask_ids); MHIMX_BAG(len_keep_dev); MHIMX_BAG(topk_out); MHIMX_BAG(rows_out);
     MHIMX_BAG(rows_img);
@@ -649,7 +657,7 @@
                        const int64_t* perm, const int64_t* other, int64_t n_other, int64_t* mask_ids,
                        int64_t* len_keep_dev, int64_t* topk_sorted, void* ws, int64_t ws_bytes, int g_use_rand,
                        uint64_t g_rand_seed, const uint64_t* g_tick, int g_merge_R, int64_t* g_rows_out, int64_t* g_rows_img = nullptr,
-                       int g_img_off = 0) {
+                       int g_img_off = 0, const PreRows* pre = nullptr) {
   MHIMX_CHECK_ARG(score && (mask_ids || g_rows_out) && ws, "select_mask: null args");
   MHIMX_CHECK_ARG(!g_rows_img || (g_rows_out && N <= 16384 && next_pow2((int)k < 2 ? 2 : (int)k) <= 4096),
                   "select_rows_img: the image-order list comes from the one-workgroup select (N <= 16384, k <= 4096)");
@@ -664,21 +672,25 @@
 #define MHIMX_SEL_SMALL(KPT)                                                                                                   \
     hipLaunchKernelGGL(select_small_kernel<KPT>, bgrid(1), dim3(SEL_THREADS), sm, (hipStream_t)stream, score, (int)N, (int)k,   \
                        (int)n_sel, largest, perm, other, n_other, mask_ids, len_keep_dev, topk_sorted, P, g_use_rand,          \
-                       g_rand_seed, g_tick, g_merge_R, g_rows_out, g_rows_img, g_img_off, cur_batch())
+                       g_rand_seed, g_tick, g_merge_R, g_rows_out, g_rows_img, g_img_off, cur_batch(), PreRows{})
     MHIMX_ONCE_PER_DEVICE(
         MHIMX_HIP(hipFuncSetAttribute((const void*)select_small_kernel<16>, hipFuncAttributeMaxDynamicSharedMemorySize, (int)select_small_smem(4096)));
         MHIMX_HIP(hipFuncSetAttribute((const void*)select_small_kernel<10>, hipFuncAttributeMaxDynamicSharedMemorySize, (int)select_small_smem(4096)));
         MHIMX_HIP(hipFuncSetAttribute((const void*)select_small_kernel<4>, hipFuncAttributeMaxDynamicSharedMemorySize, (int)select_small_smem(4096))));
     const bool lean = g_use_rand && g_rows_out && !perm && !other && !mask_ids && !len_keep_dev && !topk_sorted && n_sel < k;
+    MHIMX_CHECK_ARG(!(pre && pre->tiles > 0) || (lean && cur_batch().n == 0),
+                    "select_rows_pre: the row pass rides in the lean one-workgroup select of one bag (device-drawn subsets, no mask-id list)");
     if (lean) {
+      const PreRows pr = pre ? *pre : PreRows{};
+      const size_t sml = pr.tiles > 0 && PR_SMEM > sm ? PR_SMEM : sm;
 #define MHIMX_SEL_LEAN(KPT)                                                                                                    \
-      hipLaunchKernelGGL((select_small_kernel<KPT, true>), bgrid(1), dim3(SEL_THREADS), sm, (hipStream_t)stream, score, (int)N, (int)k,   \
+      hipLaunchKernelGGL((select_small_kernel<KPT, true>), bgrid(1 + (unsigned)pr.tiles), dim3(SEL_THREADS), sml, (hipStream_t)stream, score, (int)N, (int)k,   \
                          (int)n_sel, largest, perm, other, n_other, mask_ids, len_keep_dev, topk_sorted, P, g_use_rand,        \
-                         g_rand_seed, g_tick, g_merge_R, g_rows_out, g_rows_img, g_img_off, cur_batch())
+                         g_rand_seed, g_tick, g_merge_R, g_rows_out, g_rows_img, g_img_off, cur_batch(), pr)
       MHIMX_ONCE_PER_DEVICE(
-          MHIMX_HIP(hipFuncSetAttribute((const void*)select_small_kernel<16, true>, hipFuncAttributeMaxDynamicSharedMemorySize, (int)select_small_smem(4096)));
-          MHIMX_HIP(hipFuncSetAttribute((const void*)select_small_kernel<10, true>, hipFuncAttributeMaxDynamicSharedMemorySize, (int)select_small_smem(4096)));
-          MHIMX_HIP(hipFuncSetAttribute((const void*)select_small_kernel<4, true>, hipFuncAttributeMaxDynamicSharedMemorySize, (int)select_small_smem(4096))));
+          MHIMX_HIP(hipFuncSetAttribute((const void*)select_small_kernel<16, true>, hipFuncAttributeMaxDynamicSharedMemorySize, (int)(select_small_smem(4096) > PR_SMEM ? select_small_smem(4096) : PR_SMEM)));
+          MHIMX_HIP(hipFuncSetAttribute((const void*)select_small_kernel<10, true>, hipFuncAttributeMaxDynamicSharedMemorySize, (int)(select_small_smem(4096) > PR_SMEM ? select_small_smem(4096) : PR_SMEM)));
+          MHIMX_HIP(hipFuncSetAttribute((const void*)select_small_kernel<4, true>, hipFuncAttributeMaxDynamicSharedMemorySize, (int)(select_small_smem(4096) > PR_SMEM ? select_small_smem(4096) : PR_SMEM))));
       if (N <= 4096) MHIMX_SEL_LEAN(4);
       else if (N <= 10240) MHIMX_SEL_LEAN(10);
       else MHIMX_SEL_LEAN(16);
@@ -727,6 +739,27 @@
                      (int)merge_R, rows_out, rows_img, (int)img_merge_off);
 }
 
+extern "C" int mhimx_select_rows_pre(void* stream, const float* score, int64_t N, int64_t k, int64_t n_sel, int32_t largest, uint64_t rand_seed,
+                                     const uint64_t* tick, int64_t merge_R, int64_t* rows_out, int64_t* rows_img, int64_t img_merge_off, void* ws,
+                                     int64_t ws_bytes, int32_t merge_first, const mhimx_pre_rows* pre) {
+  if (!pre) return mhimx_select_rows_img(stream, score, N, k, n_sel, largest, rand_seed, tick, merge_R, rows_out, rows_img, img_merge_off, ws, ws_bytes, merge_first);
+  MHIMX_CHECK_ARG(rows_out && rows_img && merge_R >= 0 && merge_R <= N - n_sel && img_merge_off >= N - n_sel - merge_R && img_merge_off % 32 == 0 &&
+                      img_merge_off <= 32768,
+                  "select_rows_pre: bad args (the merged rows' image position is a multiple of 32 behind the rows that stay)");
+  const mhimx_scorer* sc = pre->sc;
+  MHIMX_CHECK_ARG(pre->T && pre->u_src && pre->s_src && sc && sc->wa_frag && sc->wc && sc->E == SF_E && sc->A == SF_A && !sc->gated &&
+                      sc->prec != MHIMX_PREC_F32 && pre->N >= 1 && pre->N <= 16384 && aligned16(pre->T) && aligned16(sc->wa_frag),
+                  "select_rows_pre: the row pass takes the one-pass scorer with its weight image (E = 512, A = 128, plain form, not f32, wa_frag), "
+                  "1 .. 16384 rows and 16-byte aligned rows");
+  static_assert(PR_THREADS == SEL_THREADS, "the riding row pass is written for the select's 1024 threads");
+  static_assert(PR_SMEM <= 160 * 1024, "a pre-select tile fits a CU's LDS");
+  PreRows pr = {};
+  pr.T = pre->T; pr.wa_frag = sc->wa_frag; pr.ba = sc->ba; pr.wc = sc->wc; pr.bc = sc->bc; pr.u_src = pre->u_src; pr.s_src = pre->s_src;
+  pr.N = (int)pre->N; pr.act = sc->act; pr.tiles = (int)cdiv(pre->N, PR_ROWS);
+  return select_impl(stream, score, N, k, n_sel, largest, nullptr, nullptr, 0, nullptr, nullptr, nullptr, ws, ws_bytes, merge_first ? 2 : 1, rand_seed, tick,
+                     (int)merge_R, rows_out, rows_img, (int)img_merge_off, &pr);
+}
+
 extern "C" int mhimx_vote_scores(void* stream, const float* attn, int64_t H, int64_t N, int64_t k, int32_t largest,
                                  float* vote, void* ws, int64_t ws_bytes) {
   (void)ws; (void)ws_bytes;
diff --git a/mhim_mil_amd/csrc/step.hip b/mhim_mil_amd/csrc/step.hip
--- a/mhim_mil_amd/csrc/step.hip
+++ b/mhim_mil_amd/csrc/step.hip
@@ -73,6 +73,7 @@
   int64_t logits, losses, g_z;
   int64_t dH, img, ws_b, ws_b_bytes, wg_ws, wg_ws_floats;
   int64_t q_scr, gslab;
+  int64_t u_src, s_src;
   int64_t rows_img, P0, L_img;
   int64_t bag0, bag_stride;
   int64_t total;
@@ -89,6 +90,8 @@
   lst->j[n0].G += t0;
   return 0;
 }
+
+bool pre_select_rows(const mhimx_step_cfg* c, int64_t N, int n_bags) { return n_bags == 1 && N <= 16384 && !c->no_pre_select; }
 
 int check_cfg(const mhimx_step_cfg* c, int64_t N, const mhimx_step_counts* n) {
   MHIMX_CHECK_ARG(c && n, "step: null configuration / counts");
@@ -161,6 +164,8 @@
   b->losses = cv.take_off(4 * F);
   b->g_z = cv.take_off(E * F);
   b->dH = cv.take_off((N + k) * E * F);
+  b->u_src = b->dH;
+  b->s_src = b->dH + N * A * F;
   b->img = cv.take_off(mhimx_wgrad_image_bytes(b->L_img, E));
   b->ws_b_bytes = (fuse_img ? b->P0 / 32 + (n->R + 31) / 32 : (n->len_keep + 31) / 32) * E * F;
   b->ws_b = cv.take_off(b->ws_b_bytes);
@@ -213,7 +218,8 @@
   return sc;
 }
 
-int mid_student_fwd(void* stream, const mhimx_step_cfg& c, const MidImages& im, const mhimx_merge& mw_prep, const MidBag& g, const MidDag* dag, MidFwd* f) {
+int mid_student_fwd(void* stream, const mhimx_step_cfg& c, const MidImages& im, const mhimx_merge& mw_prep, const MidBag& g, const MidDag* dag, MidFwd* f,
+                    const MidPre* pre) {
   const int64_t E = c.E, k = c.k;
   mhimx_merge& mw = f->mw;
   mw = mw_prep;
@@ -230,7 +236,9 @@
   } else {
     io.ride_merge = &mw; io.ride_X = g.Hbuf; io.ride_R = g.R; io.ride_ws = g.merge_ws; io.ride_ws_bytes = g.merge_ws_bytes;
   }
-  if (int r = mhimx_abmil_pool_fwd(dag ? dag->side_st : stream, &f->sc_s, &io)) return r;
+  if (pre) {
+    if (int r = mhimx_abmil_pool_fwd_pre(stream, &f->sc_s, &io, pre->u_src, pre->s_src)) return r;
+  } else if (int r = mhimx_abmil_pool_fwd(dag ? dag->side_st : stream, &f->sc_s, &io)) return r;
   mw.rows_done = io.rode_merge;
   if (int r = mhimx_merge_fwd(stream, &mw, g.Hbuf, g.R, g.Hbuf + g.N * E, g.q_out, 1, g.merge_ws, g.merge_ws_bytes)) return r;
   mw.rows_done = 0;
@@ -396,9 +404,13 @@
     }
   }
 
+  const MidPre pre = {cv.at<float>(b.u_src), cv.at<float>(b.s_src)};
+  const bool pre_on = pre_select_rows(cfg, N, 1) && !dag && cur_batch().n == 0;
   if (fuse_img) {
-    if (int r = mhimx_select_rows_img(stream, score, N, cnt->k_top, cnt->n_sel, 1, seeds->select, tick, R, rows_all, cv.at<int64_t>(b.rows_img), b.P0,
-                                      cv.at<char>(b.sel_ws), b.sel_ws_bytes, 1))
+    const mhimx_scorer sc_s = mid_scorer(c, S, im.wa_frag_s);
+    const mhimx_pre_rows pr = {Hbuf, N, &sc_s, cv.at<float>(b.u_src), cv.at<float>(b.s_src)};
+    if (int r = mhimx_select_rows_pre(stream, score, N, cnt->k_top, cnt->n_sel, 1, seeds->select, tick, R, rows_all, cv.at<int64_t>(b.rows_img), b.P0,
+                                      cv.at<char>(b.sel_ws), b.sel_ws_bytes, 1, pre_on ? &pr : nullptr))
       return r;
   } else {
     const SelLargeWs lw = {cv.at<int64_t>(b.sel_perm), cv.at<int64_t>(b.sel_ids), cv.at<int64_t>(b.sel_rows), cv.at<int64_t>(b.sel_lk), cv.at<char>(b.sel_ws),
@@ -409,7 +421,7 @@
   const MidBag bag = {Hbuf, dH, rows_all, N, R, Lk, seeds->mca, c.q_out ? c.q_out : S.q, cv.at<float>(b.s_s), cv.at<float>(b.stats_s), cv.at<float>(b.z_s),
                       cv.at<float>(b.g_z), cv.at<char>(b.pool_ws_s), b.pool_ws_s_bytes, merge_ws, b.merge_ws_bytes};
   MidFwd fwd;
-  if (int r = mid_student_fwd(stream, c, im, mw_prep, bag, dag, &fwd)) return r;
+  if (int r = mid_student_fwd(stream, c, im, mw_prep, bag, dag, &fwd, pre_on ? &pre : nullptr)) return r;
   if (int r = mid_head(stream, c, bag, cv.at<float>(b.z_t), label_dev, 1.f, cv.at<float>(b.logits), cv.at<float>(b.losses), c.grad, 0)) return r;
 
   mhimx_reduce_list lst;
diff --git a/mhim_mil_amd/csrc/step_mid.hpp b/mhim_mil_amd/csrc/step_mid.hpp
--- a/mhim_mil_amd/csrc/step_mid.hpp
+++ b/mhim_mil_amd/csrc/step_mid.hpp
@@ -19,11 +19,14 @@
 struct MidFwd { mhimx_merge mw; mhimx_scorer sc_s; mhimx_pool_io io_s; };
 struct MidImg { void* img; const void* dact; float* part; };
 
+struct MidPre { const float *u_src, *s_src; };
+
 mhimx_merge mid_merge_params(const mhimx_step_cfg& c);
 int mid_prep_head(const mhimx_step_cfg& c, const MidImages& im, mhimx_prep_job* j);
 int mid_prep_student(const mhimx_step_cfg& c, const MidImages& im, mhimx_prep_job* j);
 mhimx_scorer mid_scorer(const mhimx_step_cfg& c, const mhimx_step_params& p, const float* wa_frag);
-int mid_student_fwd(void* stream, const mhimx_step_cfg& c, const MidImages& im, const mhimx_merge& mw_prep, const MidBag& g, const MidDag* dag, MidFwd* f);
+int mid_student_fwd(void* stream, const mhimx_step_cfg& c, const MidImages& im, const mhimx_merge& mw_prep, const MidBag& g, const MidDag* dag, MidFwd* f,
+                    const MidPre* pre = nullptr);
 struct MidSurv { const float* censor; float alpha, eps; float* risk; };
 int mid_head(void* stream, const mhimx_step_cfg& c, const MidBag& g, const float* z_t, const int64_t* label, float loss_scale, float* logits,
              float* losses, const mhimx_step_grads& gr, int accumulate, const MidSurv* sv = nullptr);
diff --git a/mhim_mil_amd/engine.py b/mhim_mil_amd/engine.py
--- a/mhim_mil_amd/engine.py
+++ b/mhim_mil_amd/engine.py
@@ -439,6 +439,7 @@
         self._side = None
         self.step_dag = os.environ.get("MHIMX_STEP_DAG", "0") != "0"
         self.use_executor = os.environ.get("MHIMX_STEP_EXEC", "1") != "0"
+        self.pre_select = True
         self._exec, self.time_project = None, False
         self.exec_max_rows = 262144
         self.single_pass = True
@@ -939,6 +940,7 @@
         else:
             cfg.q_out = None
         cfg.time_project = int(bool(self.time_project))
+        cfg.no_pre_select = int(not self.pre_select)
         cfg.attn2score = int(bool(t.attn2score))
         cfg.drop_p_teacher = float(t.dropout_p if t.training else 0.0)
         cfg.merge_drop_p, cfg.merge_mm = float(s.merge.dropout), float(s.merge.g_q_mm)
diff --git a/mhim_mil_amd/ops.py b/mhim_mil_amd/ops.py
--- a/mhim_mil_amd/ops.py
+++ b/mhim_mil_amd/ops.py
@@ -324,6 +324,7 @@
         self.pscore = torch.empty(M1, device=dev) if (wp is not None and bp is not None) else None
         self.ws = None
         self.ride = None
+        self.u_pre = None
 
     def io(self, sc: ScorerW):
         M = self.M1 + self.M2
@@ -331,23 +332,32 @@
         if self.ws is None or self.ws.numel() < nbytes:
             self.ws = torch.empty(nbytes, device=self.T1.device, dtype=torch.uint8)
         return L.PoolIO(T1=_p(self.T1), M1=self.M1, T2=_p(self.T2), M2=self.M2, s=_p(self.s), stats=_p(self.stats),
-                        z=_p(self.z), u_pre=None, wp=_p(self.wp), C=0 if self.cproj is None else self.cproj.shape[1],
+                        z=_p(self.z), u_pre=_p(self.u_pre), wp=_p(self.wp), C=0 if self.cproj is None else self.cproj.shape[1],
                         cproj=_p(self.cproj), ws=_p(self.ws), ws_bytes=self.ws.numel(), bp=_p(self.bp), pscore=_p(self.pscore),
                         rows1=_p(self.rows1), excl=_p(self.excl),
                         ride_jobs=None if self.ride is None else C.cast(self.ride[0], C.c_void_p), n_ride_jobs=0 if self.ride is None else self.ride[1])
 
 
-def abmil_pool_fwd_split(sc: ScorerW, T1, rows1, tail_tokens, ride_merge=None):
-    _chk(T1, name="T1"); _chk(rows1, torch.int64, "rows1")
+def _pool_fwd_call(sc, io, pre, what):
+    if pre is None:
+        L.check(L.lib().mhimx_abmil_pool_fwd(_stream(), C.byref(sc.c), C.byref(io)), what)
+    else:
+        _chk(pre[0], name="pre_u"); _chk(pre[1], name="pre_s")
+        L.check(L.lib().mhimx_abmil_pool_fwd_pre(_stream(), C.byref(sc.c), C.byref(io), _p(pre[0]), _p(pre[1])), what + " (pre)")
+
+
+def abmil_pool_fwd_split(sc: ScorerW, T1, rows1, tail_tokens, ride_merge=None, pre=None, u_pre=None):
+    _chk(T1, name="T1"); _chk(rows1, torch.int64, "rows1"); _chk(u_pre, name="u_pre")
     st = PoolState(T1, None, 0, None, rows1=rows1)
     st.tail_tokens = int(tail_tokens)
+    st.u_pre = u_pre
     io = st.io(sc)
     io.phase, io.tail_tokens = 1, st.tail_tokens
     if ride_merge is not None:
         mw, X, ws = ride_merge
         io.ride_merge, io.ride_X = C.cast(C.pointer(mw.c), C.c_void_p), _p(X)
         io.ride_R, io.ride_ws, io.ride_ws_bytes = mw.x_rows.shape[0], _p(ws), ws.numel()
-    L.check(L.lib().mhimx_abmil_pool_fwd(_stream(), C.byref(sc.c), C.byref(io)), "mhimx_abmil_pool_fwd (phase 1)")
+    _pool_fwd_call(sc, io, pre, "mhimx_abmil_pool_fwd (phase 1)")
     return st, bool(io.rode_merge)
 
 
@@ -359,15 +369,16 @@
     return st
 
 
-def abmil_pool_fwd(sc: ScorerW, T1, T2=None, wp=None, bp=None, rows1=None, excl=None, ride_jobs=None, no_backward=False):
+def abmil_pool_fwd(sc: ScorerW, T1, T2=None, wp=None, bp=None, rows1=None, excl=None, ride_jobs=None, no_backward=False, pre=None, u_pre=None):
     _chk(T1, name="T1"); _chk(T2, name="T2"); _chk(wp, name="wp"); _chk(bp, name="bp"); _chk(rows1, torch.int64, "rows1")
-    _chk(excl, torch.uint8, "excl")
+    _chk(excl, torch.uint8, "excl"); _chk(u_pre, name="u_pre")
     st = PoolState(T1, T2, 0 if wp is None else wp.shape[0], wp, bp=bp, rows1=rows1, excl=excl)
     if ride_jobs:
         st.ride = (_prep_array(ride_jobs), len(ride_jobs))
+    st.u_pre = u_pre
     io = st.io(sc)
     io.no_backward = int(bool(no_backward))
-    L.check(L.lib().mhimx_abmil_pool_fwd(_stream(), C.byref(sc.c), C.byref(io)), "mhimx_abmil_pool_fwd")
+    _pool_fwd_call(sc, io, pre, "mhimx_abmil_pool_fwd")
     st.ride = None
     return st
 
@@ -462,6 +473,22 @@
                                           _p(tick), int(merge_R), _p(rows), _p(rows_img), int(img_merge_off), _p(ws), ws.numel(),
                                           int(bool(merge_first))), "mhimx_select_rows_img")
     return rows, rows_img
+
+
+def select_rows_pre(score, k, n_sel, merge_R, rand_seed, img_merge_off, sc: ScorerW, T, tick=None, largest=True, merge_first=True):
+    _chk(score, name="score"); _chk(T, name="T")
+    N = score.numel()
+    dev = score.device
+    rows = torch.empty(N - n_sel, device=dev, dtype=torch.int64)
+    rows_img = torch.empty(-(-(int(img_merge_off) + int(merge_R)) // 32) * 32, device=dev, dtype=torch.int64)
+    ws = torch.empty(L.lib().mhimx_select_ws_bytes(N), device=dev, dtype=torch.uint8)
+    u_src = torch.empty((T.shape[0], 128), device=dev)
+    s_src = torch.empty(T.shape[0], device=dev)
+    pre = L.PreRows(T=_p(T), N=T.shape[0], sc=C.cast(C.pointer(sc.c), C.c_void_p), u_src=_p(u_src), s_src=_p(s_src))
+    L.check(L.lib().mhimx_select_rows_pre(_stream(), _p(score), N, int(k), int(n_sel), int(bool(largest)), int(rand_seed) & 0xFFFFFFFFFFFFFFFF,
+                                          _p(tick), int(merge_R), _p(rows), _p(rows_img), int(img_merge_off), _p(ws), ws.numel(),
+                                          int(bool(merge_first)), C.byref(pre)), "mhimx_select_rows_pre")
+    return rows, rows_img, u_src, s_src
 
 
 def vote_scores(attn, k, largest=True):
```
